# miniufo/xinvert

Measured on AMD Instinct MI355X. Metric: SOR grid-points*iters/sec (fp64) at 3600x1800, masked points counted, higher is better.
Workload: dtype f64

## Files before the change

include/xinv.h:

```cpp
#ifndef XINV_H
#define XINV_H

#include <stdint.h>

#ifdef __cplusplus
extern "C" {
#endif

#define XINV_BC_FIXED    0
#define XINV_BC_EXTEND   1
#define XINV_BC_PERIODIC 2

#define XINV_OK          0
#define XINV_ERR_ARG    -1
#define XINV_ERR_HIP    -2
#define XINV_ERR_NODEV  -3
#define XINV_ERR_NOMEM  -4

#define XINV_PATH_AUTO   0
#define XINV_PATH_COLOUR 1
#define XINV_PATH_FUSED  2
#define XINV_PATH_WAVE1D 4

#define XINV_FLAG_NO_XUNIFORM 1
#define XINV_FLAG_NO_TILE_SKIP 2
#define XINV_FLAG_FORCE_TILE_SKIP 4
#define XINV_FLAG_FMA 32
#define XINV_FLAG_PIN_HOST 8

#define XINV_FLAG_NO_PIPE 16

#define XINV_FLAG_NO_POINT_FACTOR 64

#define XINV_MAX_DEVICES 16

typedef struct xinv_options {
    int32_t device;
    int32_t path;
    int32_t sweeps_per_launch;
    int32_t check_every;
    int32_t rows_per_tile;
    int32_t timing;
    int32_t flags;
    int32_t rowconst_mask;
    int32_t host_chunk;
    int32_t ndev;
    int32_t device_ids[XINV_MAX_DEVICES];
    int32_t prep_flags;
    int32_t f32_mask;
    double  prep_undef;
    double  demask_value;
    const double *prep_rowscale;
    int32_t lanes;
    int32_t norm_lag;
    int32_t pipe_fr;
    int32_t graph;
    int32_t cu_count;
    int32_t host_inflight;
} xinv_options;

#define XINV_PREP_MASK_NAN   1
#define XINV_PREP_MASK_VALUE 2
#define XINV_PREP_ROWSCALE   4
#define XINV_PREP_S_ZERO     8
#define XINV_PREP_DEMASK    16

typedef struct xinv_stats {
    int32_t path;
    int32_t colours;
    int32_t sweeps_per_launch;
    int32_t rows_per_tile;
    int32_t xuniform_mask;
    int32_t masked_tile_pct;
    int64_t sweep_launches;
    int64_t sweeps_max;
    double  sweep_ms;
    double  h2d_ms, d2h_ms;
    double  wall_ms;
    int32_t host_chunks;
    int32_t devices;
    int32_t pipelined;
    int32_t masked_tile_ppm;
    int32_t recovered_members;
    int32_t lanes;
    int32_t planned;
    int32_t point_factor;
    double  plan_ms;
    int32_t k_chunks;
    int32_t cut_tiles;
    int32_t rolling;
    int32_t reserved_;
    double  launch_us_min, launch_us_avg, launch_us_max;
} xinv_stats;

void        xinv_default_options(xinv_options *opt);
int         xinv_last_stats(xinv_stats *out);
const char *xinv_last_error(void);
int         xinv_device_count(void);
int         xinv_version(void);
void        xinv_abi_sizes(int32_t *options_bytes, int32_t *stats_bytes);

int xinv_standard_2d_f64(double *S, const double *A, const double *B, const double *C,
                         const double *F, int64_t yc, int64_t xc, double dely, double delx,
                         int BCy, int BCx, double delxSqr, double ratioQtr, double ratioSqr,
                         double optArg, double undef, double *flags, int64_t mxLoop,
                         double tolerance);

int xinv_general_2d_f64(double *S, const double *A, const double *B, const double *C,
                        const double *D, const double *E, const double *F, const double *G,
                        int64_t yc, int64_t xc, double dely, double delx, int BCy, int BCx,
                        double delxSqr, double ratio, double ratioQtr, double ratioSqr,
                        double optArg, double undef, double *flags, int64_t mxLoop,
                        double tolerance);

int xinv_standard_3d_f64(double *S, const double *A, const double *B, const double *C,
                         const double *F, int64_t zc, int64_t yc, int64_t xc, double delz,
                         double dely, double delx, int BCz, int BCy, int BCx, double delxSqr,
                         double ratio2Sqr, double ratio1Sqr, double optArg, double undef,
                         double *flags, int64_t mxLoop, double tolerance);

int xinv_standard_2d_f64_batched(double *S, const double *A, const double *B, const double *C,
                                 const double *F, int64_t nbatch, const int64_t *strides,
                                 int64_t yc, int64_t xc, double dely, double delx, int BCy,
                                 int BCx, double delxSqr, double ratioQtr, double ratioSqr,
                                 double optArg, double undef, double *flags, int64_t mxLoop,
                                 double tolerance, const xinv_options *opt);

int xinv_general_2d_f64_batched(double *S, const double *A, const double *B, const double *C,
                                const double *D, const double *E, const double *F,
                                const double *G, int64_t nbatch, const int64_t *strides,
                                int64_t yc, int64_t xc, double dely, double delx, int BCy,
                                int BCx, double delxSqr, double ratio, double ratioQtr,
                                double ratioSqr, double optArg, double undef, double *flags,
                                int64_t mxLoop, double tolerance, const xinv_options *opt);

int xinv_standard_3d_f64_batched(double *S, const double *A, const double *B, const double *C,
                                 const double *F, int64_t nbatch, const int64_t *strides,
                                 int64_t zc, int64_t yc, int64_t xc, double delz, double dely,
                                 double delx, int BCz, int BCy, int BCx, double delxSqr,
                                 double ratio2Sqr, double ratio1Sqr, double optArg,
                                 double undef, double *flags, int64_t mxLoop, double tolerance,
                                 const xinv_options *opt);

int xinv_standard_2d_f64_dev(double *S, const double *A, const double *B, const double *C,
                             const double *F, int64_t nbatch, const int64_t *strides,
                             int64_t yc, int64_t xc, double dely, double delx, int BCy,
                             int BCx, double delxSqr, double ratioQtr, double ratioSqr,
                             double optArg, double undef, double *flags, int64_t mxLoop,
                             double tolerance, const xinv_options *opt, void *stream);

int xinv_general_2d_f64_dev(double *S, const double *A, const double *B, const double *C,
                            const double *D, const double *E, const double *F, const double *G,
                            int64_t nbatch, const int64_t *strides, int64_t yc, int64_t xc,
                            double dely, double delx, int BCy, int BCx, double delxSqr,
                            double ratio, double ratioQtr, double ratioSqr, double optArg,
                            double undef, double *flags, int64_t mxLoop, double tolerance,
                            const xinv_options *opt, void *stream);

int xinv_standard_3d_f64_dev(double *S, const double *A, const double *B, const double *C,
                             const double *F, int64_t nbatch, const int64_t *strides,
                             int64_t zc, int64_t yc, int64_t xc, double delz, double dely,
                             double delx, int BCz, int BCy, int BCx, double delxSqr,
                             double ratio2Sqr, double ratio1Sqr, double optArg, double undef,
                             double *flags, int64_t mxLoop, double tolerance,
                             const xinv_options *opt, void *stream);

int xinv_general_3d_f64(double *S, const double *A, const double *B, const double *C,
                        const double *D, const double *E, const double *F, const double *G,
                        const double *H, int64_t zc, int64_t yc, int64_t xc, double delz,
                        double dely, double delx, int BCz, int BCy, int BCx, double delxSqr,
                        double ratio2, double ratio1, double ratio2Sqr, double ratio1Sqr,
                        double optArg, double undef, double *flags, int64_t mxLoop,
                        double tolerance);

int xinv_general_3d_f64_batched(double *S, const double *A, const double *B, const double *C,
                                const double *D, const double *E, const double *F,
                                const double *G, const double *H, int64_t nbatch,
                                const int64_t *strides, int64_t zc, int64_t yc, int64_t xc,
                                double delz, double dely, double delx, int BCz, int BCy, int BCx,
                                double delxSqr, double ratio2, double ratio1, double ratio2Sqr,
                                double ratio1Sqr, double optArg, double undef, double *flags,
                                int64_t mxLoop, double tolerance, const xinv_options *opt);

int xinv_general_3d_f64_dev(double *S, const double *A, const double *B, const double *C,
                            const double *D, const double *E, const double *F, const double *G,
// ... 145 lines not shown
```

xinvert_amd/_lib.py:

```python
import ctypes
import os

import numpy as np

HERE = os.path.dirname(os.path.abspath(__file__))
SO = os.environ.get('XINV_SO') or os.path.join(HERE, 'libxinv_hip.so')

BC_CODES = {'fixed': 0, 'extend': 1, 'periodic': 2}
PATH_AUTO, PATH_COLOUR, PATH_FUSED, PATH_WAVE1D = 0, 1, 2, 4
PREP_MASK_NAN, PREP_MASK_VALUE, PREP_ROWSCALE, PREP_S_ZERO, PREP_DEMASK = 1, 2, 4, 8, 16
MAX_DEVICES = 16

_dp = ctypes.POINTER(ctypes.c_double)
_ip = ctypes.POINTER(ctypes.c_int64)
_i64, _f64, _int, _vp = ctypes.c_int64, ctypes.c_double, ctypes.c_int, ctypes.c_void_p
_pvp = ctypes.POINTER(ctypes.c_void_p)


class XinvOptions(ctypes.Structure):
    _fields_ = [('device', ctypes.c_int32), ('path', ctypes.c_int32),
                ('sweeps_per_launch', ctypes.c_int32), ('check_every', ctypes.c_int32),
                ('rows_per_tile', ctypes.c_int32), ('timing', ctypes.c_int32),
                ('flags', ctypes.c_int32), ('rowconst_mask', ctypes.c_int32),
                ('host_chunk', ctypes.c_int32), ('ndev', ctypes.c_int32),
                ('device_ids', ctypes.c_int32 * MAX_DEVICES),
                ('prep_flags', ctypes.c_int32), ('f32_mask', ctypes.c_int32),
                ('prep_undef', ctypes.c_double), ('demask_value', ctypes.c_double),
                ('prep_rowscale', ctypes.POINTER(ctypes.c_double)),
                ('lanes', ctypes.c_int32), ('norm_lag', ctypes.c_int32),
                ('pipe_fr', ctypes.c_int32), ('graph', ctypes.c_int32),
                ('cu_count', ctypes.c_int32), ('host_inflight', ctypes.c_int32)]


class XinvStats(ctypes.Structure):
    _fields_ = [('path', ctypes.c_int32), ('colours', ctypes.c_int32),
                ('sweeps_per_launch', ctypes.c_int32), ('rows_per_tile', ctypes.c_int32),
                ('xuniform_mask', ctypes.c_int32), ('masked_tile_pct', ctypes.c_int32),
                ('sweep_launches', ctypes.c_int64), ('sweeps_max', ctypes.c_int64),
                ('sweep_ms', ctypes.c_double), ('h2d_ms', ctypes.c_double),
                ('d2h_ms', ctypes.c_double), ('wall_ms', ctypes.c_double),
                ('host_chunks', ctypes.c_int32), ('devices', ctypes.c_int32),
                ('pipelined', ctypes.c_int32), ('masked_tile_ppm', ctypes.c_int32),
                ('recovered_members', ctypes.c_int32), ('lanes', ctypes.c_int32),
                ('planned', ctypes.c_int32), ('point_factor', ctypes.c_int32), ('plan_ms', ctypes.c_double),
                ('k_chunks', ctypes.c_int32), ('cut_tiles', ctypes.c_int32),
                ('rolling', ctypes.c_int32), ('reserved_', ctypes.c_int32),
                ('launch_us_min', ctypes.c_double), ('launch_us_avg', ctypes.c_double),
                ('launch_us_max', ctypes.c_double)]


class XinvError(RuntimeError):
    pass


EXPORTS = [
    'xinv_default_options', 'xinv_last_stats', 'xinv_last_error', 'xinv_device_count',
    'xinv_version', 'xinv_abi_sizes',
    'xinv_standard_2d_f64', 'xinv_general_2d_f64', 'xinv_standard_3d_f64',
    'xinv_standard_2d_f64_batched', 'xinv_general_2d_f64_batched',
    'xinv_standard_3d_f64_batched',
    'xinv_standard_2d_f64_dev', 'xinv_general_2d_f64_dev', 'xinv_standard_3d_f64_dev',
    'xinv_general_bih_2d_f64', 'xinv_general_bih_2d_f64_batched', 'xinv_general_bih_2d_f64_dev',
    'xinv_standard_2d_test_f64', 'xinv_standard_2d_test_f64_batched', 'xinv_standard_2d_test_f64_dev',
    'xinv_general_3d_f64', 'xinv_general_3d_f64_batched', 'xinv_general_3d_f64_dev',
    'xinv_standard_1d_f64', 'xinv_standard_1d_f64_batched', 'xinv_standard_1d_f64_dev',
    'xinv_gm_flow_f64_dev',
    'xinv_abs_norm_f64_dev',
    'xinv_fd_f64', 'xinv_fd_f64_dev',
    'xinv_mg_restrict_f64_dev', 'xinv_mg_prolong_f64_dev',
    'xinv_plan_create_standard_2d_f64_dev', 'xinv_plan_create_general_2d_f64_dev',
    'xinv_plan_create_standard_3d_f64_dev', 'xinv_plan_create_general_3d_f64_dev',
    'xinv_plan_create_general_bih_2d_f64_dev', 'xinv_plan_create_standard_2d_test_f64_dev',
    'xinv_plan_solve_f64_dev', 'xinv_plan_solve_frames_f64_dev', 'xinv_plan_refresh', 'xinv_plan_destroy',
]

_lib = None


def load():
    global _lib
    if _lib is not None:
        return _lib
    if not os.path.exists(SO):
        raise XinvError('HIP extension %s is missing: run `python -m xinvert_amd.build` '
                        '(there is no CPU fallback)' % SO)
    try:
        import torch
    except ImportError:
        pass
    try:
        L = ctypes.CDLL(SO)
    except OSError as e:
        raise XinvError('cannot load %s: %s' % (SO, e))
    _opt = ctypes.POINTER(XinvOptions)
    from . import forms
    for kind, f in forms.FORMS.items():
        for entry in ('single', 'batched', 'dev') + (('plan',) if f.resident else ()):
            getattr(L, forms.symbol(kind, entry)).argtypes = forms.argtypes(kind, entry)
    L.xinv_gm_flow_f64_dev.argtypes = [_vp, _vp, _vp, _i64, _i64, _i64, _vp, _vp, _int, _int, _vp, _f64, _int, _vp]
    L.xinv_abs_norm_f64_dev.argtypes = [_vp, _i64, _f64, _dp, _vp]
    fd_args = [_pvp, _int, _pvp, _int, _int, _ip, _int, _int, _ip, _dp, _vp, _i64, _int, _i64]
    L.xinv_fd_f64.argtypes = fd_args
    L.xinv_fd_f64_dev.argtypes = fd_args + [_vp]
    L.xinv_mg_restrict_f64_dev.argtypes = [_vp, _vp, _i64, _int, _ip, _ip, _f64, _vp]
    L.xinv_mg_prolong_f64_dev.argtypes = [_vp, _vp, _vp, _i64, _int, _ip, _ip, _vp, _vp, _int, _f64, _vp]
    L.xinv_plan_solve_f64_dev.argtypes = [_vp, _vp, _dp, _i64, _f64, _vp]
    L.xinv_plan_solve_frames_f64_dev.argtypes = [_vp, _vp, _vp, _i64, _i64, _dp, _i64, _f64, _vp]
    L.xinv_plan_refresh.argtypes = [_vp, _vp]
    L.xinv_plan_destroy.argtypes = [_vp]
    for name in EXPORTS:
        getattr(L, name).restype = _int
    L.xinv_last_error.restype = ctypes.c_char_p
    L.xinv_default_options.restype = None
    L.xinv_default_options.argtypes = [_opt]
    L.xinv_last_stats.argtypes = [ctypes.POINTER(XinvStats)]
    so, ss = ctypes.c_int32(0), ctypes.c_int32(0)
    try:
        abi_sizes = L.xinv_abi_sizes
    except AttributeError:
        raise XinvError('%s predates xinv_abi_sizes (a stale prebuilt library): rebuild it with '
                        '`python -m xinvert_amd.build --force`' % SO) from None
    abi_sizes.restype = None
    abi_sizes(ctypes.byref(so), ctypes.byref(ss))
    if (so.value, ss.value) != (ctypes.sizeof(XinvOptions), ctypes.sizeof(XinvStats)):
        raise XinvError('%s was built from another include/xinv.h: xinv_options %d / xinv_stats %d bytes there, %d / %d '
                        'in xinvert_amd/_lib.py' % (SO, so.value, ss.value, ctypes.sizeof(XinvOptions),
                                                    ctypes.sizeof(XinvStats)))
    _lib = L
    return L


def require_gpu():
    L = load()
    if L.xinv_device_count() < 1:
        raise XinvError('libxinv_hip.so loaded but no MI355X/HIP device is visible '
                        '(there is no CPU fallback)')
    return L


def check(rc):
    if rc != 0:
        raise XinvError('xinv call failed (rc=%d): %s' % (rc, load().xinv_last_error().decode()))


def options(device=-1, path=PATH_AUTO, sweeps_per_launch=0, check_every=0, rows_per_tile=0,
            timing=0, no_xuniform=0, no_tile_skip=0, force_tile_skip=0, rowconst_mask=0,
            host_chunk=0, devices=None, prep=None, pin_host=0, no_pipe=0, fma=0, f32_mask=0,
            lanes=0, norm_lag=0, pipe_fr=0, graph=0, no_point_factor=0, cu_count=0, host_inflight=0):
    o = XinvOptions()
    load().xinv_default_options(ctypes.byref(o))
    o.device, o.path, o.sweeps_per_launch = device, path, sweeps_per_launch
    o.check_every, o.rows_per_tile, o.timing = check_every, rows_per_tile, timing
    o.flags = (1 if no_xuniform else 0) | (2 if no_tile_skip else 0) | (4 if force_tile_skip else 0) | \
              (8 if pin_host else 0) | (16 if no_pipe else 0) | (32 if fma else 0) | \
              (64 if no_point_factor else 0)
    o.rowconst_mask = int(rowconst_mask)
    o.host_chunk = int(host_chunk)
    o.f32_mask = int(f32_mask)
    o.lanes, o.norm_lag, o.pipe_fr, o.graph = int(lanes), int(norm_lag), int(pipe_fr), int(graph)
    o.cu_count = int(cu_count)
    o.host_inflight = int(host_inflight)
    if prep:
        fl = 0
        if isinstance(prep.get('mask'), str):
            fl |= PREP_MASK_NAN
        elif prep.get('mask') is not None:
            fl |= PREP_MASK_VALUE
            o.prep_undef = float(prep['mask'])
        if prep.get('rowscale') is not None:
            rs = np.ascontiguousarray(prep['rowscale'], dtype=np.float64)
            o._rowscale_keepalive = rs
            o.prep_rowscale = rs.ctypes.data_as(ctypes.POINTER(ctypes.c_double))
            fl |= PREP_ROWSCALE
        if prep.get('s_zero'):
            fl |= PREP_S_ZERO
        if 'demask' in prep and prep['demask'] is not None:
            fl |= PREP_DEMASK
            o.demask_value = float(prep['demask'])
        o.prep_flags = fl
    if devices is None:
        o.ndev = 0
    elif isinstance(devices, str):
        if devices != 'all':
            raise XinvError("devices must be None, 'all' or a list of device ordinals")
        o.ndev = -1
    else:
        devices = [int(d) for d in devices]
        if len(devices) > MAX_DEVICES:
            raise XinvError('at most %d devices' % MAX_DEVICES)
        o.ndev = len(devices)
        for i, d in enumerate(devices):
            o.device_ids[i] = d
    return o


def last_stats():
    s = XinvStats()
    load().xinv_last_stats(ctypes.byref(s))
    return {f: getattr(s, f) for f, _ in XinvStats._fields_}


def bc(b):
    if isinstance(b, str):
        if b not in BC_CODES:
            raise XinvError('unknown boundary condition %r' % (b,))
        return BC_CODES[b]
    return int(b)


def hptr(a, f32=False):
    if a is None:
        return None
    want = np.float32 if f32 else np.float64
    if a.dtype != want or not a.flags.c_contiguous:
        raise XinvError('need a C-contiguous %s array at the C-ABI here, got %s%s'
                        % (np.dtype(want).name, a.dtype.name, '' if a.flags.c_contiguous else ' (not contiguous)'))
    return ctypes.cast(a.ctypes.data, _dp)


def strides_arg(vals):
    return (ctypes.c_int64 * len(vals))(*[int(v) for v in vals])
```

xinvert_amd/csrc/xinv_device.h:

```cpp
#pragma once
#include <hip/hip_runtime.h>
#include <stdint.h>
#include <float.h>
#include <math.h>

#define XINV_WAVE 64

__device__ __forceinline__ void xinv_fresh_scalar_cache()
{
    asm volatile("s_dcache_inv\n\ts_waitcnt lgkmcnt(0)" ::: "memory");
}

struct XinvCtl {
    double normPrev;
    double flag1;
    double flag2;
    long long loop;
    long long sweeps;
    int done;
    int overflow;
    int wrote;
    unsigned ticket;
    unsigned seq;
    unsigned pad_;
};

struct XinvStop {
    long long mxLoop;
    double tolerance;
    int stop_on_zero_norm;
};

__device__ __forceinline__ int xinv_ctl_done(const XinvCtl *c)
{
    return __hip_atomic_load(&c->done, __ATOMIC_RELAXED, __HIP_MEMORY_SCOPE_AGENT);
}
__device__ __forceinline__ unsigned xinv_ctl_seq(const XinvCtl *c)
{
    return __hip_atomic_load(&c->seq, __ATOMIC_RELAXED, __HIP_MEMORY_SCOPE_AGENT);
}

__device__ __forceinline__ void xinv_ctl_update(XinvCtl *c, double sum, long long count,
                                                const XinvStop &st)
{
    if (c->done) return;
    double norm = (count != 0) ? sum / (double)count : NAN;
    if (isnan(norm) || norm > 1e100) {
        c->overflow = 1;
        c->done = 1;
        c->sweeps = c->loop + 1;
        return;
    }
    c->flag1 = fabs(norm - c->normPrev) / c->normPrev;
    c->flag2 = (double)c->loop;
    c->wrote = 1;
    if (c->flag1 < st.tolerance || c->loop >= st.mxLoop ||
        (st.stop_on_zero_norm && norm == 0.0)) {
        c->done = 1;
        c->sweeps = c->loop + 1;
        return;
    }
    c->normPrev = norm;
    c->loop += 1;
}

template <int CTRL, int ROW_MASK>
__device__ __forceinline__ double xinv_dpp_add(double v)
{
    int lo = __builtin_amdgcn_update_dpp(0, __double2loint(v), CTRL, ROW_MASK, 0xf, true);
    int hi = __builtin_amdgcn_update_dpp(0, __double2hiint(v), CTRL, ROW_MASK, 0xf, true);
    return v + __hiloint2double(hi, lo);
}

__device__ __forceinline__ double xinv_wave_sum(double v)
{
    v = xinv_dpp_add<0x111, 0xf>(v);
    v = xinv_dpp_add<0x112, 0xf>(v);
    v = xinv_dpp_add<0x114, 0xf>(v);
    v = xinv_dpp_add<0x118, 0xf>(v);
    v = xinv_dpp_add<0x142, 0xa>(v);
    v = xinv_dpp_add<0x143, 0xc>(v);
    const int lo = __builtin_amdgcn_readlane(__double2loint(v), 63);
    const int hi = __builtin_amdgcn_readlane(__double2hiint(v), 63);
    return __hiloint2double(hi, lo);
}

template <int CTRL, int ROW_MASK>
__device__ __forceinline__ long long xinv_dpp_add_ll(long long v)
{
    const int lo = __builtin_amdgcn_update_dpp(0, (int)(unsigned long long)v, CTRL, ROW_MASK, 0xf, true);
    const int hi = __builtin_amdgcn_update_dpp(0, (int)((unsigned long long)v >> 32), CTRL, ROW_MASK, 0xf, true);
    return v + (long long)(((unsigned long long)(unsigned)hi << 32) | (unsigned)lo);
}

__device__ __forceinline__ long long xinv_wave_sum_ll(long long v)
{
    v = xinv_dpp_add_ll<0x111, 0xf>(v);
    v = xinv_dpp_add_ll<0x112, 0xf>(v);
    v = xinv_dpp_add_ll<0x114, 0xf>(v);
    v = xinv_dpp_add_ll<0x118, 0xf>(v);
    v = xinv_dpp_add_ll<0x142, 0xa>(v);
    v = xinv_dpp_add_ll<0x143, 0xc>(v);
    const unsigned lo = (unsigned)__builtin_amdgcn_readlane((int)(unsigned long long)v, 63);
    const unsigned hi = (unsigned)__builtin_amdgcn_readlane((int)((unsigned long long)v >> 32), 63);
    return (long long)(((unsigned long long)hi << 32) | lo);
}

__device__ __forceinline__ double xinv_lane_up(double v)
{
    int lo = __double2loint(v), hi = __double2hiint(v);
    lo = __builtin_amdgcn_update_dpp(0, lo, 0x138, 0xf, 0xf, true);
    hi = __builtin_amdgcn_update_dpp(0, hi, 0x138, 0xf, 0xf, true);
    return __hiloint2double(hi, lo);
}

__device__ __forceinline__ double xinv_lane_down(double v)
{
    int lo = __double2loint(v), hi = __double2hiint(v);
    lo = __builtin_amdgcn_update_dpp(0, lo, 0x130, 0xf, 0xf, true);
    hi = __builtin_amdgcn_update_dpp(0, hi, 0x130, 0xf, 0xf, true);
    return __hiloint2double(hi, lo);
}

__device__ __forceinline__ double xinv_add_where(double a, double b, unsigned long long mask)
{
    unsigned long long sv;
    asm("s_and_saveexec_b64 %1, %3\n\tv_add_f64 %0, %0, %2\n\ts_mov_b64 exec, %1"
        : "+v"(a), "=&s"(sv) : "v"(b), "s"(mask) : "scc");
    return a;
}
__device__ __forceinline__ double xinv_add_abs_where(double a, double b, unsigned long long mask)
{
    unsigned long long sv;
    asm("s_and_saveexec_b64 %1, %3\n\tv_add_f64 %0, %0, |%2|\n\ts_mov_b64 exec, %1"
        : "+v"(a), "=&s"(sv) : "v"(b), "s"(mask) : "scc");
    return a;
}

__device__ __forceinline__ double xinv_add_where_ne(double a, double b, double f, double u, unsigned long long rowmask)
{
    unsigned long long sv;
    asm("s_and_saveexec_b64 %1, %5\n\tv_cmpx_neq_f64_e32 vcc, %4, %3\n\tv_add_f64 %0, %0, %2\n\ts_mov_b64 exec, %1"
        : "+v"(a), "=&s"(sv) : "v"(b), "v"(f), "s"(u), "s"(rowmask) : "scc", "vcc");
    return a;
}
__device__ __forceinline__ double xinv_fma_where_ne(double a, double t, double rq, double f, double u, unsigned long long rowmask)
{
    unsigned long long sv;
    asm("s_and_saveexec_b64 %1, %6\n\tv_cmpx_neq_f64_e32 vcc, %5, %4\n\tv_fma_f64 %0, %2, %3, %0\n\ts_mov_b64 exec, %1"
        : "+v"(a), "=&s"(sv) : "v"(t), "s"(rq), "v"(f), "s"(u), "s"(rowmask) : "scc", "vcc");
    return a;
}
__device__ __forceinline__ void xinv_norm_row(double &sx, double &sy, int &nx, int &ny, double x, double y, double u)
{
    unsigned long long sv;
    asm("s_mov_b64 %4, exec\n\t"
        "v_cmpx_neq_f64_e32 vcc, %7, %5\n\tv_add_f64 %0, %0, |%5|\n\tv_add_u32 %2, %2, 1\n\ts_mov_b64 exec, %4\n\t"
        "v_cmpx_neq_f64_e32 vcc, %7, %6\n\tv_add_f64 %1, %1, |%6|\n\tv_add_u32 %3, %3, 1\n\ts_mov_b64 exec, %4"
        : "+v"(sx), "+v"(sy), "+v"(nx), "+v"(ny), "=&s"(sv) : "v"(x), "v"(y), "s"(u) : "vcc");
}

struct XinvScal {
    double delx, delxSqr, ratio, ratioQtr, ratioSqr;
    double ratio2Sqr, ratio1Sqr;
    double ratio2, ratio1;
    double delxSSr, delxTr, ratioSSr;
    double optArg, undef;
};


__device__ __forceinline__ double xinv_upd_std2d_9(
    double sC, double sP, double sM, double sW, double sE,
    double sPE, double sPW, double sME, double sMW, double sM_q,
    double aP, double a0, double bE, double bW, double bP_chk, double bP_use, double bM,
    double cE, double c0, double f, const XinvScal &sc)
{
    const double u = sc.undef;
    bool cond = (f != u) && (aP != u) && (a0 != u) && (bE != u) && (bW != u) &&
                (bP_chk != u) && (bM != u) && (cE != u) && (c0 != u);
    if (!cond) return sC;
    double temp = (
        (
            aP * (sP - sC) -
            a0 * (sC - sM)
        ) * sc.ratioSqr + (
            bP_use * (sPE - sPW) -
            bM * (sM_q - sMW)
        ) * sc.ratioQtr + (
            bE * (sPE - sME) -
            bW * (sPW - sMW)
        ) * sc.ratioQtr + (
            cE * (sE - sC) -
            c0 * (sC - sW)
        )
    ) - f * sc.delxSqr;
    temp *= sc.optArg / ((aP + a0) * sc.ratioSqr + (cE + c0));
    return sC + temp;
}

__device__ __forceinline__ double xinv_upd_std2d_5(
    double sC, double sP, double sM, double sW, double sE,
    double aP, double a0, double cE, double c0, double f, bool inrange, const XinvScal &sc)
{
    const double u = sc.undef;
    bool cond = inrange && (f != u) && (aP != u) && (a0 != u) && (cE != u) && (c0 != u);
    double temp = (
        (
            aP * (sP - sC) -
            a0 * (sC - sM)
        ) * sc.ratioSqr + (
            cE * (sE - sC) -
            c0 * (sC - sW)
        )
    ) - f * sc.delxSqr;
    temp *= sc.optArg / ((aP + a0) * sc.ratioSqr + (cE + c0));
    return cond ? sC + temp : sC;
}

__device__ __forceinline__ double xinv_upd_gen2d_9(
    double sC, double sP, double sM, double sW, double sE,
    double sPE, double sPW, double sME, double sMW,
    double A, double B, double C, double D, double E, double F, double G, const XinvScal &sc)
{
    const double u = sc.undef;
    bool cond = (G != u) && (A != u) && (B != u) && (C != u) && (D != u) && (E != u) && (F != u);
    if (!cond) return sC;
    double temp = (
        A * (
            (sP - sC) - (sC - sM)
        ) * sc.ratioSqr +
        B * (
            (sPE - sME) - (sPW - sMW)
        ) * sc.ratioQtr +
        C * (
            (sE - sC) - (sC - sW)
        ) + (
        D * (
            (sP - sM)
        ) * sc.ratio +
        E * (
            (sE - sW)
        )) * sc.delx / 2.0 + (
        F * sC - G) * sc.delxSqr
    );
    temp *= sc.optArg / ((A * sc.ratioSqr + C) * 2.0
                         - F * sc.delxSqr);
    return sC + temp;
}

__device__ __forceinline__ double xinv_upd_gen2d_5(
    double sC, double sP, double sM, double sW, double sE,
    double A, double C, double D, double E, double F, double G, bool inrange,
    const XinvScal &sc)
{
    const double u = sc.undef;
    bool cond = inrange && (G != u) && (A != u) && (C != u) && (D != u) && (E != u) && (F != u);
    double temp = (
        A * (
            (sP - sC) - (sC - sM)
        ) * sc.ratioSqr +
        C * (
            (sE - sC) - (sC - sW)
        ) + (
        D * (
            (sP - sM)
        ) * sc.ratio +
        E * (
            (sE - sW)
        )) * sc.delx / 2.0 + (
        F * sC - G) * sc.delxSqr
    );
    temp *= sc.optArg / ((A * sc.ratioSqr + C) * 2.0
                         - F * sc.delxSqr);
    return cond ? sC + temp : sC;
}

__device__ __forceinline__ double xinv_upd_std3d(
    double sC, double sKP, double sKM, double sJP, double sJM, double sE, double sW,
    double aP, double a0, double bP, double b0, double cE, double c0, double f,
    const XinvScal &sc)
{
    const double u = sc.undef;
    bool cond = (f != u) && (aP != u) && (a0 != u) && (bP != u) && (b0 != u) &&
                (cE != u) && (c0 != u);
    if (!cond) return sC;
    double temp = (
        (
            aP * (sKP - sC) -
            a0 * (sC - sKM)
        ) * sc.ratio2Sqr + (
            bP * (sJP - sC) -
            b0 * (sC - sJM)
        ) * sc.ratio1Sqr + (
            cE * (sE - sC) -
            c0 * (sC - sW)
        )
    ) - f * sc.delxSqr;
    temp *= sc.optArg / ((aP + a0) * sc.ratio2Sqr +
                         (bP + b0) * sc.ratio1Sqr +
                         (cE + c0));
    return sC + temp;
}

__device__ __forceinline__ double xinv_upd_gen3d(
    double sC, double sKP, double sKM, double sJP, double sJM, double sE, double sW,
    double A, double B, double C, double D, double E, double F, double G, double H, bool testH,
    const XinvScal &sc)
{
    const double u = sc.undef;
    bool cond = (!testH || H != u) && (G != u) && (A != u) && (B != u) && (C != u) && (D != u) &&
                (E != u) && (F != u);
    if (!cond) return sC;
// ... 191 lines not shown
```

xinvert_amd/csrc/xinv_dispatch.h:

```cpp
#pragma once
#include <hip/hip_runtime.h>
#include "xinv_fused.h"
#include "xinv_pipe2d.h"
#include "xinv_fused3d.h"
#include "xinv_fused3dg.h"
#include "xinv_pipe3d.h"
#include "xinv_fusedbih.h"

#define XINV_HIDDEN __attribute__((visibility("hidden")))

XINV_HIDDEN int xinv_launch_fused2d_std(bool al, bool ext, unsigned um, int K, dim3 grid, dim3 block,
                                        hipStream_t st, const FusedArgs &a, int *occ);
XINV_HIDDEN int xinv_launch_fused2d_gen(bool al, bool ext, unsigned um, int K, dim3 grid, dim3 block,
                                        hipStream_t st, const FusedArgs &a, int *occ);
XINV_HIDDEN int xinv_launch_fused2d_std2dt(bool al, bool ext, unsigned um, int K, dim3 grid, dim3 block,
                                           hipStream_t st, const FusedArgs &a, int *occ);
XINV_HIDDEN int xinv_launch_fused2d_std_seam(bool al, bool ext, unsigned um, int K, dim3 grid, dim3 block,
                                             hipStream_t st, const FusedArgs &a, int *occ);
XINV_HIDDEN int xinv_launch_fused2d_gen_seam(bool al, bool ext, unsigned um, int K, dim3 grid, dim3 block,
                                             hipStream_t st, const FusedArgs &a, int *occ);
XINV_HIDDEN int xinv_launch_fused2d_std2dt_seam(bool al, bool ext, unsigned um, int K, dim3 grid, dim3 block,
                                                hipStream_t st, const FusedArgs &a, int *occ);
XINV_HIDDEN int xinv_launch_fused2d_stdf(bool al, bool ext, unsigned um, int K, dim3 grid, dim3 block,
                                         hipStream_t st, const FusedArgs &a, int *occ);
XINV_HIDDEN int xinv_launch_fused2d_genf(bool al, bool ext, unsigned um, int K, dim3 grid, dim3 block,
                                         hipStream_t st, const FusedArgs &a, int *occ);
XINV_HIDDEN int xinv_launch_fused2d_genq(bool al, bool ext, unsigned um, int K, dim3 grid, dim3 block,
                                         hipStream_t st, const FusedArgs &a, int *occ);
XINV_HIDDEN int xinv_launch_pipe2d_fma(bool gen, unsigned um, bool fr, bool al, bool ext, dim3 grid, hipStream_t st,
                                       const FusedArgs &a, int *occ, int lds_pad);
XINV_HIDDEN int xinv_launch_pipe2d_std(unsigned um, int np, bool fr, bool al, bool ext, dim3 grid, hipStream_t st,
                                       const FusedArgs &a, int *occ, int lds_pad);
XINV_HIDDEN int xinv_launch_pipe2d_gen(unsigned um, int np, bool fr, bool al, bool ext, dim3 grid, hipStream_t st,
                                       const FusedArgs &a, int *occ, int lds_pad);
XINV_HIDDEN int xinv_launch_pipe2d_std_seam(unsigned um, int np, bool fr, bool al, bool ext, dim3 grid, hipStream_t st,
                                            const FusedArgs &a, int *occ, int lds_pad);
XINV_HIDDEN int xinv_launch_pipe2d_gen_seam(unsigned um, int np, bool fr, bool al, bool ext, dim3 grid, hipStream_t st,
                                            const FusedArgs &a, int *occ, int lds_pad);
static inline int xinv_launch_pipe2d(bool gen, unsigned um, int np, bool fr, bool al, bool ext, dim3 grid, hipStream_t st,
                                     const FusedArgs &a, int *occ, int lds_pad = 0, bool seam = false, bool fma = false)
{
    if (fma) return (seam || np != 1) ? 1 : xinv_launch_pipe2d_fma(gen, um, fr, al, ext, grid, st, a, occ, lds_pad);
    if (seam) return gen ? xinv_launch_pipe2d_gen_seam(um, np, fr, al, ext, grid, st, a, occ, lds_pad)
                         : xinv_launch_pipe2d_std_seam(um, np, fr, al, ext, grid, st, a, occ, lds_pad);
    return gen ? xinv_launch_pipe2d_gen(um, np, fr, al, ext, grid, st, a, occ, lds_pad)
               : xinv_launch_pipe2d_std(um, np, fr, al, ext, grid, st, a, occ, lds_pad);
}
XINV_HIDDEN int xinv_launch_fused9(bool gen, int K, bool al, bool ext, dim3 grid, hipStream_t st,
                                   const FusedArgs &a, int *occ, bool seam = false);
XINV_HIDDEN int xinv_launch_fused3d(int NW, bool al, bool uni, bool ext, dim3 grid, hipStream_t st,
                                    const Fused3Args &a);
XINV_HIDDEN int xinv_launch_pipe3d(bool al, dim3 grid, hipStream_t st, const Fused3Args &a, bool seam = false, bool ext = false);
XINV_HIDDEN int xinv_launch_fused3d_seam(int NW, bool uni, bool ext, dim3 grid, hipStream_t st, const Fused3Args &a);
XINV_HIDDEN int xinv_launch_fused3dg_seam(int NW, bool ext, dim3 grid, hipStream_t st, const Fused3GArgs &a);
XINV_HIDDEN int xinv_launch_fused3d_fma(int NW, bool al, bool ext, dim3 grid, hipStream_t st, const Fused3Args &a);
XINV_HIDDEN int xinv_launch_pipe3d_fma(bool al, dim3 grid, hipStream_t st, const Fused3Args &a);
XINV_HIDDEN int xinv_launch_fused3dg(int NW, bool al, bool ext, dim3 grid, hipStream_t st,
                                     const Fused3GArgs &a);
XINV_HIDDEN int xinv_launch_fusedbih(bool per, bool zbe, int vm, dim3 grid, hipStream_t st,
                                     const FusedBihArgs &a, int *occ);
```

xinvert_amd/csrc/xinv_fused.h:

```cpp
#pragma once
#include "xinv_device.h"
#include <type_traits>
#include <utility>

#define XINV_KMAX 4
#ifndef XINV_TEST_HOOKS
#define XINV_TEST_HOOKS 0
#endif
#if XINV_TEST_HOOKS
#define XINV_WATCHDOG_TICKS 3000000ull
#else
#define XINV_WATCHDOG_TICKS 200000000ull
#endif
__device__ __forceinline__ bool xinv_hook_withhold(const void *hook, int T, unsigned tag, int64_t m)
{
#if XINV_TEST_HOOKS
    const int *h = reinterpret_cast<const int *>(hook);
    return h && __hip_atomic_load(h + 0, __ATOMIC_RELAXED, __HIP_MEMORY_SCOPE_AGENT) == T &&
           (unsigned)__hip_atomic_load(h + 1, __ATOMIC_RELAXED, __HIP_MEMORY_SCOPE_AGENT) == tag &&
           (int64_t)__hip_atomic_load(h + 2, __ATOMIC_RELAXED, __HIP_MEMORY_SCOPE_AGENT) == m;
#else
    (void)hook; (void)T; (void)tag; (void)m;
    return false;
#endif
}
typedef int64_t row_t;

struct FusedArgs {
    const double *src;
    double *dst;
    const double *c[7];
    int64_t sS, sc[7];
    int64_t yc, xc;
    int per, ext, tall;
    int nstrip, nrb, RY;
    int nwg;
    int force, no_ctl;
    int lag;
    unsigned tag;
    unsigned long long *lagp_psum;
    const double *lagp_xsum;
    const long long *lagp_xcnt;
    int lagp_NB, lagp_K;
    unsigned lagp_tag;
    int64_t member0;
    XinvScal sc_;
    XinvCtl *ctl;
    XinvStop stop;
    unsigned long long *psum;
    const int *tile_list;
    int ntl;
    const double *xsum;
    const long long *xcnt;
    const void *rowf;
    double *dbg;
};

#include "xinv_tiles.h"

template <class F, int... U>
__device__ __forceinline__ void xinv_unroll_steps(F &&f, std::integer_sequence<int, U...>)
{
    (f(std::integral_constant<int, U>{}), ...);
}

template <int X> __device__ __forceinline__ double comp(const double2 &v) { return X ? v.y : v.x; }
template <int X> __device__ __forceinline__ void setc(double2 &v, double t) { if (X) v.y = t; else v.x = t; }

template <int X> __device__ __forceinline__ void row_neighbours(const double2 &row, double &w, double &e)
{
    if (X == 0) { w = xinv_lane_up(row.y); e = row.y; }
    else        { w = row.x; e = xinv_lane_down(row.x); }
}

template <int NC, int D> struct CoefWin {
    double2 v[NC][D];
    double s[NC][D];
    double rq[D];
    double2 rqv[D];
    unsigned mx[D], my[D];
};

__device__ __forceinline__ unsigned xinv_lane_word(bool b)
{
    unsigned m = b ? ~0u : 0u;
    return m;
}

__device__ __forceinline__ double xinv_bitsel(unsigned m, double a, double b)
{
    const unsigned long long ua = (unsigned long long)__double_as_longlong(a);
    const unsigned long long ub = (unsigned long long)__double_as_longlong(b);
    const unsigned lo = ((unsigned)ua & m) | ((unsigned)ub & ~m);
    const unsigned hi = ((unsigned)(ua >> 32) & m) | ((unsigned)(ub >> 32) & ~m);
    return __longlong_as_double((long long)(((unsigned long long)hi << 32) | lo));
}

__device__ __forceinline__ double xinv_bitsel64(unsigned long long m, double a, double b)
{
    unsigned lo, hi;
    asm("v_cndmask_b32_e64 %0, %2, %3, %6\n\tv_cndmask_b32_e64 %1, %4, %5, %6"
        : "=&v"(lo), "=&v"(hi)
        : "v"((unsigned)__double2loint(b)), "v"((unsigned)__double2loint(a)),
          "v"((unsigned)__double2hiint(b)), "v"((unsigned)__double2hiint(a)), "s"(m));
    return __hiloint2double((int)hi, (int)lo);
}

template <int X, unsigned UM, int Q, int NC, int D>
__device__ __forceinline__ double cget(const CoefWin<NC, D> &w, int slot)
{
    if ((UM >> Q) & 1u) return w.s[Q][slot];
    return comp<X>(w.v[Q][slot]);
}

struct FusedStd2D {
    static constexpr int NC = 3;
    template <unsigned UM> static constexpr bool hoist() { return (UM & 3u) == 3u; }
    static constexpr int PIPE_PFR = 2;

    template <unsigned UM, int D, bool PRE = true>
    static __device__ __forceinline__ void derive(CoefWin<NC, D> &w, int sr, int s1, bool okx, bool oky,
                                                  const XinvScal &sc)
    {
        const double u = sc.undef;
        const double fx = cget<0, UM, 2>(w, s1), fy = cget<1, UM, 2>(w, s1);
        bool bx = okx && (fx != u), by = oky && (fy != u);
        if (hoist<UM>()) {
            const double aP = w.s[0][sr], a0 = w.s[0][s1], c = w.s[1][s1];
            w.rq[s1] = sc.optArg / ((aP + a0) * sc.ratioSqr + (c + c));
            const bool rok = (aP != u) && (a0 != u) && (c != u);
            bx = bx && rok; by = by && rok;
        } else {
            const double aPx = cget<0, UM, 0>(w, sr), aPy = cget<1, UM, 0>(w, sr);
            const double a0x = cget<0, UM, 0>(w, s1), a0y = cget<1, UM, 0>(w, s1);
            const double c0x = cget<0, UM, 1>(w, s1), c0y = cget<1, UM, 1>(w, s1);
            const double cEy = ((UM >> 1) & 1u) ? w.s[1][s1] : xinv_lane_down(w.v[1][s1].x);
            bx = bx && (aPx != u) && (a0x != u) && (c0y != u) && (c0x != u);
            by = by && (aPy != u) && (a0y != u) && (cEy != u) && (c0y != u);
        }
        w.mx[s1] = xinv_lane_word(bx);
        w.my[s1] = xinv_lane_word(by);
        if (PRE) {
            if (!((UM >> 2) & 1u)) { w.v[2][s1].x = fx * sc.delxSqr; w.v[2][s1].y = fy * sc.delxSqr; }
            else                   w.s[2][s1] = fx * sc.delxSqr;
        }
    }

    template <int X, unsigned UM, int D, bool PRE = true>
    static __device__ __forceinline__ double inc(const CoefWin<NC, D> &w, int sj, int sjp, double sC,
                                                 double sP, double sM, double sW, double sE,
                                                 const XinvScal &sc)
    {
        const double aP = cget<X, UM, 0>(w, sjp);
        const double a0 = cget<X, UM, 0>(w, sj);
        const double c0 = cget<X, UM, 1>(w, sj);
        double cE;
        if ((UM >> 1) & 1u) cE = w.s[1][sj];
        else if (X == 0)    cE = w.v[1][sj].y;
        else                cE = xinv_lane_down(w.v[1][sj].x);
        const double fd = PRE ? cget<X, UM, 2>(w, sj)
                              : cget<X, UM, 2>(w, sj) * sc.delxSqr;
        double temp = (
            (
                aP * (sP - sC) -
                a0 * (sC - sM)
            ) * sc.ratioSqr + (
                cE * (sE - sC) -
                c0 * (sC - sW)
            )
        ) - fd;
        if (hoist<UM>()) temp *= w.rq[sj];
        else             temp *= sc.optArg / ((aP + a0) * sc.ratioSqr + (cE + c0));
        return temp;
    }
    template <int X, unsigned UM, int D, bool PRE = true>
    static __device__ __forceinline__ double upd(const CoefWin<NC, D> &w, int sj, int sjp, double sC,
                                                 double sP, double sM, double sW, double sE,
                                                 const XinvScal &sc)
    {
        const double temp = inc<X, UM, D, PRE>(w, sj, sjp, sC, sP, sM, sW, sE, sc);
        return xinv_bitsel(X ? w.my[sj] : w.mx[sj], sC + temp, sC);
    }
};

struct FusedStd2DT {
    static constexpr int NC = 4;
    template <unsigned UM> static constexpr bool hoist() { return (UM & 7u) == 7u; }

    template <unsigned UM, int D>
    static __device__ __forceinline__ void derive(CoefWin<NC, D> &w, int sr, int s1, bool okx, bool oky,
                                                  const XinvScal &sc)
    {
        const double u = sc.undef;
        bool bx = okx && (cget<0, UM, 3>(w, s1) != u), by = oky && (cget<1, UM, 3>(w, s1) != u);
        if (hoist<UM>()) {
            const double aP = w.s[0][sr], a0 = w.s[0][s1], d = w.s[1][s1], e = w.s[2][s1];
            w.rq[s1] = sc.optArg / ((aP + a0) * sc.ratioSqr +
                                    (d + d) - e * sc.delxSqr);
            const bool rok = (aP != u) && (a0 != u) && (d != u) && (e != u);
            bx = bx && rok; by = by && rok;
        } else {
            const double d0x = cget<0, UM, 1>(w, s1), d0y = cget<1, UM, 1>(w, s1);
            const double dEy = ((UM >> 1) & 1u) ? w.s[1][s1] : xinv_lane_down(w.v[1][s1].x);
            bx = bx && (cget<0, UM, 0>(w, sr) != u) && (cget<0, UM, 0>(w, s1) != u) && (d0y != u) &&
                 (d0x != u) && (cget<0, UM, 2>(w, s1) != u);
            by = by && (cget<1, UM, 0>(w, sr) != u) && (cget<1, UM, 0>(w, s1) != u) && (dEy != u) &&
                 (d0y != u) && (cget<1, UM, 2>(w, s1) != u);
// ... 68 lines not shown
    template <int X, unsigned UM, int D, bool PRE = true>
    static __device__ __forceinline__ double inc(const CoefWin<NC, D> &w, int sj, int, double sC,
                                                 double sP, double sM, double sW, double sE,
                                                 const XinvScal &sc)
    {
        const double A = cget<X, UM, 0>(w, sj), C = cget<X, UM, 1>(w, sj);
        const double Dd = cget<X, UM, 2>(w, sj), E = cget<X, UM, 3>(w, sj);
        const double F = cget<X, UM, 4>(w, sj), G = cget<X, UM, 5>(w, sj);
        double temp = (
            A * (
                (sP - sC) - (sC - sM)
            ) * sc.ratioSqr +
            C * (
                (sE - sC) - (sC - sW)
            ) + (
            Dd * (
                (sP - sM)
            ) * sc.ratio +
            E * (
                (sE - sW)
            )) * sc.delx / 2.0 + (
            F * sC - G) * sc.delxSqr
        );
        if (hoist<UM>()) temp *= w.rq[sj];
        else if (PRE)    temp *= comp<X>(w.rqv[sj]);
        else             temp *= sc.optArg / ((A * sc.ratioSqr + C) * 2.0
                                              - F * sc.delxSqr);
        return temp;
    }
    template <int X, unsigned UM, int D, bool PRE = true>
    static __device__ __forceinline__ double upd(const CoefWin<NC, D> &w, int sj, int sjp, double sC,
                                                 double sP, double sM, double sW, double sE,
                                                 const XinvScal &sc)
    {
        const double temp = inc<X, UM, D, PRE>(w, sj, sjp, sC, sP, sM, sW, sE, sc);
        return xinv_bitsel(X ? w.my[sj] : w.mx[sj], sC + temp, sC);
    }
};

struct FusedStd2DF : FusedStd2D {
    static constexpr bool FMA = true;
    template <unsigned UM, int D, bool PRE = true>
    static __device__ __forceinline__ void derive(CoefWin<NC, D> &w, int sr, int s1, bool okx, bool oky,
                                                  const XinvScal &sc)
    { FusedStd2D::derive<UM, D, false>(w, sr, s1, okx, oky, sc); }
    template <int X, unsigned UM, int D, bool PRE = true>
    static __device__ __forceinline__ double inc(const CoefWin<NC, D> &w, int sj, int sjp, double sC,
                                                 double sP, double sM, double sW, double sE,
                                                 const XinvScal &sc)
    {
        static_assert(hoist<UM>(), "contracted arithmetic: per-row A and C only");
        const double aP = w.s[0][sjp], a0 = w.s[0][sj], c = w.s[1][sj];
        const double y = __builtin_fma(aP, sP - sC, -(a0 * (sC - sM)));
        const double x = __builtin_fma(c, sE - sC, -(c * (sC - sW)));
        double t = __builtin_fma(y, sc.ratioSqr, x);
        t = __builtin_fma(-cget<X, UM, 2>(w, sj), sc.delxSqr, t);
        return t;
    }
    template <int X, unsigned UM, int D, bool PRE = true>
    static __device__ __forceinline__ double upd(const CoefWin<NC, D> &w, int sj, int sjp, double sC,
                                                 double sP, double sM, double sW, double sE,
                                                 const XinvScal &sc)
    {
        const double t = inc<X, UM, D, PRE>(w, sj, sjp, sC, sP, sM, sW, sE, sc);
        return xinv_bitsel(X ? w.my[sj] : w.mx[sj], __builtin_fma(t, w.rq[sj], sC), sC);
    }
};

struct FusedGen2DF : FusedGen2D {
    static constexpr bool FMA = true;
    template <int X, unsigned UM, int D, bool PRE = true>
    static __device__ __forceinline__ double inc(const CoefWin<NC, D> &w, int sj, int, double sC,
                                                 double sP, double sM, double sW, double sE,
                                                 const XinvScal &sc)
    {
        static_assert((UM & 0x1fu) == 0x1fu, "contracted arithmetic: per-row A, C, D, E, F only");
        const double A = w.s[0][sj], C = w.s[1][sj], Dd = w.s[2][sj], E = w.s[3][sj], F = w.s[4][sj];
        const double G = cget<X, UM, 5>(w, sj);
        double t = (A * ((sP - sC) - (sC - sM))) * sc.ratioSqr;
        t = __builtin_fma(C, (sE - sC) - (sC - sW), t);
        double v = (Dd * (sP - sM)) * sc.ratio;
        v = __builtin_fma(E, sE - sW, v);
        t = __builtin_fma(v * sc.delx, 0.5, t);
        t = __builtin_fma(__builtin_fma(F, sC, -G), sc.delxSqr, t);
        return t;
    }
    template <int X, unsigned UM, int D, bool PRE = true>
    static __device__ __forceinline__ double upd(const CoefWin<NC, D> &w, int sj, int sjp, double sC,
                                                 double sP, double sM, double sW, double sE,
                                                 const XinvScal &sc)
    {
        const double t = inc<X, UM, D, PRE>(w, sj, sjp, sC, sP, sM, sW, sE, sc);
        return xinv_bitsel(X ? w.my[sj] : w.mx[sj], __builtin_fma(t, w.rq[sj], sC), sC);
    }
};

template <bool AC> struct FusedGen2DQ_ {
    static constexpr int NC = 7;
    static constexpr bool PQ = true;
    static constexpr int QI = 5;
    template <unsigned UM> static constexpr bool hoist() { return false; }
    static constexpr int PIPE_PFR = 1;
    template <unsigned UM, int D, bool PRE = true>
    static __device__ __forceinline__ void derive(CoefWin<NC, D> &w, int, int s1, bool okx, bool oky, const XinvScal &)
    {
        w.mx[s1] = xinv_lane_word(okx && (w.v[QI][s1].x != 0.0));
        w.my[s1] = xinv_lane_word(oky && (w.v[QI][s1].y != 0.0));
    }
    template <int X, unsigned UM, int D, bool PRE = true>
    static __device__ __forceinline__ double upd(const CoefWin<NC, D> &w, int sj, int sjp, double sC,
                                                 double sP, double sM, double sW, double sE,
                                                 const XinvScal &sc)
    {
        const double temp = inc<X, UM, D, PRE>(w, sj, sjp, sC, sP, sM, sW, sE, sc);
        return xinv_bitsel(X ? w.my[sj] : w.mx[sj], sC + temp, sC);
    }
    template <int X, unsigned UM, int D, bool PRE = true>
    static __device__ __forceinline__ double inc(const CoefWin<NC, D> &w, int sj, int, double sC,
                                                 double sP, double sM, double sW, double sE,
                                                 const XinvScal &sc)
    {
        const double A = cget<X, UM, 0>(w, sj), C = AC ? A : cget<X, UM, 1>(w, sj);
        const double Dd = cget<X, UM, 2>(w, sj), E = cget<X, UM, 3>(w, sj);
        const double F = cget<X, UM, 4>(w, sj), G = cget<X, UM, 6>(w, sj);
        double temp = (
            A * (
                (sP - sC) - (sC - sM)
            ) * sc.ratioSqr +
            C * (
                (sE - sC) - (sC - sW)
            ) + (
            Dd * (
                (sP - sM)
            ) * sc.ratio +
            E * (
                (sE - sW)
            )) * sc.delx / 2.0 + (
            F * sC - G) * sc.delxSqr
        );
        temp *= cget<X, UM, QI>(w, sj);
        return temp;
    }
};
using FusedGen2DQ = FusedGen2DQ_<false>;
using FusedGen2DQA = FusedGen2DQ_<true>;
template <class M, class = void> struct ModelPQ { static constexpr bool value = false; };
template <class M> struct ModelPQ<M, std::void_t<decltype(M::PQ)>> { static constexpr bool value = M::PQ; };

template <class M, class = void> struct ModelFma { static constexpr bool value = false; };
template <class M> struct ModelFma<M, std::void_t<decltype(M::FMA)>> { static constexpr bool value = M::FMA; };

template <int NC> struct RowPack { double2 s; double2 c[NC]; double cs[NC]; };

struct LaneCols {
    int64_t l0, l1;
    bool ok_x, ok_y;
    bool use_x, use_y;
    int cls_x, cls_y;
};

template <bool AL>
__device__ __forceinline__ double2 ld2(const double *p, int64_t row_off, const LaneCols &lc)
{
    if (AL) return *reinterpret_cast<const double2 *>(p + row_off + lc.l0);
    double2 v; v.x = p[row_off + lc.l0]; v.y = p[row_off + lc.l1]; return v;
}

template <bool AL>
__device__ __forceinline__ LaneCols make_lanecols(int64_t xu0, int H, int UW, int lane, int64_t xc,
                                                  bool per, int np = 1, int q = 0)
{
    LaneCols lc;
    const int64_t c0 = xu0 - H + 2 * np * lane + 2 * q, c1 = c0 + 1;
    if (per) {
        int64_t w0 = c0 % xc; if (w0 < 0) w0 += xc;
        int64_t w1 = c1 % xc; if (w1 < 0) w1 += xc;
        lc.l0 = w0; lc.l1 = w1;
        lc.ok_x = lc.ok_y = true;
        lc.cls_x = lc.cls_y = 1;
    } else {
        if (AL) {
            int64_t p = c0 < 0 ? 0 : (c0 > xc - 2 ? xc - 2 : c0);
            lc.l0 = p; lc.l1 = p + 1;
        } else {
            lc.l0 = c0 < 0 ? 0 : (c0 > xc - 1 ? xc - 1 : c0);
            lc.l1 = c1 < 0 ? 0 : (c1 > xc - 1 ? xc - 1 : c1);
        }
        lc.ok_x = (c0 >= 1 && c0 <= xc - 2);
        lc.ok_y = (c1 >= 1 && c1 <= xc - 2);
        lc.cls_x = lc.ok_x ? 1 : (c0 == 0 ? 2 : (c0 == xc - 1 ? 3 : 0));
        lc.cls_y = lc.ok_y ? 1 : (c1 == xc - 1 ? 3 : 0);
    }
    lc.use_x = (c0 >= xu0 && c0 < xu0 + UW && c0 < xc);
    lc.use_y = (c1 >= xu0 && c1 < xu0 + UW && c1 < xc);
    return lc;
}

struct RingSeam { unsigned long long lanes; bool any; };
__device__ __forceinline__ LaneCols make_lanecols_ring(int64_t xu0, int HW, int UW, int lane, int64_t xc, RingSeam &rs)
{
    LaneCols lc;
    const int64_t c0 = xu0 - HW + 2 * lane, c1 = c0 + 1, xv = xc + 1;
    int64_t w0 = c0 % xv; if (w0 < 0) w0 += xv;
    int64_t w1 = c1 % xv; if (w1 < 0) w1 += xv;
    lc.l0 = w0; lc.l1 = (w1 == xc) ? xc - 1 : w1;
    lc.ok_x = true; lc.ok_y = (w1 != xc);
    lc.cls_x = lc.cls_y = 1;
    lc.use_x = (c0 >= xu0 && c0 < xu0 + UW && c0 < xc);
    lc.use_y = (c1 >= xu0 && c1 < xu0 + UW && c1 < xc);
    rs.lanes = __builtin_amdgcn_ballot_w64(w0 == xc - 1);
    rs.any = rs.lanes != 0ull;
    return lc;
}

__device__ __forceinline__ void fused_extend_fix(double2 &edge, const double2 &inner,
                                                 const LaneCols &lc, bool tall, double u)
{
    const double inner_w = xinv_lane_up(inner.y);
    if (lc.cls_x == 1) { if (inner.x != u) edge.x = inner.x; }
    else if (lc.cls_x == 2) { if (inner.y != u) edge.x = inner.y; }
    else if (lc.cls_x == 3) {
        if (tall && inner.x != u) edge.x = inner.x;
        if (inner_w != u) edge.x = inner_w;
    }
    if (lc.cls_y == 1) { if (inner.y != u) edge.y = inner.y; }
    else if (lc.cls_y == 3) {
        if (tall && inner.y != u) edge.y = inner.y;
        if (inner.x != u) edge.y = inner.x;
    }
}

#define XINV_PW 3
template <int K, int NWV, bool EXTS = false>
__device__ __forceinline__ void xinv_norm_publish(const double (&acc)[K], const int (&cnt)[K],
                                                  int wave, int lane, int NB, int T, unsigned tag,
                                                  unsigned long long *pw, char *scr = nullptr, bool withhold = false)
{
    double (*ls)[K]; long long (*lcn)[K];
    if constexpr (EXTS) {
        ls = reinterpret_cast<double (*)[K]>(scr);
        lcn = reinterpret_cast<long long (*)[K]>(scr + sizeof(double) * NWV * K);
    } else {
        __shared__ double ls_[NWV][K];
        __shared__ long long lcn_[NWV][K];
        ls = ls_; lcn = lcn_;
    }
#pragma unroll
    for (int s = 0; s < K; s++) {
        double ws = xinv_wave_sum(acc[s]);
        long long wc = xinv_wave_sum_ll((long long)cnt[s]);
        if (lane == 0) { ls[wave][s] = ws; lcn[wave][s] = wc; }
    }
    __syncthreads();
    const unsigned long long hi = (unsigned long long)tag << 32;
    if (threadIdx.x < K && !withhold) {
        const int s = threadIdx.x;
        double ts = 0.0; long long tc = 0;
        for (int q = 0; q < NWV; q++) { ts += ls[q][s]; tc += lcn[q][s]; }
        const unsigned long long bits = (unsigned long long)__double_as_longlong(ts);
        unsigned long long *q = pw + ((size_t)s * NB + T) * XINV_PW;
        __hip_atomic_store(q + 0, hi | (bits & 0xffffffffull), __ATOMIC_RELAXED, __HIP_MEMORY_SCOPE_AGENT);
        __hip_atomic_store(q + 1, hi | (bits >> 32), __ATOMIC_RELAXED, __HIP_MEMORY_SCOPE_AGENT);
        __hip_atomic_store(q + 2, hi | (unsigned long long)(unsigned)tc, __ATOMIC_RELAXED,
                           __HIP_MEMORY_SCOPE_AGENT);
    }
}

template <int K, int NWV, bool EXTS = false>
__device__ __forceinline__ void xinv_norm_reduce(int wave, int lane, int NB, unsigned tag,
                                                 unsigned long long *pw, XinvCtl *ctl, const XinvStop &stop,
                                                 double xsum, long long xcnt, char *scr = nullptr)
{
    double (*ls)[K]; long long (*lcn)[K]; unsigned *s_timeout_p;
    if constexpr (EXTS) {
        ls = reinterpret_cast<double (*)[K]>(scr);
        lcn = reinterpret_cast<long long (*)[K]>(scr + sizeof(double) * NWV * K);
        s_timeout_p = reinterpret_cast<unsigned *>(scr + 2 * sizeof(double) * NWV * K);
    } else {
        __shared__ double ls_[NWV][K];
        __shared__ long long lcn_[NWV][K];
        __shared__ unsigned s_timeout_;
        ls = ls_; lcn = lcn_; s_timeout_p = &s_timeout_;
    }
#define s_timeout (*s_timeout_p)
    if (threadIdx.x == 0) s_timeout = 0u;
    const unsigned long long hi = (unsigned long long)tag << 32;
    constexpr int NT = NWV * XINV_WAVE, C = 4;
    const int tid = threadIdx.x, nitem = K * NB;
    double ps[K]; long long pc[K];
#pragma unroll
    for (int s = 0; s < K; s++) { ps[s] = 0.0; pc[s] = 0; }
    unsigned long long t0 = 0;
    bool timed_out = false;
    for (int base = 0; base < nitem && !timed_out; base += NT * C) {
        unsigned long long w[C][XINV_PW];
        bool ready;
        do {
            ready = true;
#pragma unroll
            for (int c = 0; c < C; c++) {
                const int i = base + c * NT + tid;
                if (i < nitem) {
#pragma unroll
                    for (int k = 0; k < XINV_PW; k++)
                        w[c][k] = __hip_atomic_load(pw + (size_t)i * XINV_PW + k, __ATOMIC_RELAXED,
                                                    __HIP_MEMORY_SCOPE_AGENT);
                } else {
#pragma unroll
                    for (int k = 0; k < XINV_PW; k++) w[c][k] = hi;
                }
            }
#pragma unroll
            for (int c = 0; c < C; c++)
#pragma unroll
                for (int k = 0; k < XINV_PW; k++) ready = ready && ((unsigned)(w[c][k] >> 32) == tag);
            if (!ready) {
                const unsigned long long now = __builtin_amdgcn_s_memrealtime();
                if (t0 == 0) t0 = now;
                else if (now - t0 > XINV_WATCHDOG_TICKS) { timed_out = true; s_timeout = 1u; }
            }
        } while (!ready && !timed_out);
#pragma unroll
        for (int c = 0; c < C; c++) {
            const int i = base + c * NT + tid;
            const double v = __longlong_as_double((long long)((w[c][1] << 32) | (w[c][0] & 0xffffffffull)));
            const long long n = (long long)(unsigned)w[c][2];
#pragma unroll
            for (int s = 0; s < K; s++) {
                const bool mine = (i < nitem) && (i >= s * NB) && (i < (s + 1) * NB);
                ps[s] += mine ? v : 0.0;
                pc[s] += mine ? n : 0;
            }
        }
    }
    __syncthreads();
    if (s_timeout) {
        if (tid == 0) {
            ctl->overflow = 2; ctl->done = 1; ctl->sweeps = ctl->loop + 1;
            ctl->seq = tag + 1u;
        }
        return;
    }
#pragma unroll
    for (int s = 0; s < K; s++) {
        double ws = xinv_wave_sum(ps[s]);
        long long wc = xinv_wave_sum_ll(pc[s]);
        if (lane == 0) { ls[wave][s] = ws; lcn[wave][s] = wc; }
    }
    __syncthreads();
    if (tid == 0) {
#pragma unroll
        for (int s = 0; s < K; s++) {
            double ts = 0.0; long long tc = 0;
            for (int q = 0; q < NWV; q++) { ts += ls[q][s]; tc += lcn[q][s]; }
            xinv_ctl_update(ctl, ts + xsum, tc + xcnt, stop);
        }
        ctl->seq = tag + 1u;
    }
#undef s_timeout
}

template <int K, int NWV, bool EXTS = false>
__device__ __forceinline__ void xinv_norm_finalize(const double (&acc)[K], const int (&cnt)[K],
// ... 441 lines not shown
```

xinvert_amd/csrc/xinv_launch.h:

```cpp
#pragma once

static inline unsigned cdiv(int64_t a, int64_t b) { return (unsigned)((a + b - 1) / b); }

#if XINV_TEST_HOOKS
static thread_local int *t_hook_record = nullptr;
#endif

struct Plan {
    int path, base, seam, ncol;
    int K, RY, nsg, nrb;
    int nkc, KC;
    bool K2;
    int nsg2, nrb2, nkc2, KC2;
    int joff2;
    int cus;
    int64_t srowf2;
    bool bih_zbe;
    int bih_vm;
    bool aligned;
    unsigned umask;
    unsigned um;
    bool even_split;
    bool nine;
    bool skip;
    SkipNormArgs skipna;
    int ntl, nskip;
    int skip_pct;
    int skip_ppm;
    double lone = 1.6;
    bool pipe;
    int tpw;
    int npair;
    bool pipe_fr;
    int64_t xc;
    bool fma;
    bool alias_ac;
    bool pq;
};

static unsigned pick_um(int kind, unsigned umask)
{
    if (kind == KIND_STD2D) return ((umask & 3u) == 3u) ? 3u : 0u;
    if (kind == KIND_STD2DT) return ((umask & 7u) == 7u) ? 7u : 0u;
    if ((umask & 0x1fu) == 0x1fu) return 0x1fu;
    if ((umask & 0x1cu) == 0x1cu) return 0x1cu;
    return 0u;
}

struct StreamMap {
    int n, c[6];
    int forcing;
    int nuni;
};
static const StreamMap &stream_map(int kind)
{
    static const StreamMap std2d = {3, {0, 2, 3}, 2, 2}, std2dt = {4, {0, 3, 4, 5}, 3, 3}, gen2d = {6, {0, 2, 3, 4, 5, 6}, 5, 5};
    return kind == KIND_STD2D ? std2d : (kind == KIND_STD2DT ? std2dt : gen2d);
}

static inline int strip_uw(const Plan &pl, int K, bool pipe)
{
    if (pl.seam) return xinv_ring_uw(pl.xc, pipe ? 2 * XINV_PIPE_P : 2 * K);
    return pipe ? XINV_PIPE_UW(pl.npair) : 128 - 4 * K;
}

static int p3_extend_joff(int64_t yc)
{
    static_assert(XINV_P3_RR == 3 && XINV_P3_G * XINV_P3_RR - 8 > 0, "k_pipe3d: three rows per wavefront");
    return xinv_p3_extend_joff(yc, XINV_P3_G * XINV_P3_RR - 8, 4, XINV_P3_RR);
}

static int fused_dispatch(int kind, bool al, bool ext, unsigned um, int K, dim3 grid, dim3 block,
                          hipStream_t st, const FusedArgs &a, int *occ, bool seam = false, bool fma = false, bool pq = false)
{
    if (pq) return (kind != KIND_GEN2D || seam || fma) ? 1 : xinv_launch_fused2d_genq(al, ext, um, K, grid, block, st, a, occ);
    if (fma) {
        if (seam || kind == KIND_STD2DT) return 1;
        return kind == KIND_GEN2D ? xinv_launch_fused2d_genf(al, ext, um, K, grid, block, st, a, occ)
                                  : xinv_launch_fused2d_stdf(al, ext, um, K, grid, block, st, a, occ);
    }
    if (seam) {
        if (kind == KIND_GEN2D) return xinv_launch_fused2d_gen_seam(al, ext, um, K, grid, block, st, a, occ);
        if (kind == KIND_STD2DT) return xinv_launch_fused2d_std2dt_seam(al, ext, um, K, grid, block, st, a, occ);
        return xinv_launch_fused2d_std_seam(al, ext, um, K, grid, block, st, a, occ);
    }
    if (kind == KIND_GEN2D) return xinv_launch_fused2d_gen(al, ext, um, K, grid, block, st, a, occ);
    if (kind == KIND_STD2DT) return xinv_launch_fused2d_std2dt(al, ext, um, K, grid, block, st, a, occ);
    return xinv_launch_fused2d_std(al, ext, um, K, grid, block, st, a, occ);
}

static bool ptr_al16(const void *p) { return (((uintptr_t)p) & 15u) == 0; }
static bool vec_aligned(const double *a, int64_t stride) { return ptr_al16(a) && !(stride & 1); }

template <class F>
static int for_member_chunks(int64_t member0, int64_t nmem, F launch, int64_t chunk = XINV_MEMBER_CHUNK)
{
    for (int64_t m0 = 0; m0 < nmem; m0 += chunk) {
        const int rc = launch(member0 + m0, std::min<int64_t>(chunk, nmem - m0));
        if (rc) return rc;
    }
    return XINV_OK;
}

static void launch_extend(const Problem &p, const Workspace *ws, hipStream_t st, double *S, int force, int64_t member0, int64_t nm)
{
    ExtendArgs e;
    e.S = S; e.sS = p.sS; e.yc = p.yc; e.xc = p.xc;
    e.kfirst = is3d(p.kind) ? 1 : 0;
    e.nk = is3d(p.kind) ? p.zc - 2 : 1;
    e.per = (p.BCx == XINV_BC_PERIODIC); e.tall = (p.kind != KIND_STD3D) && (p.yc > p.xc); e.force = force;
    e.undef = p.sc_.undef; e.ctl = ws->ctl; e.member0 = member0;
    dim3 g(cdiv(p.xc, 256), (unsigned)e.nk, (unsigned)nm), b(256, 1, 1);
    if (p.kind == KIND_BIH2D) hipLaunchKernelGGL(k_extend_bih, g, b, 0, st, e);
    else                      hipLaunchKernelGGL(k_extend, g, b, 0, st, e);
}

struct TsumPtrs { double *tsum; long long *tcnt; double *xsum; long long *xcnt; unsigned *ticket; size_t bytes; };
static TsumPtrs tsum_layout(void *buf, int64_t nbatch, int nskip)
{
    const size_t nb = (size_t)nbatch, nt = nb * (size_t)nskip, pair = sizeof(double) + sizeof(long long);
    const uintptr_t base = (uintptr_t)buf;
    TsumPtrs t;
    t.tsum = (double *)base;
    t.tcnt = (long long *)(base + nt * sizeof(double));
    t.xsum = (double *)(base + nt * pair);
    t.xcnt = (long long *)(base + nt * pair + nb * sizeof(double));
    t.ticket = (unsigned *)(base + (nt + nb) * pair);
    t.bytes = (nt + nb) * pair + nb * sizeof(unsigned);
    return t;
}

template <class A>
static void set_skip(A &a, const Workspace *ws, const Problem &p, const Plan &pl, int tpw)
{
    a.tile_list = ws->d_list;
    a.ntl = pl.ntl;
    a.nwg = pl.ntl / tpw;
    const TsumPtrs t = tsum_layout(ws->d_tsum, p.nbatch, pl.nskip);
    a.xsum = t.xsum; a.xcnt = t.xcnt;
}

template <class A>
static void set_lag(A &a, const Workspace *ws, const Problem &p, int K, unsigned lag_tag, NormLagArgs *lag_out,
                    const NormLagArgs *lag_prev)
{
    if (lag_tag) {
        a.lag = 1; a.tag = lag_tag;
        a.psum = (unsigned long long *)((char *)ws->partials + (size_t)((lag_tag - 1u) & 1u) * ws->partials_half);
        if (lag_prev && lag_prev->tag) {
            a.lagp_psum = lag_prev->psum; a.lagp_xsum = lag_prev->xsum; a.lagp_xcnt = lag_prev->xcnt;
            a.lagp_NB = lag_prev->NB; a.lagp_K = lag_prev->K; a.lagp_tag = lag_prev->tag;
        }
    }
    if (lag_out) {
        memset(lag_out, 0, sizeof *lag_out);
        lag_out->psum = a.psum; lag_out->ctl = ws->ctl; lag_out->stop = p.stop;
        lag_out->xsum = a.xsum; lag_out->xcnt = a.xcnt; lag_out->NB = a.nwg; lag_out->K = K; lag_out->tag = lag_tag;
    }
}

static void fused_args(FusedArgs &a, const Problem &p, const Plan &pl, const Workspace *ws, const double *src, double *dst,
                       int UW, int force, int no_ctl)
{
    memset(&a, 0, sizeof a);
    a.src = src; a.dst = dst; a.sS = p.sS;
    a.yc = p.yc; a.xc = p.xc;
    a.per = (p.BCx == XINV_BC_PERIODIC);
    a.ext = (p.BCy == XINV_BC_EXTEND);
    a.tall = (p.yc > p.xc);
    a.RY = pl.even_split ? 0 : pl.RY;
    a.nstrip = (int)cdiv(p.xc, UW);
    a.nrb = pl.even_split ? pl.nrb : (int)cdiv(p.yc, pl.RY);
    a.nwg = (int)cdiv((int64_t)a.nstrip * a.nrb, 4);
    a.force = force; a.no_ctl = no_ctl;
    a.sc_ = p.sc_; a.ctl = ws->ctl; a.stop = p.stop;
    a.psum = (unsigned long long *)ws->partials;
}

static int launch_fused(const Problem &p, const Plan &pl, int K, const double *src, double *dst,
                        Workspace *ws, hipStream_t st, int64_t member0, int64_t nmem, int force,
                        int no_ctl, unsigned lag_tag = 0, NormLagArgs *lag_out = nullptr,
                        const NormLagArgs *lag_prev = nullptr)
{
    FusedArgs a;
    const bool pipe = pl.pipe && K == pl.K;
    fused_args(a, p, pl, ws, src, dst, strip_uw(pl, K, pipe), force, no_ctl);
    const StreamMap &sm = stream_map(p.kind);
    for (int q = 0; q < sm.n; q++) { a.c[q] = p.c[sm.c[q]]; a.sc[q] = p.sc[sm.c[q]]; }
    if (pl.pq) {
        a.c[sm.forcing + 1] = a.c[sm.forcing]; a.sc[sm.forcing + 1] = a.sc[sm.forcing];
        a.c[sm.forcing] = (const double *)ws->d_pfac; a.sc[sm.forcing] = p.yc * p.xc;
    }
    if (pipe) { a.nwg = a.nstrip * a.nrb; a.rowf = ws->d_rowf; }
#if XINV_TEST_HOOKS
    a.dbg = (double *)t_hook_record;
#endif
    if (pl.skip && K == pl.K) set_skip(a, ws, p, pl, pl.tpw);
    set_lag(a, ws, p, K, lag_tag, lag_out, lag_prev);
    const int rc = for_member_chunks(member0, nmem, [&](int64_t m, int64_t nm) {
        a.member0 = m;
        dim3 grid((unsigned)a.nwg + (lag_tag ? 1u : 0u), (unsigned)nm, 1), block(256, 1, 1);
        if (pipe) {
            const int pad = std::max(0, XINV_ENV_INT("XINV_PIPE_LDSPAD", 0));
            xinv_launch_pipe2d(p.kind == KIND_GEN2D, pl.um, pl.npair, pl.pipe_fr, pl.aligned, a.ext != 0, grid, st, a, nullptr, pad, pl.seam != 0, pl.fma);
            return XINV_OK;
        }
        if (fused_dispatch(p.kind, pl.aligned, a.ext != 0, pl.um | (pl.alias_ac ? 2u : 0u), K, grid, block, st, a, nullptr, pl.seam != 0, pl.fma, pl.pq))
            return fail_arg("unsupported sweeps_per_launch for this kernel variant");
        return XINV_OK;
    });
    if (rc) return rc;
    HIPCHK(hipGetLastError());
    return XINV_OK;
}

static inline int strip9_uw(const Plan &pl, int K) { return pl.seam ? xinv_ring_uw(pl.xc, 4 * K) : 128 - 8 * K; }

static int launch_fused9(const Problem &p, const Plan &pl, int K, const double *src, double *dst,
                         Workspace *ws, hipStream_t st, int64_t member0, int64_t nmem, int force,
                         int no_ctl, unsigned lag_tag = 0, NormLagArgs *lag_out = nullptr,
                         const NormLagArgs *lag_prev = nullptr)
{
    FusedArgs a;
    fused_args(a, p, pl, ws, src, dst, strip9_uw(pl, K), force, no_ctl);
    const int nc = (p.kind == KIND_GEN2D) ? 7 : 4;
    for (int q = 0; q < nc; q++) { a.c[q] = p.c[q]; a.sc[q] = p.sc[q]; }
    if (pl.skip && K == pl.K) set_skip(a, ws, p, pl, 4);
    set_lag(a, ws, p, K, lag_tag, lag_out, lag_prev);
    const int rc = for_member_chunks(member0, nmem, [&](int64_t m, int64_t nm) {
        a.member0 = m;
        dim3 grid((unsigned)a.nwg + (lag_tag ? 1u : 0u), (unsigned)nm, 1);
        if (xinv_launch_fused9(p.kind == KIND_GEN2D, K, pl.aligned, a.ext != 0, grid, st, a, nullptr, pl.seam != 0))
            return fail_arg("unsupported sweeps_per_launch for the 9-point kernel");
        return XINV_OK;
    });
    if (rc) return rc;
    HIPCHK(hipGetLastError());
    return XINV_OK;
}

static int launch_fused3d(const Problem &p, const Plan &pl, int K, const double *src, double *dst,
                          Workspace *ws, hipStream_t st, int64_t member0, int64_t nmem, int force,
                          int no_ctl)
{
    Fused3Args a;
    memset(&a, 0, sizeof a);
    a.src = src; a.dst = dst; a.sS = p.sS;
    for (int q = 0; q < 4; q++) { a.c[q] = p.c[q]; a.sc[q] = p.sc[q]; }
    a.zc = p.zc; a.yc = p.yc; a.xc = p.xc;
    a.per = (p.BCx == XINV_BC_PERIODIC);
    a.force = force; a.no_ctl = no_ctl;
    a.sc_ = p.sc_; a.ctl = ws->ctl; a.stop = p.stop;
    a.psum = (unsigned long long *)ws->partials;
    int rc;
    if (K == 2) {
        if (!pl.K2) return fail_arg("internal: two-sweep 3-D pass without its plan");
        a.nstrip = pl.nsg2; a.njb = pl.nrb2; a.joff = pl.joff2;
        a.nkc = std::max(1, pl.nkc2); a.KC = pl.KC2;
        a.rowf = (const double *)ws->d_rowf; a.srowf = pl.srowf2;
        const int64_t NT2 = (int64_t)a.nstrip * a.njb;
        const int64_t mstep = std::max<int64_t>(1, std::min<int64_t>(XINV_MEMBER_CHUNK, ((int64_t)1 << 30) / (NT2 * a.nkc)));
        const bool ext2 = (p.BCy == XINV_BC_EXTEND);
        rc = for_member_chunks(member0, nmem, [&](int64_t m, int64_t nm) {
            a.member0 = m;
            if (ext2)
                for_member_chunks(m, nm, [&](int64_t q, int64_t nq) { launch_extend(p, ws, st, const_cast<double *>(src), force, q, nq); return XINV_OK; });
            a.nfull = xinv_p3_whole_tiles(NT2 * nm, a.nkc, a.KC, p.zc, pl.cus);
            const int64_t nwg = a.nfull + (NT2 * nm - a.nfull) * a.nkc;
            if (pl.fma) xinv_launch_pipe3d_fma(pl.aligned, dim3((unsigned)nwg, 1, 1), st, a);
            else        xinv_launch_pipe3d(pl.aligned, dim3((unsigned)nwg, 1, 1), st, a, pl.seam != 0, ext2);
            return XINV_OK;
        }, mstep);
    } else {
        a.nstrip = pl.nsg; a.njb = pl.nrb;
        a.nkc = std::max(1, pl.nkc); a.KC = pl.KC;
        const size_t NB = (size_t)pl.nsg * pl.nrb * a.nkc;
        const bool ext = (p.BCy == XINV_BC_EXTEND), uni = (pl.um == 7u);
        rc = for_member_chunks(member0, nmem, [&](int64_t m, int64_t nm) {
            a.member0 = m;
            dim3 grid((unsigned)NB, (unsigned)nm, 1);
            if (pl.seam ? xinv_launch_fused3d_seam(pl.RY, uni, ext, grid, st, a)
                : pl.fma ? xinv_launch_fused3d_fma(pl.RY, pl.aligned, ext, grid, st, a)
                         : xinv_launch_fused3d(pl.RY, pl.aligned, uni, ext, grid, st, a))
                return fail_arg("internal: no 3-D kernel variant for this cross-section");
            return XINV_OK;
        });
    }
    if (rc) return rc;
    HIPCHK(hipGetLastError());
    return XINV_OK;
}

static int launch_fusedbih(const Problem &p, const Plan &pl, const double *src, double *dst,
                           Workspace *ws, hipStream_t st, int64_t member0, int64_t nmem, int force,
                           int no_ctl, unsigned lag_tag = 0, NormLagArgs *lag_out = nullptr,
                           const NormLagArgs *lag_prev = nullptr, bool prepass = true)
{
    const bool per = (p.BCx == XINV_BC_PERIODIC);
    if (p.BCy == XINV_BC_EXTEND && prepass)
        for_member_chunks(member0, nmem, [&](int64_t m, int64_t nm) { launch_extend(p, ws, st, const_cast<double *>(src), force, m, nm); return XINV_OK; });
    FusedBihArgs a;
    memset(&a, 0, sizeof a);
    a.src = src; a.dst = dst; a.sS = p.sS;
    for (int q = 0; q < 10; q++) { a.c[q] = p.c[q]; a.sc[q] = p.sc[q]; }
    a.yc = p.yc; a.xc = p.xc; a.per = per;
    a.nstrip = (int)cdiv(p.xc, XINV_BIH_OWN(per)); a.nrb = pl.nrb; a.RB = pl.RY;
    a.nwg = (int)cdiv((int64_t)a.nstrip * a.nrb, 4);
    a.force = force; a.no_ctl = no_ctl;
    a.sc_ = p.sc_; a.ctl = ws->ctl; a.stop = p.stop;
    a.rowf = (const double *)ws->d_rowf;
    a.q = pl.bih_vm ? (const double *)ws->d_pfac : nullptr;
    a.psum = (unsigned long long *)ws->partials;
    if (pl.skip) set_skip(a, ws, p, pl, 4);
    set_lag(a, ws, p, 1, lag_tag, lag_out, lag_prev);
    for_member_chunks(member0, nmem, [&](int64_t m, int64_t nm) {
        a.member0 = m;
        dim3 grid((unsigned)a.nwg + (lag_tag ? 1u : 0u), (unsigned)nm, 1);
        xinv_launch_fusedbih(per, pl.bih_zbe, pl.bih_vm, grid, st, a, nullptr);
        return XINV_OK;
    });
    HIPCHK(hipGetLastError());
    return XINV_OK;
}

static int launch_fused3dg(const Problem &p, const Plan &pl, const double *src, double *dst,
                           Workspace *ws, hipStream_t st, int64_t member0, int64_t nmem, int force,
                           int no_ctl)
{
    Fused3GArgs a;
    memset(&a, 0, sizeof a);
    a.src = src; a.dst = dst; a.sS = p.sS;
    for (int q = 0; q < 8; q++) { a.c[q] = p.c[q]; a.sc[q] = p.sc[q]; }
    a.zc = p.zc; a.yc = p.yc; a.xc = p.xc;
    a.per = (p.BCx == XINV_BC_PERIODIC);
    a.nstrip = pl.nsg; a.njb = pl.nrb;
    a.nkc = std::max(1, pl.nkc); a.KC = pl.KC;
    a.force = force; a.no_ctl = no_ctl;
    a.sc_ = p.sc_; a.ctl = ws->ctl; a.stop = p.stop;
    const size_t NB = (size_t)pl.nsg * pl.nrb * a.nkc;
    a.psum = (unsigned long long *)ws->partials;
    const bool ext = (p.BCy == XINV_BC_EXTEND);
    const int rc = for_member_chunks(member0, nmem, [&](int64_t m, int64_t nm) {
        a.member0 = m;
        dim3 grid((unsigned)NB, (unsigned)nm, 1);
        if (pl.seam ? xinv_launch_fused3dg_seam(pl.RY, ext, grid, st, a) : xinv_launch_fused3dg(pl.RY, pl.aligned, ext, grid, st, a))
            return fail_arg("internal: no general 3-D kernel variant for this cross-section");
        return XINV_OK;
    });
    if (rc) return rc;
    HIPCHK(hipGetLastError());
    return XINV_OK;
}

static inline int seam_sequence(int pos, int base, int seam)
{
    static const int s2[4] = {0, 2, 1, 3}, s4[6] = {0, 4, 1, 2, 5, 3};
    if (!seam) return pos;
    return base == 2 ? s2[pos] : s4[pos];
}

static int launch_colour_chunk(const Problem &p, const Plan &pl, Workspace *ws, hipStream_t st,
                               int64_t m0, int64_t nm)
{
    const int per = (p.BCx == XINV_BC_PERIODIC);
    if (p.BCy == XINV_BC_EXTEND) launch_extend(p, ws, st, p.S, 0, m0, nm);
    if (p.kind == KIND_BIH2D) {
        ColourArgsBih a;
        memset(&a, 0, sizeof a);
        a.S = p.S; a.sS = p.sS;
        for (int q = 0; q < 10; q++) { a.c[q] = p.c[q]; a.sc[q] = p.sc[q]; }
        a.yc = p.yc; a.xc = p.xc; a.per = per; a.trail = pl.seam; a.force = 0; a.member0 = m0;
        a.sc_ = p.sc_; a.ctl = ws->ctl; a.umask = pl.umask;
        dim3 b(64, 4, 1);
        dim3 g(cdiv(cdiv(p.xc, 3) + 1, 64), cdiv(cdiv(p.yc, 3) + 1, 4), (unsigned)nm);
        if (!per || p.xc % 3 == 0) {
            dim3 gb(cdiv(cdiv(p.xc, 180), 4), cdiv(p.yc, 3) + 1, (unsigned)nm), bb(256, 1, 1);
            a.Y = ws->S2; a.sY = p.sS;
            for (int cj = 0; cj < 3; cj++) {
                a.colour = cj;
                if (per) {
                    if (pl.umask) hipLaunchKernelGGL((k_bih_rowclass<true, true>), gb, bb, 0, st, a);
                    else          hipLaunchKernelGGL((k_bih_rowclass<false, true>), gb, bb, 0, st, a);
                } else {
                    if (pl.umask) hipLaunchKernelGGL((k_bih_rowclass<true, false>), gb, bb, 0, st, a);
                    else          hipLaunchKernelGGL((k_bih_rowclass<false, false>), gb, bb, 0, st, a);
                }
            }
            hipLaunchKernelGGL(k_rows_copy_back, dim3(256, (unsigned)nm, 1), dim3(256), 0, st,
                               (const double *)ws->S2, p.sS, p.S, p.sS, p.yc, p.xc,
                               (const XinvCtl *)ws->ctl, m0, 0);
        } else
        for (int cc = 0; cc < pl.ncol; cc++) {
            a.colour = cc;
            if (pl.umask) hipLaunchKernelGGL(k_colour_bih2d<true>, g, b, 0, st, a);
            else          hipLaunchKernelGGL(k_colour_bih2d<false>, g, b, 0, st, a);
        }
    } else if (is3d(p.kind)) {
        ColourArgs3D a;
        memset(&a, 0, sizeof a);
        a.S = p.S; a.sS = p.sS;
        for (int q = 0; q < p.ncoef; q++) { a.c[q] = p.c[q]; a.sc[q] = p.sc[q]; }
        a.zc = p.zc; a.yc = p.yc; a.xc = p.xc;
        a.per = per; a.seam = pl.seam; a.force = 0; a.sc_ = p.sc_; a.ctl = ws->ctl;
        a.nbatch = p.nbatch; a.member0 = m0;
        dim3 b(64, 4, 1);
        dim3 g(cdiv(cdiv(p.xc, 2) + 1, 64), cdiv(p.yc - 2, 4), (unsigned)(nm * (p.zc - 2)));
        for (int pos = 0; pos < pl.ncol; pos++) {
            a.colour = seam_sequence(pos, 2, pl.seam);
            if (p.kind == KIND_GEN3D) hipLaunchKernelGGL(k_colour_gen3d, g, b, 0, st, a);
            else                      hipLaunchKernelGGL(k_colour_std3d, g, b, 0, st, a);
        }
    } else {
        ColourArgs2D a;
        memset(&a, 0, sizeof a);
        a.S = p.S; a.sS = p.sS;
        for (int q = 0; q < p.ncoef; q++) { a.c[q] = p.c[q]; a.sc[q] = p.sc[q]; }
        a.yc = p.yc; a.xc = p.xc;
        a.per = per; a.base = pl.base; a.seam = pl.seam; a.force = 0;
        a.sc_ = p.sc_; a.ctl = ws->ctl; a.member0 = m0;
        dim3 b(64, 4, 1);
        dim3 g(cdiv(cdiv(p.xc, 2) + 1, 64), cdiv(p.yc - 2, 4), (unsigned)nm);
        const bool nine = (pl.base == 4);
        for (int pos = 0; pos < pl.ncol; pos++) {
            a.colour = seam_sequence(pos, pl.base, pl.seam);
            if (p.kind == KIND_STD2D) {
                if (nine) hipLaunchKernelGGL(k_colour_std2d<true>, g, b, 0, st, a);
                else      hipLaunchKernelGGL(k_colour_std2d<false>, g, b, 0, st, a);
            } else if (p.kind == KIND_STD2DT) {
                if (nine) hipLaunchKernelGGL(k_colour_std2dt<true>, g, b, 0, st, a);
                else      hipLaunchKernelGGL(k_colour_std2dt<false>, g, b, 0, st, a);
            } else {
                if (nine) hipLaunchKernelGGL(k_colour_gen2d<true>, g, b, 0, st, a);
                else      hipLaunchKernelGGL(k_colour_gen2d<false>, g, b, 0, st, a);
            }
        }
    }
    NormArgs n;
    n.S = p.S; n.sS = p.sS; n.n = p.zc * p.yc * p.xc; n.undef = p.sc_.undef;
    n.psum = (double *)ws->partials;
    n.pcnt = (long long *)((char *)ws->partials + p.nbatch * XINV_NORM_BLOCKS * sizeof(double));
    n.ctl = ws->ctl; n.stop = p.stop; n.force = 0; n.member0 = m0;
    int nblk = (int)std::min<int64_t>(XINV_NORM_BLOCKS, std::max<int64_t>(1, n.n / 2048));
    hipLaunchKernelGGL(k_norm_partial, dim3(nblk, (unsigned)nm, 1), dim3(256, 1, 1), 0, st, n);
    hipLaunchKernelGGL(k_norm_final, dim3((unsigned)nm, 1, 1), dim3(64, 1, 1), 0, st, n, nblk);
    HIPCHK(hipGetLastError());
    return XINV_OK;
}

static int launch_colour_sweep(const Problem &p, const Plan &pl, Workspace *ws, hipStream_t st)
{
    int64_t chunk = XINV_MEMBER_CHUNK;
    if (is3d(p.kind)) chunk = std::max<int64_t>(1, 65535 / std::max<int64_t>(1, p.zc - 2));
    return for_member_chunks(0, p.nbatch, [&](int64_t m0, int64_t nm) { return launch_colour_chunk(p, pl, ws, st, m0, nm); }, chunk);
}

static int pipe_occ_cap()
{
    return std::max(1, XINV_ENV_INT("XINV_PIPE_OCC", 5));
}

static double tile_cost(int64_t wgs, int64_t rows, int K, int occ, double lone, bool pipe)
{
    return xinv_tile_cost(wgs, rows, K, occ, pipe ? pipe_occ_cap() : 3, lone, pipe ? XINV_PIPE_LAG : 0);
}

static int64_t choose_row_blocks(int64_t yc, int64_t nstrip, int64_t nbatch, int K, int occ, double lone, bool pipe)
{
    return xinv_choose_row_blocks(yc, nstrip, nbatch, K, occ, pipe ? pipe_occ_cap() : 3, lone, pipe ? XINV_PIPE_LAG : 0);
}

static int plan_occ(const Problem &p, const Plan &pl, hipStream_t st, int K, bool *have = nullptr)
{
    const bool ext = (p.BCy == XINV_BC_EXTEND);
    int occ, missing;
    if (p.kind == KIND_BIH2D) {
        FusedBihArgs dummy; memset(&dummy, 0, sizeof dummy);
        occ = 1;
        missing = xinv_launch_fusedbih(false, pl.bih_zbe, pl.bih_vm, dim3(1), st, dummy, &occ);
    } else {
        FusedArgs dummy; memset(&dummy, 0, sizeof dummy);
        occ = pl.nine ? 1 : 2;
        if (pl.nine) missing = xinv_launch_fused9(p.kind == KIND_GEN2D, K, pl.aligned, ext, dim3(1), st, dummy, &occ, pl.seam != 0);
        else if (pl.pipe) missing = xinv_launch_pipe2d(p.kind == KIND_GEN2D, pl.um, pl.npair, pl.pipe_fr, pl.aligned, ext, dim3(1), st, dummy, &occ, 0, pl.seam != 0, pl.fma);
        else missing = fused_dispatch(p.kind, pl.aligned, ext, pl.um | (pl.alias_ac ? 2u : 0u), K, dim3(1), dim3(256), st, dummy, &occ, pl.seam != 0, pl.fma, pl.pq);
    }
    if (have) *have = !missing;
    return occ;
}

static void split_rows_evenly(const Problem &p, Plan &pl, int64_t nrb)
{
    pl.nrb = (int)nrb;
    pl.even_split = true;
    pl.RY = (int)cdiv(p.yc, pl.nrb);
}
static bool rows_per_tile_given(const Problem &p, const xinv_options &opt, Plan &pl)
{
    pl.even_split = false;
    if (opt.rows_per_tile > 0) {
        pl.RY = (opt.rows_per_tile + 1) & ~1;
        pl.nrb = (int)cdiv(p.yc, pl.RY);
    } else if (opt.rows_per_tile < 0)
        split_rows_evenly(p, pl, std::max<int64_t>(1, std::min<int64_t>(-opt.rows_per_tile, p.yc / 2)));
    return opt.rows_per_tile != 0;
}

static int issue_strip_active(const Problem &p, Workspace *ws, hipStream_t st, int UW, int fi)
{
    const int64_t yc = p.yc, nb = p.nbatch;
    const int nstrip = (int)cdiv(p.xc, UW);
    const int64_t cells = yc * nstrip;
    int rc = ensure_dev(&ws->d_act, &ws->d_act_cap, (size_t)(nb * cells));
    if (rc) return rc;
    if (ws->h_act_cap < (size_t)(nb * cells)) {
        if (ws->h_act) HIPCHK(hipHostFree(ws->h_act));
        HIPCHK(hipHostMalloc((void **)&ws->h_act, (size_t)(nb * cells), hipHostMallocDefault));
        ws->h_act_cap = (size_t)(nb * cells);
    }
    StripActArgs sa;
    sa.f = p.c[fi]; sa.sf = p.sc[fi]; sa.yc = yc; sa.xc = p.xc; sa.nstrip = nstrip; sa.UW = UW;
    sa.undef = p.sc_.undef; sa.act = ws->d_act;
    hipLaunchKernelGGL(k_strip_active, dim3(cdiv(cells, 4), (unsigned)nb, 1), dim3(256), 0, st, sa);
    HIPCHK(hipMemcpyAsync(ws->h_act, ws->d_act, (size_t)(nb * cells), hipMemcpyDeviceToHost, st));
    ws->act_ready = true; ws->act_uw = UW; ws->act_f = p.c[fi]; ws->act_synced = false;
    return XINV_OK;
}

static int plan_tile_skip(const Problem &p, Plan &pl, Workspace *ws, hipStream_t st,
                          const xinv_options &opt, int fixedRB = 0, int UW_ = 0)
{
    pl.skip = false; pl.ntl = pl.nskip = 0; pl.skip_pct = 0; pl.skip_ppm = 0;
    const bool forced = (opt.flags & XINV_FLAG_FORCE_TILE_SKIP) != 0;
    const int tpw = pl.pipe ? 1 : 4;
    const int K = pl.K, UW = UW_ ? UW_ : strip_uw(pl, K, pl.pipe);
    const int nstrip = (int)cdiv(p.xc, UW);
    const int64_t wscale = 4 / tpw;
    if (!forced && ((int64_t)nstrip * pl.nrb * p.nbatch * wscale < 1024 || (int64_t)nstrip * pl.nrb * wscale < 64 ||
                    p.nbatch > 64))
        return XINV_OK;
    const int64_t yc = p.yc, nb = p.nbatch;
    const int64_t cells = yc * nstrip;
    if (nb * nstrip * (yc + 1) > (int64_t)50000000) return XINV_OK;
    const StreamMap &sm = stream_map(p.kind);
    const int fi = (p.kind == KIND_BIH2D) ? 9 : sm.c[sm.forcing];

    int rc = XINV_OK;
    if (!(ws->act_ready && ws->act_uw == UW && ws->act_f == p.c[fi])) {
        rc = issue_strip_active(p, ws, st, UW, fi);
        if (rc) return rc;
        HIPCHK(hipStreamSynchronize(st));
    } else if (!ws->act_synced)
        HIPCHK(hipStreamSynchronize(st));
    ws->act_ready = false;

    std::vector<int> &pre = ws->h_pre;
    pre.resize((size_t)(nb * nstrip * (yc + 1)));
    int64_t nact = 0;
    for (int64_t m = 0; m < nb; m++) {
        int *q = &pre[(size_t)(m * (yc + 1) * nstrip)];
        for (int s = 0; s < nstrip; s++) q[s] = 0;
        const unsigned char *ha = ws->h_act + m * yc * nstrip;
        for (int64_t r = 0; r < yc; r++, q += nstrip, ha += nstrip)
            for (int s = 0; s < nstrip; s++) q[nstrip + s] = q[s] + ha[s];
        for (int s = 0; s < nstrip; s++) nact += q[s];
    }
    if (!forced && (double)nact > 0.92 * (double)(nb * cells)) return XINV_OK;
    auto rows_active = [&](int64_t m, int strip, int64_t y0, int64_t y1) {
        const int *q = &pre[(size_t)(m * (yc + 1) * nstrip)];
        return q[y1 * nstrip + strip] - q[y0 * nstrip + strip] > 0;
    };

    const bool ext = (p.BCy == XINV_BC_EXTEND);
    auto ntile_ids = [&](int nrb) { return nstrip * nrb; };
    auto id_rb = [&](int, int id) { return id / nstrip; };
    auto tile_active = [&](int64_t m, int nrb, int id) {
        const int rb = id_rb(nrb, id);
        const TileRows t = xinv_tile_rows(id, nstrip, nrb, yc, fixedRB);
        if (t.y0 >= t.y1) return false;
        if (ext && (rb == 0 || rb >= nrb - (fixedRB ? 2 : 1))) return true;
        return rows_active(m, t.strip, t.y0, t.y1);
    };
    auto active_wgs = [&](int nrb, int64_t *maxact) {
        int64_t wgs = 0, mx = 0;
        for (int64_t m = 0; m < nb; m++) {
            int64_t c = 0;
            const int *q = &pre[(size_t)(m * (yc + 1) * nstrip)];
            for (int rb = 0; rb < nrb; rb++) {
                const TileRows t = xinv_tile_rows(rb * nstrip, nstrip, nrb, yc, fixedRB);
                if (t.y0 >= t.y1) continue;
                if (ext && (rb == 0 || rb >= nrb - (fixedRB ? 2 : 1))) { c += nstrip; continue; }
                const int *q0 = q + t.y0 * nstrip, *q1 = q + t.y1 * nstrip;
                for (int st_ = 0; st_ < nstrip; st_++) c += (q1[st_] - q0[st_]) > 0;
            }
            wgs += cdiv(c, tpw); mx = std::max(mx, c);
        }
        if (maxact) *maxact = mx;
        return wgs;
    };
    const int occ = fixedRB ? 2 : plan_occ(p, pl, st, K);
    const bool pp = pl.pipe;
    const double cost0 = tile_cost((int64_t)cdiv((int64_t)nstrip * pl.nrb, tpw) * nb, cdiv(yc, pl.nrb), K, occ, pl.lone, pp);
    int best = pl.nrb; double best_cost = 1e300;
    int lo = pl.nrb, hi = pl.nrb;
    if (!forced && opt.rows_per_tile == 0 && !fixedRB) {
        const int64_t w0 = active_wgs(pl.nrb, nullptr);
        const double share = std::max(0.05, (double)w0 / (double)((int64_t)cdiv((int64_t)nstrip * pl.nrb, tpw) * nb));
        const double centre = (double)pl.nrb / share;
        const int64_t cap_rows = std::max<int64_t>(pl.nrb, yc / 4);
        lo = (int)std::min<int64_t>(cap_rows, std::max<int64_t>(pl.nrb, (int64_t)(centre * 0.85)));
        hi = (int)std::min<int64_t>(cap_rows, std::max<int64_t>(lo, (int64_t)(centre * 1.10) + 1));
    }
    best_cost = tile_cost(active_wgs(pl.nrb, nullptr), cdiv(yc, pl.nrb), K, occ, pl.lone, pp);
    for (int nrb = lo; nrb <= hi; nrb++) {
        const double c = tile_cost(active_wgs(nrb, nullptr), cdiv(yc, nrb), K, occ, pl.lone, pp);
        if (c < best_cost) { best_cost = c; best = nrb; }
    }
    if (!forced && best_cost > 0.95 * cost0) return XINV_OK;

    int64_t maxact = 0;
    active_wgs(best, &maxact);
    const int64_t ntiles = (int64_t)ntile_ids(best);
    const int ntl = (int)(tpw * std::max<int64_t>(1, cdiv(maxact, tpw)));
    int64_t maxskip = 0, nskipped = 0;
    std::vector<std::vector<int>> act((size_t)nb), skp((size_t)nb);
    for (int64_t m = 0; m < nb; m++) {
        for (int id = 0; id < (int)ntiles; id++) {
            const TileRows t = xinv_tile_rows(id, nstrip, best, yc, fixedRB);
            if (t.y0 >= t.y1) continue;
            (tile_active(m, best, id) ? act[(size_t)m] : skp[(size_t)m]).push_back(id);
        }
        maxskip = std::max<int64_t>(maxskip, (int64_t)skp[(size_t)m].size());
        nskipped += (int64_t)skp[(size_t)m].size();
    }
    if (nskipped == 0) return XINV_OK;
    const int nskip = (int)maxskip;
    const size_t nints = (size_t)nb * ((size_t)ntl + nskip);
// ... 92 lines not shown
```

xinvert_amd/csrc/xinv_pipe2d.h:

```cpp
#pragma once
#include "xinv_fused.h"

#define XINV_PIPE_P 4
#ifndef XINV_PIPE_B
#define XINV_PIPE_B 2
#endif
#define XINV_PIPE_LAG (XINV_PIPE_B + 5)
#define XINV_PIPE_NS 4
#define XINV_PIPE_UW(np) (128 * (np) - 4 * XINV_PIPE_P)
#ifndef XINV_PIPE_PF0
#define XINV_PIPE_PF0 4
#endif
#ifndef XINV_PIPE_PF
#define XINV_PIPE_PF 4
#endif

template <class M, unsigned UM> struct PipeRec {
    static constexpr int NCO = M::NC - 1;
    static constexpr int NUNI = __builtin_popcount(UM & ((1u << NCO) - 1u));
    static constexpr bool HOIST = M::template hoist<UM>();
    static constexpr int NW = NUNI + (HOIST ? 2 : 0);
    static constexpr int RW = NW == 0 ? 0 : (NW <= 4 ? 4 : 8);
};

struct RowFactorArgs {
    const double *c[5];
    int64_t sc[5];
    int64_t yc, xc;
    int gen;
    unsigned um;
    int hoist, rw;
    XinvScal sc_;
    double *rowf;
};

#ifdef XINV_AUX_KERNELS
__global__ __launch_bounds__(256) void k_row_factor(RowFactorArgs a)
{
    const int64_t j = (int64_t)blockIdx.x * 256 + threadIdx.x, m = blockIdx.y;
    if (j >= a.yc) return;
    const double u = a.sc_.undef;
    const bool inner = (j >= 1 && j <= a.yc - 2);
    const int nco = a.gen ? 5 : 2;
    const double ones = __longlong_as_double(-1LL);
    double *f = a.rowf + (m * a.yc + j) * a.rw;
    double v[5];
    int k = 0;
    bool def = true;
    for (int q = 0; q < nco; q++) {
        v[q] = 0.0;
        if ((a.um >> q) & 1u) { v[q] = a.c[q][m * a.sc[q] + j * a.xc]; f[k++] = v[q]; def = def && (v[q] != u); }
    }
    if (a.hoist) {
        double rq = 0.0, rok = 0.0;
        if (inner) {
            if (!a.gen) {
                const double aP = a.c[0][m * a.sc[0] + (j + 1) * a.xc], a0 = v[0], c = v[1];
                rq = a.sc_.optArg / ((aP + a0) * a.sc_.ratioSqr + (c + c));
                rok = (def && (aP != u)) ? ones : 0.0;
            } else {
                const double A = v[0], C = v[1], F = v[4];
                rq = a.sc_.optArg / ((A * a.sc_.ratioSqr + C) * 2.0
                                     - F * a.sc_.delxSqr);
                rok = def ? ones : 0.0;
            }
        }
        f[k++] = rq; f[k++] = rok;
    }
    for (; k < a.rw; k++) f[k] = 0.0;
}
#endif

struct PointFactorArgs {
    const double *c[6];
    int64_t sc[6];
    int64_t yc, xc, n;
    XinvScal sc_;
    double *q;
    int *flag;
};
#ifdef XINV_AUX_KERNELS
__global__ __launch_bounds__(256) void k_point_factor(PointFactorArgs a)
{
    const int64_t m = blockIdx.y;
    const double u = a.sc_.undef;
    bool zero = false, differ = false;
    for (int64_t t = (int64_t)blockIdx.x * 256 + threadIdx.x; t < a.n; t += (int64_t)gridDim.x * 256) {
        const int64_t j = t / a.xc;
        const double A = a.c[0][m * a.sc[0] + t], C = a.c[1][m * a.sc[1] + t], Dd = a.c[2][m * a.sc[2] + t];
        const double E = a.c[3][m * a.sc[3] + t], F = a.c[4][m * a.sc[4] + t], G = a.c[5][m * a.sc[5] + t];
        differ = differ || (__double_as_longlong(A) != __double_as_longlong(C));
        const bool ok = (j >= 1) && (j <= a.yc - 2) && (G != u) && (A != u) && (C != u) && (Dd != u) && (E != u) && (F != u);
        double q = 0.0;
        if (ok) {
            q = a.sc_.optArg / ((A * a.sc_.ratioSqr + C) * 2.0
                                - F * a.sc_.delxSqr);
            zero = zero || (q == 0.0);
        }
        a.q[m * a.n + t] = q;
    }
    if (__any(zero) && (threadIdx.x & 63) == 0) atomicOr(a.flag, 1);
    if (__any(differ) && (threadIdx.x & 63) == 0) atomicOr(a.flag, 2);
}
#endif

__device__ __forceinline__ void xinv_pipe_barrier()
{
    asm volatile("s_waitcnt lgkmcnt(0)\n\ts_barrier" ::: "memory");
}

typedef const double __attribute__((address_space(4))) *xinv_cdouble_ptr;
typedef const char __attribute__((address_space(1))) *xinv_gcptr;
typedef char __attribute__((address_space(1))) *xinv_gptr;
typedef double xinv_v2d __attribute__((ext_vector_type(2)));
typedef const xinv_v2d __attribute__((address_space(1))) *xinv_gcd2ptr;
typedef const double __attribute__((address_space(1))) *xinv_gcdptr;
typedef xinv_v2d __attribute__((address_space(1))) *xinv_gd2ptr;
typedef double __attribute__((address_space(1))) *xinv_gdptr;

__device__ __forceinline__ void pipe_extend_fix(double2 &edge, const double2 &inner, double inner_w,
                                                const LaneCols &lc, bool tall, double u)
{
    if (lc.cls_x == 1) { if (inner.x != u) edge.x = inner.x; }
    else if (lc.cls_x == 2) { if (inner.y != u) edge.x = inner.y; }
    else if (lc.cls_x == 3) {
        if (tall && inner.x != u) edge.x = inner.x;
        if (inner_w != u) edge.x = inner_w;
    }
    if (lc.cls_y == 1) { if (inner.y != u) edge.y = inner.y; }
    else if (lc.cls_y == 3) {
        if (tall && inner.y != u) edge.y = inner.y;
        if (inner.x != u) edge.y = inner.x;
    }
}

template <class M, unsigned UM, bool FR, int NP, bool AL, bool EXT, int PW, int PF, bool SEAM = false>
__device__ __forceinline__ void xinv_pipe_wave(const FusedArgs &a, int64_t m, int yu0, int yu1,
                                               const LaneCols (&lc)[NP], const int64_t (&st0)[NP], int lane,
                                               double2 (*ring)[XINV_PIPE_NS][NP * (FR ? 2 : 1)][XINV_WAVE], int gtot,
                                               double &acc, int &cnt,
                                               unsigned long long seam_lanes = 0ull)
{
    constexpr int P = XINV_PIPE_P, H = 2 * P, D = 4, LAG = XINV_PIPE_LAG, B = XINV_PIPE_B;
    constexpr int R = PF + D;
    constexpr int PFR = M::PIPE_PFR;
    using REC = PipeRec<M, UM>;
    constexpr int NC = M::NC, FQ = M::NC - 1, RW = REC::RW;
    constexpr bool HOIST = REC::HOIST;
    constexpr int RS = FR ? 2 : 1;
    static_assert(R % D == 0 && R % B == 0 && R % XINV_PIPE_NS == 0,
                  "the unroll period must keep row parity, ring slots and barriers compile-time");
    const int ycr = (int)a.yc;
    const unsigned rowbytes = (unsigned)a.xc * 8u;
    const double u = a.sc_.undef;
    const int slice_bytes = (int)(rowbytes * (unsigned)ycr);
    const __amdgpu_buffer_rsrc_t rsS = __builtin_amdgcn_make_buffer_rsrc((void *)(a.src + m * a.sS), 0, slice_bytes, 0x00020000);
    const __amdgpu_buffer_rsrc_t rsD = __builtin_amdgcn_make_buffer_rsrc((void *)(a.dst + m * a.sS), 0, slice_bytes, 0x00020000);
    __amdgpu_buffer_rsrc_t rsC[NC];
#pragma unroll
    for (int q = 0; q < NC; q++)
        rsC[q] = __builtin_amdgcn_make_buffer_rsrc((void *)(a.c[q] + m * a.sc[q]), 0, slice_bytes, 0x00020000);
    const xinv_cdouble_ptr rowf = (xinv_cdouble_ptr)(uintptr_t)(reinterpret_cast<const double *>(a.rowf) + m * a.yc * RW);
    unsigned lo0[NP], lo1[NP], so0[NP], so1[NP];
#pragma unroll
    for (int q = 0; q < NP; q++) {
        lo0[q] = (unsigned)lc[q].l0 * 8u; lo1[q] = (unsigned)lc[q].l1 * 8u;
        so0[q] = lc[q].use_x ? (unsigned)st0[q] * 8u : 0xffffffffu;
        so1[q] = lc[q].use_y ? (unsigned)(st0[q] + 1) * 8u : 0xffffffffu;
    }

    unsigned long long okx64[NP], oky64[NP];
    double nsx[NP], nsy[NP];
    int nnx[NP], nny[NP];
#pragma unroll
    for (int q = 0; q < NP; q++) {
        okx64[q] = __builtin_amdgcn_ballot_w64(lc[q].ok_x) & ~seam_lanes; oky64[q] = __builtin_amdgcn_ballot_w64(lc[q].ok_y);
        nsx[q] = nsy[q] = 0.0; nnx[q] = nny[q] = 0;
    }
    static_assert(!SEAM || (NP == 1 && !AL && PipeRec<M, UM>::HOIST),
                  "seam variants: one column pair per lane, per-row records, updates under EXEC masks");

    const int in_lo = yu0 - H + 2 * PW;
    const int in_hi = yu1 - 1 + H - 2 * PW;

    double2 sw[NP][R];
    CoefWin<NC, R> cw[NP];
    double rokw[R];
#pragma unroll
    for (int t = 0; t < R; t++) {
        rokw[t] = 0.0;
#pragma unroll
        for (int q = 0; q < NP; q++) {
            sw[q][t] = make_double2(0.0, 0.0);
            cw[q].rq[t] = 0.0; cw[q].mx[t] = 0u; cw[q].my[t] = 0u;
#pragma unroll
            for (int c = 0; c < NC; c++) { cw[q].v[c][t] = make_double2(0.0, 0.0); cw[q].s[c][t] = 0.0; }
        }
    }

    const int maxo = (int)(rowbytes * (unsigned)(ycr - 1));
    int nxo = (yu0 - H + 2 * PW) * (int)rowbytes;
    int nxr = (yu0 - H + 2 * PW) * (RW * 8);
    auto ldrow = [&](__amdgpu_buffer_rsrc_t rs, int soff, auto qtag) {
        constexpr int q = decltype(qtag)::value;
        double2 v;
        if (AL) {
            const auto t = __builtin_amdgcn_raw_buffer_load_b128(rs, (int)lo0[q], soff, 0);
            v.x = __hiloint2double((int)t[1], (int)t[0]); v.y = __hiloint2double((int)t[3], (int)t[2]);
        } else {
            const auto t0 = __builtin_amdgcn_raw_buffer_load_b64(rs, (int)lo0[q], soff, 0);
            const auto t1 = __builtin_amdgcn_raw_buffer_load_b64(rs, (int)lo1[q], soff, 0);
            v.x = __hiloint2double((int)t0[1], (int)t0[0]); v.y = __hiloint2double((int)t1[1], (int)t1[0]);
        }
        return v;
    };
    auto request = [&](int, auto stag) {
        constexpr int slot = decltype(stag)::value;
        const int soff = min(max(nxo, 0), maxo);
        nxo += (int)rowbytes;
        asm("" : "+s"(nxo));
        xinv_unroll_steps([&](auto qtag) {
            constexpr int q = decltype(qtag)::value;
            if (PW == 0) sw[q][slot] = ldrow(rsS, soff, qtag);
            xinv_unroll_steps([&](auto ctag) {
                constexpr int c = decltype(ctag)::value;
                if (!((UM >> c) & 1u) && !(FR && c == FQ && PW > 0)) cw[q].v[c][slot] = ldrow(rsC[c], soff, qtag);
            }, std::make_integer_sequence<int, NC>{});
        }, std::make_integer_sequence<int, NP>{});
    };
    auto request_rf = [&](int, auto stag) {
        constexpr int slot = decltype(stag)::value;
        if constexpr (RW > 0) {
            const unsigned roff = (unsigned)min(max(nxr, 0), (ycr - 1) * (RW * 8));
            nxr += RW * 8;
            const xinv_cdouble_ptr pr = (xinv_cdouble_ptr)((const char __attribute__((address_space(4))) *)rowf + roff);
            double rec[RW];
#pragma unroll
            for (int k = 0; k < RW; k++) rec[k] = pr[k];
#pragma unroll
            for (int q = 0; q < NP; q++) {
                int k = 0;
#pragma unroll
                for (int c = 0; c < NC - 1; c++)
                    if ((UM >> c) & 1u) cw[q].s[c][slot] = rec[k++];
                if (HOIST) { cw[q].rq[slot] = rec[k]; rokw[slot] = rec[k + 1]; }
            }
        }
    };
    xinv_unroll_steps([&](auto ttag) { request(in_lo + decltype(ttag)::value, ttag); asm volatile("" ::: "memory"); },
                      std::make_integer_sequence<int, PF>{});
    xinv_unroll_steps([&](auto ttag) { request_rf(in_lo + decltype(ttag)::value, ttag); },
                      std::make_integer_sequence<int, PFR>{});

    auto half_pass = [&](auto xtag, auto jtag, auto ptag, auto mtag, auto fixt) {
        constexpr int X = decltype(xtag)::value, sj = decltype(jtag)::value, sjp = decltype(ptag)::value,
                      sjm = decltype(mtag)::value;
        constexpr bool FIX = decltype(fixt)::value;
        static_assert(!FIX || (X == 0 && NP == 1), "column xc-1 sits in an .x slot");
        const double edge = (X == 0) ? xinv_lane_up(sw[NP - 1][sj].y) : xinv_lane_down(sw[0][sj].x);
        double nv[NP];
#pragma unroll
        for (int q = 0; q < NP; q++) {
            double w, e;
            if (X == 0) { w = (q == 0) ? edge : sw[q > 0 ? q - 1 : 0][sj].y; e = sw[q][sj].y; }
            else        { w = sw[q][sj].x; e = (q == NP - 1) ? edge : sw[q < NP - 1 ? q + 1 : q][sj].x; }
            if constexpr (FIX) e = xinv_lane_down(sw[q][sj].x);
            const double t = M::template inc<X, UM, R, false>(cw[q], sj, sjp, comp<X>(sw[q][sj]), comp<X>(sw[q][sjp]),
                                              comp<X>(sw[q][sjm]), w, e, a.sc_);
            if constexpr (HOIST) {
                const unsigned long long rm = (FIX ? seam_lanes : (X ? oky64[q] : okx64[q])) &
                                              (unsigned long long)__double_as_longlong(rokw[sj]);
                if constexpr (ModelFma<M>::value)
                    nv[q] = xinv_fma_where_ne(comp<X>(sw[q][sj]), t, cw[q].rq[sj], comp<X>(cw[q].v[FQ][sj]), u, rm);
                else
                    nv[q] = xinv_add_where_ne(comp<X>(sw[q][sj]), t, comp<X>(cw[q].v[FQ][sj]), u, rm);
            } else {
                const unsigned long long pm = __builtin_amdgcn_ballot_w64((X ? cw[q].my[sj] : cw[q].mx[sj]) != 0u);
                nv[q] = xinv_add_where(comp<X>(sw[q][sj]), t, pm);
            }
        }
#pragma unroll
        for (int q = 0; q < NP; q++) setc<X>(sw[q][sj], nv[q]);
    };
    auto half_sweep = [&](auto xtag, auto jtag, auto ptag, auto mtag) {
        constexpr int X = decltype(xtag)::value;
        half_pass(xtag, jtag, ptag, mtag, std::false_type{});
        if constexpr (SEAM && X == 0) {
            constexpr int sj = decltype(jtag)::value;
            half_pass(xtag, jtag, ptag, mtag, std::true_type{});
            sw[0][sj].y = xinv_bitsel64(seam_lanes, sw[0][sj].x, sw[0][sj].y);
        }
    };

    int g = 0;
#pragma unroll
    for (; g < LAG * PW; g++) {
        if (PW > 0 && g == LAG * PW - 1) {
#pragma unroll
            for (int q = 0; q < NP; q++) {
                sw[q][0] = ring[PW - 1][(2 * PW) % XINV_PIPE_NS][q * RS][lane];
                if (FR) cw[q].v[FQ][0] = ring[PW - 1][(2 * PW) % XINV_PIPE_NS][q * RS + 1][lane];
            }
        }
        if ((g + 1) % B == 0) xinv_pipe_barrier();
    }

    for (int rb_ = in_lo; rb_ <= in_hi; rb_ += R) {
        xinv_unroll_steps([&](auto utag) {
            constexpr int U = decltype(utag)::value;
            constexpr int X = (U & 1) ? 0 : 1;
#define SLOT(w) ((U - (w) + 4 * R) % R)
#define RSLOT(w) ((2 * PW + U - (w) + 64 * XINV_PIPE_NS) % XINV_PIPE_NS)
#define ITAG(v) std::integral_constant<int, (v)>{}
            const int r = rb_ + U;
            request(r + PF, ITAG((U + PF) % R));
            request_rf(r + PFR, ITAG((U + PFR) % R));
            if (PW > 0) {
#pragma unroll
                for (int q = 0; q < NP; q++) {
                    sw[q][(U + 1) % R] = ring[PW - 1][RSLOT(-1)][q * RS][lane];
                    if (FR) cw[q].v[FQ][(U + 1) % R] = ring[PW - 1][RSLOT(-1)][q * RS + 1][lane];
                }
            }
            if constexpr (!HOIST) {
                const bool rv = (r - 1 >= 1) && (r - 1 <= ycr - 2);
#pragma unroll
                for (int q = 0; q < NP; q++)
                    M::template derive<UM, R, false>(cw[q], SLOT(0), SLOT(1), rv && lc[q].ok_x, rv && lc[q].ok_y, a.sc_);
            }
            {
                const int ja = r - 1;
                constexpr int sj = SLOT(1), sjp = SLOT(0), sjm = SLOT(2);
                if (EXT) {
                    if (ja == 1 || ja == ycr - 2) {
                        const double wl = xinv_lane_up(sw[NP - 1][sj].y);
#pragma unroll
                        for (int q = 0; q < NP; q++) {
                            const double iw = (q == 0) ? wl : sw[q > 0 ? q - 1 : 0][sj].y;
                            if (ja == 1) pipe_extend_fix(sw[q][sjm], sw[q][sj], iw, lc[q], a.tall, u);
                            if (ja == ycr - 2) pipe_extend_fix(sw[q][sjp], sw[q][sj], iw, lc[q], a.tall, u);
                        }
                    }
                }
                half_sweep(ITAG(X), ITAG(sj), ITAG(sjp), ITAG(sjm));
            }
            {
                const int jb = r - 2;
                constexpr int sj = SLOT(2), sjp = SLOT(1), sjm = SLOT(3);
                half_sweep(ITAG(X), ITAG(sj), ITAG(sjp), ITAG(sjm));
                if ((unsigned)(jb - yu0) < (unsigned)(yu1 - yu0)) {
#pragma unroll
                    for (int q = 0; q < NP; q++) {
                        const double2 t = sw[q][sj];
                        xinv_norm_row(nsx[q], nsy[q], nnx[q], nny[q], t.x, t.y, u);
                    }
                }
                if (PW < P - 1) {
#pragma unroll
                    for (int q = 0; q < NP; q++) {
                        ring[PW][RSLOT(2)][q * RS][lane] = sw[q][sj];
                        if (FR) ring[PW][RSLOT(2)][q * RS + 1][lane] = cw[q].v[FQ][sj];
                    }
                } else if ((unsigned)(jb - yu0) < (unsigned)(yu1 - yu0)) {
                    const int doff = jb * (int)rowbytes;
                    xinv_unroll_steps([&](auto qtag) {
                        constexpr int q = decltype(qtag)::value;
                        const double2 t = sw[q][sj];
                        typedef unsigned xinv_v4u __attribute__((__vector_size__(16)));
                        typedef unsigned xinv_v2u __attribute__((__vector_size__(8)));
                        if (AL) {
                            const xinv_v4u tv = {(unsigned)__double2loint(t.x), (unsigned)__double2hiint(t.x),
                                                 (unsigned)__double2loint(t.y), (unsigned)__double2hiint(t.y)};
                            __builtin_amdgcn_raw_buffer_store_b128(tv, rsD, (int)so0[q], doff, 0);
                        } else {
                            const xinv_v2u tx = {(unsigned)__double2loint(t.x), (unsigned)__double2hiint(t.x)};
                            const xinv_v2u ty = {(unsigned)__double2loint(t.y), (unsigned)__double2hiint(t.y)};
                            __builtin_amdgcn_raw_buffer_store_b64(tx, rsD, (int)so0[q], doff, 0);
                            __builtin_amdgcn_raw_buffer_store_b64(ty, rsD, (int)so1[q], doff, 0);
                        }
                    }, std::make_integer_sequence<int, NP>{});
                }
            }
            if ((LAG * PW + U + 1) % B == 0) xinv_pipe_barrier();
#undef SLOT
#undef RSLOT
#undef ITAG
        }, std::make_integer_sequence<int, R>{});
        g += R;
    }
    for (; g < gtot; g++) if ((g + 1) % B == 0) xinv_pipe_barrier();
#pragma unroll
    for (int q = 0; q < NP; q++) {
        acc += (lc[q].use_x ? nsx[q] : 0.0);
        acc += (lc[q].use_y ? nsy[q] : 0.0);
        cnt += (lc[q].use_x ? nnx[q] : 0) + (lc[q].use_y ? nny[q] : 0);
    }
}

template <class M, unsigned UM, bool FR, int NP, bool AL, bool EXT, bool SEAM = false>
__global__ __launch_bounds__(64 * XINV_PIPE_P) void k_pipe2d(FusedArgs a_)
{
    xinv_fresh_scalar_cache();
    constexpr int P = XINV_PIPE_P, K = P, H = 2 * K, LAG = XINV_PIPE_LAG, B = XINV_PIPE_B;
    __shared__ double2 ring[P - 1][XINV_PIPE_NS][NP * (FR ? 2 : 1)][XINV_WAVE];

    unsigned tag;
    int T;
    double acc = 0.0;
    int cnt = 0;
    const int wave = threadIdx.x >> 6, lane = threadIdx.x & 63;
    int pwi;
    {
    const FusedArgs &a = a_;
    const int64_t m = a.member0 + blockIdx.y;
    XinvCtl *ctl = a.ctl + m;
    if (!a.force && xinv_ctl_done(ctl)) return;
    if (a.lag && (int)blockIdx.x == a.nwg) { xinv_lag_reduce_prev(a, ctl, m); return; }
    tag = a.lag ? a.tag : xinv_ctl_seq(ctl);

    const int NB = a.nwg;
    {
        const int L = blockIdx.x, q = NB >> 3, rem = NB & 7, xcd = L & 7, idx = L >> 3;
        T = xcd * q + (xcd < rem ? xcd : rem) + idx;
    }
    pwi = (wave + (int)(blockIdx.x >> 8)) & (P - 1);
    int wt = T;
    bool active = wt < a.nstrip * a.nrb;
    if constexpr (SEAM) {
        if (!a.tile_list && NB == a.nstrip * a.nrb)
            wt = xinv_seam_tile(xinv_heavy_first((int)blockIdx.x, NB, (a.nstrip == 1 ? 1 : 2) * a.nrb), a.nstrip, a.nrb);
    }
    if (a.tile_list) {
        wt = a.tile_list[m * a.ntl + T];
        active = wt >= 0;
        wt = active ? wt : 0;
    }
    int rb = wt / a.nstrip, strip = wt - rb * a.nstrip;
    const int64_t xc = a.xc, yc = a.yc;
    int yu0, yu1;
    if (a.RY > 0) {
        yu0 = rb * a.RY;
        yu1 = (yu0 + a.RY < (int)yc) ? yu0 + a.RY : (int)yc;
    } else {
        yu0 = (int)((((int64_t)rb * yc) / a.nrb) & ~(int64_t)1);
        yu1 = (rb + 1 == a.nrb) ? (int)yc : (int)((((int64_t)(rb + 1) * yc) / a.nrb) & ~(int64_t)1);
    }
    const int UW = SEAM ? xinv_ring_uw(xc, H) : XINV_PIPE_UW(NP), HW = SEAM ? xinv_ring_hw(xc, H, strip) : H;
    const int64_t xu0 = (int64_t)strip * UW;
    LaneCols lc[NP];
    int64_t st0[NP];
    RingSeam rs = {0ull, false};
#pragma unroll
    for (int q = 0; q < NP; q++) {
        if constexpr (SEAM) lc[q] = make_lanecols_ring(xu0, HW, UW, lane, xc, rs);
        else lc[q] = make_lanecols<AL>(xu0, H, UW, lane, xc, a.per != 0, NP, q);
        st0[q] = xu0 - HW + 2 * NP * lane + 2 * q;
    }

    if (active) {
        const int ry = yu1 - yu0;
        int gtot = 0;
#pragma unroll
        for (int pw = 0; pw < P; pw++) {
            const int per = (pw == 0 ? XINV_PIPE_PF0 : XINV_PIPE_PF) + 4;
            const int n = ry + 2 * H - 4 * pw;
            const int g = LAG * pw + ((n + per - 1) / per) * per;
            gtot = g > gtot ? g : gtot;
        }
        gtot = ((gtot + B - 1) / B) * B;
        const bool wraps = rs.any;
#define XINV_PIPE_MARCH(SM) \
        switch (pwi) { \
        case 0: xinv_pipe_wave<M, UM, FR, NP, AL, EXT, 0, XINV_PIPE_PF0, SM>(a, m, yu0, yu1, lc, st0, lane, ring, gtot, acc, cnt, rs.lanes); break; \
        case 1: xinv_pipe_wave<M, UM, FR, NP, AL, EXT, 1, XINV_PIPE_PF, SM>(a, m, yu0, yu1, lc, st0, lane, ring, gtot, acc, cnt, rs.lanes); break; \
        case 2: xinv_pipe_wave<M, UM, FR, NP, AL, EXT, 2, XINV_PIPE_PF, SM>(a, m, yu0, yu1, lc, st0, lane, ring, gtot, acc, cnt, rs.lanes); break; \
        default: xinv_pipe_wave<M, UM, FR, NP, AL, EXT, 3, XINV_PIPE_PF, SM>(a, m, yu0, yu1, lc, st0, lane, ring, gtot, acc, cnt, rs.lanes); break; \
        }
        if (wraps) { XINV_PIPE_MARCH(SEAM) } else { XINV_PIPE_MARCH(false) }
#undef XINV_PIPE_MARCH
    }
    }
    const FusedArgs __attribute__((address_space(4))) *kp =
        (const FusedArgs __attribute__((address_space(4))) *)__builtin_amdgcn_kernarg_segment_ptr();
    asm volatile("" : "+s"(kp) :: "memory");
    if (kp->no_ctl) return;
    const int64_t m = kp->member0 + blockIdx.y;
    XinvCtl *ctl = kp->ctl + m;
    const int NB = kp->nwg;
    struct { unsigned long long *psum; const double *xsum; const long long *xcnt; int lag; XinvStop stop; const void *hook; } a;
    a.psum = kp->psum; a.xsum = kp->xsum; a.xcnt = kp->xcnt; a.lag = kp->lag;
    a.hook = XINV_TEST_HOOKS ? (const void *)kp->dbg : nullptr;
    a.stop.mxLoop = kp->stop.mxLoop; a.stop.tolerance = kp->stop.tolerance;
    a.stop.stop_on_zero_norm = kp->stop.stop_on_zero_norm;

    {
        unsigned long long *pw = a.psum + (size_t)m * XINV_KMAX * NB * XINV_PW;
        const double ws = xinv_wave_sum(acc);
        const long long wc = xinv_wave_sum_ll((long long)cnt);
        if (lane == 0 && !xinv_hook_withhold(a.hook, T, tag, m)) {
            const unsigned long long hi = (unsigned long long)tag << 32;
            const unsigned long long bits = (unsigned long long)__double_as_longlong(ws);
            unsigned long long *q = pw + ((size_t)pwi * NB + T) * XINV_PW;
            __hip_atomic_store(q + 0, hi | (bits & 0xffffffffull), __ATOMIC_RELAXED, __HIP_MEMORY_SCOPE_AGENT);
            __hip_atomic_store(q + 1, hi | (bits >> 32), __ATOMIC_RELAXED, __HIP_MEMORY_SCOPE_AGENT);
            __hip_atomic_store(q + 2, hi | (unsigned long long)(unsigned)wc, __ATOMIC_RELAXED,
                               __HIP_MEMORY_SCOPE_AGENT);
        }
        if (a.lag || blockIdx.x != gridDim.x - 1) return;
        __syncthreads();
        xinv_norm_reduce<K, P>(wave, lane, NB, tag, pw, ctl, a.stop, a.xsum ? a.xsum[m] : 0.0,
                               a.xcnt ? a.xcnt[m] : 0);
    }
}
```

xinvert_amd/csrc/xinv_plan.h:

```cpp
#pragma once


template <class F>
static int flag_pass(Workspace *ws, hipStream_t st, int *flag, F issue)
{
    HIPCHK(hipMemsetAsync(ws->dflag, 0, sizeof(int), st));
    issue();
    HIPCHK(hipMemcpyAsync(ws->hflag, ws->dflag, sizeof(int), hipMemcpyDeviceToHost, st));
    HIPCHK(hipStreamSynchronize(st));
    *flag = *ws->hflag;
    return XINV_OK;
}

static int any_nonzero(const Problem &p, Workspace *ws, hipStream_t st, std::initializer_list<int> arrays, int *nonzero)
{
    const int64_t n = p.zc * p.yc * p.xc;
    return flag_pass(ws, st, nonzero, [&] {
        for (int q : arrays) {
            const int64_t nb = (p.sc[q] == 0) ? n : (p.nbatch - 1) * p.sc[q] + n;
            hipLaunchKernelGGL(k_any_nonzero, dim3(1024), dim3(256), 0, st, p.c[q], nb, ws->dflag);
        }
    });
}

// ... 81 lines not shown
        const int n = streams ? 1 : std::min(occ, 3);
        const int64_t cap = 256 * (int64_t)n;
        const int64_t rounds = cdiv(wgs, cap);
        const int64_t w_last = wgs - (rounds - 1) * cap;
        const double cost = ((double)(rounds - 1) * wg_cost((double)n) + wg_cost((double)w_last / 256.0)) * (double)(RB + 11 + 8);
        if (cost < best) { best = cost; bestRB = RB; }
    }
    pl.RY = bestRB;
    pl.nrb = (int)cdiv(p.yc, bestRB);
    pl.nsg = (int)cdiv((int64_t)nstrip * pl.nrb, 4) + 1;
    if (!(opt.flags & XINV_FLAG_NO_TILE_SKIP)) {
        rc = plan_tile_skip(p, pl, ws, st, opt, bestRB, XINV_BIH_OWN(p.BCx == XINV_BC_PERIODIC));
        if (rc) return rc;
    }
    return XINV_OK;
}

static int plan_fused9(const Problem &p, const xinv_options &opt, Workspace *ws, hipStream_t st, Plan &pl)
{
    pl.um = pl.umask = 0;
    const int k9max = (p.kind == KIND_STD2D) ? 3 : 2;
    const int k9def = 2;
    pl.K = opt.sweeps_per_launch > 0 ? std::min(opt.sweeps_per_launch, k9max) : k9def;
    pl.aligned = !(p.xc & 1) && vec_aligned(p.S, p.sS);
    for (int q = 0; q < p.ncoef; q++) pl.aligned = pl.aligned && vec_aligned(p.c[q], p.sc[q]);
    if (!rows_per_tile_given(p, opt, pl)) {
        const int occ = plan_occ(p, pl, st, pl.K);
        pl.lone = 1.0;
        split_rows_evenly(p, pl, choose_row_blocks(p.yc, cdiv(p.xc, strip9_uw(pl, pl.K)), p.nbatch, pl.K, occ, pl.lone, false));
    }
    pl.nsg = (int)cdiv((int64_t)cdiv(p.xc, strip9_uw(pl, XINV_KMAX)) * pl.nrb, 4) + 1;
    if (pl.even_split && !(opt.flags & XINV_FLAG_NO_TILE_SKIP))
        return plan_tile_skip(p, pl, ws, st, opt, 0, strip9_uw(pl, pl.K));
    return XINV_OK;
}

static int plan_fused3d(const Problem &p, const xinv_options &opt, Workspace *ws, hipStream_t st, Plan &pl)
{
    int rc = XINV_OK;
    pl.K = 1;
    pl.RY = (opt.rows_per_tile == 8 || opt.rows_per_tile == 12 || opt.rows_per_tile == 16)
                ? opt.rows_per_tile : 0;
    pl.nsg = (int)cdiv(p.xc, pl.seam ? xinv_ring_uw(p.xc, 2) : 124);
    pl.aligned = !(p.xc & 1) && vec_aligned(p.S, p.sS) && vec_aligned(p.c[p.ncoef - 1], p.sc[p.ncoef - 1]);
    if (p.kind == KIND_STD3D) {
        for (int q = 0; q < 3; q++) pl.aligned = pl.aligned && vec_aligned(p.c[q], p.sc[q]);
        pl.umask = 0;
        if (!(opt.flags & XINV_FLAG_NO_XUNIFORM)) {
            const int idx3[3] = {0, 1, 2};
            rc = detect_xuniform_of(p, ws, st, idx3, 3, p.zc * p.yc, &pl.umask);
            if (rc) return rc;
        }
        pl.um = (pl.umask == 7u) ? 7u : 0u;
        const bool nw16_ok = (pl.um == 7u && p.BCy != XINV_BC_EXTEND);
        const bool nw16 = nw16_ok && !pl.seam;
        if (pl.RY == 0) pl.RY = nw16 ? 16 : 12;
        if (pl.RY == 16 && !nw16) pl.RY = 12;
    } else {
        pl.um = pl.umask;
        if (pl.RY == 0 || pl.RY == 16) pl.RY = 12;
    }
    pl.nrb = (int)cdiv(p.yc, pl.RY - 4);
    pl.nkc = xinv_k_chunks_fused3d(p.zc, (int64_t)pl.nsg * pl.nrb * p.nbatch);
    pl.KC = (int)xinv_k_chunk_planes(p.zc, pl.nkc);
    pl.K2 = false;
    const int k2_auto = XINV_ENV_INT("XINV_3D_K2", 1);
    const bool ext3 = (p.BCy == XINV_BC_EXTEND);
    if (p.kind == KIND_STD3D && pl.um == 7u && !(ext3 && (pl.seam || pl.fma || p3_extend_joff(p.yc) < 0)) && !(pl.seam && (pl.fma || p.xc < 64)) &&
        (opt.sweeps_per_launch == 2 || (opt.sweeps_per_launch == 0 && k2_auto)) &&
        opt.rows_per_tile == 0 && p.stop.mxLoop >= 1 &&
        p.zc * p.yc * 64 < ((int64_t)1 << 31) &&
        p.zc * p.yc * p.xc * 8 < ((int64_t)1 << 31)) {
        pl.K2 = true;
        pl.K = 2;
        pl.nsg2 = (int)cdiv(p.xc, pl.seam ? xinv_ring_uw(p.xc, 4) : 120);
        pl.joff2 = ext3 ? p3_extend_joff(p.yc) : 0;
        pl.nrb2 = (int)cdiv(p.yc + pl.joff2, XINV_P3_G * XINV_P3_RR - 8);
        {
            const bool shared = (p.sc[0] == 0 && p.sc[1] == 0 && p.sc[2] == 0);
            const int64_t tab = p.zc * p.yc * 8;
            rc = ensure_dev(&ws->d_rowf, &ws->d_rowf_cap, (size_t)(shared ? 1 : p.nbatch) * tab * sizeof(double));
            if (rc) return rc;
            RowFactor3Args ra;
            memset(&ra, 0, sizeof ra);
            for (int q = 0; q < 3; q++) { ra.c[q] = p.c[q]; ra.sc[q] = p.sc[q]; }
            ra.zc = p.zc; ra.yc = p.yc; ra.xc = p.xc; ra.sc_ = p.sc_;
            ra.rowf = (double *)ws->d_rowf; ra.srowf = shared ? 0 : tab;
            pl.srowf2 = ra.srowf;
            hipLaunchKernelGGL(k_row_factor3d, dim3((unsigned)cdiv(p.zc * p.yc, 256), (unsigned)(shared ? 1 : p.nbatch), 1),
                               dim3(256), 0, st, ra);
        }
        pl.nkc2 = xinv_k_chunks_pipe3d(p.zc, (int64_t)pl.nsg2 * pl.nrb2 * p.nbatch, pl.cus);
        pl.KC2 = (int)xinv_k_chunk_planes(p.zc, pl.nkc2);
    }
    return XINV_OK;
}

static int plan5_xuniform(const Problem &p, const xinv_options &opt, Workspace *ws, hipStream_t st, Plan &pl)
{
    const StreamMap &sm = stream_map(p.kind);
    pl.umask = 0;
    ws->act_ready = false;
    if (!(opt.flags & XINV_FLAG_NO_XUNIFORM)) {
        if (p.kind != KIND_STD2DT && opt.rows_per_tile == 0 && opt.sweeps_per_launch == 0 &&
            !(opt.flags & (XINV_FLAG_NO_TILE_SKIP | XINV_FLAG_NO_PIPE)) && p.nbatch <= 64 &&
            p.nbatch * p.yc * p.xc >= (int64_t)2000000) {
            const int uw_pipe = pl.seam ? xinv_ring_uw(p.xc, 2 * XINV_PIPE_P) : XINV_PIPE_UW(1);
            if (p.xc >= uw_pipe && p.nbatch * cdiv(p.xc, uw_pipe) * (p.yc + 1) <= (int64_t)50000000) {
                const int rc = issue_strip_active(p, ws, st, uw_pipe, sm.c[sm.forcing]);
                if (rc) return rc;
            }
        }
        const int rc = detect_xuniform_of(p, ws, st, sm.c, sm.nuni, p.yc, &pl.umask);
        if (rc) return rc;
    }
    pl.um = pick_um(p.kind, pl.umask);
    return XINV_OK;
}

static int plan5_sweeps(const Problem &p, const xinv_options &opt, Workspace *, hipStream_t st, Plan &pl)
{
    if (opt.sweeps_per_launch > XINV_KMAX) return fail_arg("sweeps_per_launch must be 1 to 4");
    const StreamMap &sm = stream_map(p.kind);
    pl.aligned = !(p.xc & 1) && vec_aligned(p.S, p.sS);
    for (int q = 0; q < sm.n; q++) pl.aligned = pl.aligned && vec_aligned(p.c[sm.c[q]], p.sc[sm.c[q]]);
    const int nvec = 1 + sm.n - __builtin_popcount(pl.um & ((1u << sm.n) - 1u));
    pl.lone = nvec <= 2 ? 1.6 : (nvec == 3 ? 1.3 : 1.0);
    const int pipe_mode = XINV_ENV_INT("XINV_PIPE", 1);
    const bool pipe_form = (p.kind == KIND_STD2D && pl.um == 3u) || (p.kind == KIND_GEN2D && pl.um == 0x1fu);
    const bool pipe_size_ok = pipe_mode != 3 || p.kind == KIND_GEN2D || p.nbatch * p.yc * p.xc <= (int64_t)10000000;
    const bool pipe_want = pipe_mode != 0 && pipe_form && pipe_size_ok && !(opt.flags & XINV_FLAG_NO_PIPE) &&
                           (opt.sweeps_per_launch == 0 || opt.sweeps_per_launch == XINV_PIPE_P) &&
                           (p.yc + 16) * p.xc * 8 < ((int64_t)1 << 31);
    const bool hoisted_gen = (p.kind == KIND_GEN2D && nvec <= 2);
    const int ksup = (p.kind == KIND_STD2D && nvec <= 2) ? XINV_KMAX : (hoisted_gen ? 2 : 3);
    const int occ_needed = nvec >= 4 ? 1 : 2;
    if (pipe_want)
        pl.K = XINV_PIPE_P;
    else if (opt.sweeps_per_launch > 0)
        pl.K = std::min(opt.sweeps_per_launch, (p.kind == KIND_STD2D) ? XINV_KMAX : 3);
    else {
        pl.K = 2;
        for (int k = ksup; k > 2; k--) {
            bool have = false;
            if (plan_occ(p, pl, st, k, &have) >= occ_needed && have) { pl.K = k; break; }
        }
    }
    pl.pipe = pipe_want && pl.K == XINV_PIPE_P;
    pl.tpw = pl.pipe ? 1 : 4;
    pl.npair = 1;
    const int fr_env = opt.pipe_fr ? (opt.pipe_fr > 0 ? 1 : 0) : XINV_ENV_INT("XINV_PIPE_FR", -1);
    const bool fr_size = (double)p.nbatch * (double)p.yc * (double)p.xc * 24.0 > 2.0e8;
    pl.pipe_fr = pl.pipe && pipe_form && pl.npair == 1 && (fr_env < 0 ? fr_size : fr_env != 0);
    return XINV_OK;
}

static int plan5_point_factor(const Problem &p, const xinv_options &opt, Workspace *ws, hipStream_t st, Plan &pl)
{
    pl.pq = p.kind == KIND_GEN2D && (pl.um == 0x1cu || pl.um == 0u) && !pl.pipe && !pl.seam && !pl.fma &&
            !(opt.flags & XINV_FLAG_NO_POINT_FACTOR) && p.sc_.optArg != 0.0;
    if (!pl.pq) return XINV_OK;
    int rc = ensure_dev(&ws->d_pfac, &ws->d_pfac_cap, (size_t)p.nbatch * p.yc * p.xc * sizeof(double));
    if (rc) return rc;
    const StreamMap &sm = stream_map(p.kind);
    PointFactorArgs fa;
    memset(&fa, 0, sizeof fa);
    for (int q = 0; q < sm.n; q++) { fa.c[q] = p.c[sm.c[q]]; fa.sc[q] = p.sc[sm.c[q]]; }
    fa.yc = p.yc; fa.xc = p.xc; fa.n = p.yc * p.xc; fa.sc_ = p.sc_; fa.q = ws->d_pfac; fa.flag = ws->dflag;
    int flag = 0;
    rc = flag_pass(ws, st, &flag, [&] {
        hipLaunchKernelGGL(k_point_factor, dim3((unsigned)std::min<int64_t>(2048, cdiv(fa.n, 256)), (unsigned)p.nbatch, 1),
                           dim3(256), 0, st, fa);
    });
    if (rc) return rc;
    if (flag & 1) pl.pq = false;
    pl.alias_ac = pl.pq && !(flag & 2);
    return XINV_OK;
}

static int plan5_row_records(const Problem &p, const xinv_options &, Workspace *ws, hipStream_t st, Plan &pl)
{
    if (!pl.pipe) return XINV_OK;
    const StreamMap &sm = stream_map(p.kind);
    const bool gen = (p.kind == KIND_GEN2D);
    const bool hoist = gen ? ((pl.um & 0x13u) == 0x13u) : ((pl.um & 3u) == 3u);
    const int nw = __builtin_popcount(pl.um & ((1u << sm.nuni) - 1u)) + (hoist ? 2 : 0);
    const int rw = nw == 0 ? 0 : (nw <= 4 ? 4 : 8);
    if (!rw) return XINV_OK;
    const int rc = ensure_dev(&ws->d_rowf, &ws->d_rowf_cap, (size_t)p.nbatch * p.yc * rw * sizeof(double));
    if (rc) return rc;
    RowFactorArgs ra;
    memset(&ra, 0, sizeof ra);
    for (int q = 0; q < sm.nuni; q++) { ra.c[q] = p.c[sm.c[q]]; ra.sc[q] = p.sc[sm.c[q]]; }
    ra.gen = gen ? 1 : 0; ra.um = pl.um; ra.hoist = hoist ? 1 : 0; ra.rw = rw;
    ra.yc = p.yc; ra.xc = p.xc; ra.sc_ = p.sc_; ra.rowf = (double *)ws->d_rowf;
    hipLaunchKernelGGL(k_row_factor, dim3(cdiv(p.yc, 256), (unsigned)p.nbatch, 1), dim3(256), 0, st, ra);
    return XINV_OK;
}

static int plan5_row_split(const Problem &p, const xinv_options &opt, Workspace *, hipStream_t st, Plan &pl)
{
    if (rows_per_tile_given(p, opt, pl)) return XINV_OK;
    const int occ = plan_occ(p, pl, st, pl.K);
    split_rows_evenly(p, pl, choose_row_blocks(p.yc, cdiv(p.xc, strip_uw(pl, pl.K, pl.pipe)), p.nbatch, pl.K, occ, pl.lone, pl.pipe));
    return XINV_OK;
}

static int plan5_partials(const Problem &p, const xinv_options &, Workspace *, hipStream_t, Plan &pl)
{
    pl.nsg = (int)cdiv((int64_t)cdiv(p.xc, strip_uw(pl, XINV_KMAX, false)) * pl.nrb, 4) + 1;
    if (pl.pipe) pl.nsg = std::max(pl.nsg, (int)cdiv(p.xc, strip_uw(pl, pl.K, true)) * pl.nrb + 1);
    return XINV_OK;
}

static int plan_fused5(const Problem &p, const xinv_options &opt, Workspace *ws, hipStream_t st, Plan &pl)
{
    for (auto step : {plan5_xuniform, plan5_sweeps, plan5_point_factor, plan5_row_records, plan5_row_split, plan5_partials}) {
        const int rc = step(p, opt, ws, st, pl);
        if (rc) return rc;
    }
    if (pl.even_split && !(opt.flags & XINV_FLAG_NO_TILE_SKIP)) return plan_tile_skip(p, pl, ws, st, opt);
    return XINV_OK;
}

static int plan_path(const Problem &p, const xinv_options &opt, Workspace *ws, hipStream_t st, Plan &pl)
{
    ws->act_ready = false;
    int rc = XINV_OK;
    const bool seam5_ok = !pl.seam || p.xc >= 64;
    const bool fused5_ok = pl.base == 2 && seam5_ok && p.kind != KIND_BIH2D && p.kind != KIND_GEN3D;
    const bool fused9_ok = pl.base == 4 && seam5_ok && p.c[1] &&
                           (p.kind == KIND_STD2D || p.kind == KIND_GEN2D);
    bool fusedbih_ok = false;
    if (p.kind == KIND_BIH2D) {
        pl.umask = 0;
        if (!(opt.flags & XINV_FLAG_NO_XUNIFORM)) {
            const int idx10[10] = {0, 1, 2, 3, 4, 5, 6, 7, 8, 9};
            rc = detect_xuniform_of(p, ws, st, idx10, 10, p.yc, &pl.umask);
            if (rc) return rc;
        }
        pl.um = pl.umask;
        fusedbih_ok = (p.BCx != XINV_BC_PERIODIC || p.xc % 3 == 0) && !(opt.flags & XINV_FLAG_NO_XUNIFORM) &&
                      p.sc_.optArg != 0.0;
    }
    bool fused3g_ok = false;
    if (p.kind == KIND_GEN3D && seam5_ok && opt.path != XINV_PATH_COLOUR && !(opt.flags & XINV_FLAG_NO_XUNIFORM)) {
        const int idx7[7] = {0, 1, 2, 3, 4, 5, 6};
        rc = detect_xuniform_of(p, ws, st, idx7, 7, p.zc * p.yc, &pl.umask);
        if (rc) return rc;
        fused3g_ok = (pl.umask == 0x7fu);
    }
    const bool fused_ok = fused5_ok || fused9_ok || fused3g_ok || fusedbih_ok;
    pl.path = XINV_PATH_COLOUR;
    pl.nine = false;
    if (fused_ok && opt.path != XINV_PATH_COLOUR) { pl.path = XINV_PATH_FUSED; pl.nine = fused9_ok && !fused5_ok; }
    if (opt.path == XINV_PATH_FUSED && !fused_ok)
        return fail_arg("no fused kernel for this form (odd-xc periodic seam with xc < 64; 9-point test form; biharmonic with periodic x and xc % 3 != 0; general 3-D with coefficients that vary along x)");
    if (pl.path == XINV_PATH_COLOUR && !is3d(p.kind) && !p.c[1] && pl.base == 4)
        return fail_arg("internal: 9-point form without B");

    if (pl.path != XINV_PATH_FUSED) return XINV_OK;
    if (p.kind == KIND_BIH2D) return plan_fusedbih(p, opt, ws, st, pl);
    if (pl.nine) return plan_fused9(p, opt, ws, st, pl);
    if (is3d(p.kind)) return plan_fused3d(p, opt, ws, st, pl);
    return plan_fused5(p, opt, ws, st, pl);
}
```

xinvert_amd/csrc/xinv_tiles.h:

```cpp
#pragma once
#include <cstdint>
#ifndef __HIPCC__
#ifndef __host__
#define __host__
#endif
#ifndef __device__
#define __device__
#endif
#endif

struct TileRows { int strip; int64_t y0, y1; };
__host__ __device__ inline TileRows xinv_tile_rows(int wt, int nstrip, int nrb, int64_t yc, int RY)
{
    TileRows t;
    const int rb = wt / nstrip;
    t.strip = wt - rb * nstrip;
    if (RY > 0) { t.y0 = (int64_t)rb * RY; t.y1 = (t.y0 + RY < yc) ? t.y0 + RY : yc; }
    else {
        t.y0 = (((int64_t)rb * yc) / nrb) & ~(int64_t)1;
        t.y1 = (rb + 1 == nrb) ? yc : ((((int64_t)(rb + 1) * yc) / nrb) & ~(int64_t)1);
    }
    return t;
}

__host__ __device__ inline int xinv_heavy_first(int L, int n, int nh)
{
    const int hq = (nh < n ? nh : n) >> 3, xcd = L & 7, idx = L >> 3;
    if (idx < hq) return idx * 8 + xcd;
    const int nr = n - 8 * hq, q = nr >> 3, rem = nr & 7;
    return 8 * hq + xcd * q + (xcd < rem ? xcd : rem) + (idx - hq);
}
__host__ __device__ inline int xinv_seam_tile(int s, int nstrip, int nrb)
{
    const int edges = nstrip == 1 ? 1 : 2, nh = edges * nrb;
    if (s < nh) {
        const int e = s / nrb, rb = s - e * nrb;
        return rb * nstrip + (e == 0 ? nstrip - 1 : 0);
    }
    const int k = s - nh, nl = nstrip > edges ? nstrip - edges : 1, rb = k / nl;
    return rb * nstrip + (k - rb * nl) + 1;
}

__host__ __device__ inline bool xinv_ring_asym(int64_t xc, int H) { return xc >= (int64_t)(128 - 2 * H - 2) + H; }
__host__ __device__ inline int xinv_ring_uw(int64_t xc, int H) { return 128 - 2 * H - (xinv_ring_asym(xc, H) ? 2 : 4); }
__host__ __device__ inline int xinv_ring_hw(int64_t xc, int H, int strip)
{
    return xinv_ring_asym(xc, H) ? (strip == 0 ? H + 2 : H) : H + 2;
}

__host__ __device__ inline int xinv_p3_slot_tile(int L, int nfull, int nkc, int &kc)
{
    int g;
    kc = 0;
    if (L < nfull) g = L;
    else { const int q = L - nfull; g = nfull + q / nkc; kc = q - (g - nfull) * nkc; }
    return g;
}
__host__ __device__ inline bool xinv_p3_slot_reduces(int L, int nfull, int nkc, int NT, int ml)
{
    const int gl = (ml + 1) * NT - 1;
    return (gl < nfull) ? (L == gl) : (L == nfull + (gl - nfull) * nkc + nkc - 1);
}
__host__ __device__ inline int xinv_p3_slot_member_tile(int L, int nfull, int NT, int ml, int g)
{
    if (L < nfull) {
        const int L0 = ml * NT;
        const int n = (L0 + NT <= nfull) ? NT : (nfull - L0);
        const int xcd = L & 7;
        auto below = [](int e, int x) { return (e >> 3) * x + ((e & 7) < x ? (e & 7) : x); };
        auto same = [](int e, int x) { return e <= x ? 0 : ((e - x + 7) >> 3); };
        return (below(L0 + n, xcd) - below(L0, xcd)) + (same(L, xcd) - same(L0, xcd));
    }
    return g - ml * NT;
}
struct P3Slot { int ml, Tj, kc; bool whole, reducer; };
__host__ __device__ inline P3Slot xinv_p3_slot(int L, int nfull, int nkc, int NT)
{
    P3Slot s;
    s.whole = L < nfull;
    const int g = xinv_p3_slot_tile(L, nfull, nkc, s.kc);
    s.ml = g / NT;
    s.reducer = xinv_p3_slot_reduces(L, nfull, nkc, NT, s.ml);
    s.Tj = xinv_p3_slot_member_tile(L, nfull, NT, s.ml, g);
    return s;
}

__host__ inline int64_t xinv_p3_whole_tiles(int64_t tiles, int nk, int64_t KC, int64_t zc, int cus_, double *cost_out = nullptr)
{
    const bool no_rem = cus_ < 0;
    const int64_t cus = cus_ < 0 ? -cus_ : cus_;
    auto cdiv64 = [](int64_t a, int64_t b) { return (a + b - 1) / b; };
    const double cf = (double)(zc + 4), cs = (double)(KC + 14);
    double best = (double)cdiv64(tiles, cus) * cf;
    int64_t nfull = tiles;
    if (nk > 1) {
        const double call = (double)cdiv64(tiles * nk, cus) * cs;
        if (call < best * 0.97) { best = call; nfull = 0; }
        const int64_t r = tiles % cus, R = tiles / cus;
        if (r && R && !no_rem) {
            const double crem = (double)R * cf + (double)cdiv64(r * nk, cus) * cs;
            if (crem < best * 0.985) { best = crem; nfull = tiles - r; }
        }
    }
    if (cost_out) *cost_out = best;
    return nfull;
}

__host__ __device__ inline bool xinv_p3_extend_ok(int64_t yc, int joff, int RJ, int H, int RR)
{
    if ((H + joff) % RR == RR - 1) return false;
    const int64_t jbo = (yc - 1 + joff) / RJ;
    auto together = [&](int64_t jb) { return ((yc - 2) - (jb * RJ - H - joff)) % RR != RR - 1; };
    if (!together(jbo)) return false;
    if (jbo > 0 && (yc - 1 + joff) - jbo * RJ <= 1 && !together(jbo - 1)) return false;
    return true;
}
__host__ __device__ inline int xinv_p3_extend_joff(int64_t yc, int RJ, int H, int RR)
{
    return xinv_p3_extend_ok(yc, 0, RJ, H, RR) ? 0 : (xinv_p3_extend_ok(yc, 2, RJ, H, RR) ? 2 : -1);
}

__host__ inline int64_t xinv_cdiv(int64_t a, int64_t b) { return (a + b - 1) / b; }

__host__ inline double xinv_tile_cost(int64_t wgs, int64_t rows, int K, int occ, int occ_cap, double lone, int pipe_lag)
{
    const bool pipe = pipe_lag > 0;
    occ = occ < occ_cap ? occ : occ_cap;
    occ = occ > 1 ? occ : 1;
    const int64_t cap = 256 * (int64_t)occ, period = pipe ? 4 : 2 * K + 2;
    const int64_t steps = pipe ? xinv_cdiv(rows + 1 + 4 + 3 * pipe_lag, 8) * 8
                               : xinv_cdiv(rows + 1 + 4 * K, period) * period;
    const int64_t r = xinv_cdiv(wgs, cap), rounds = r > 1 ? r : 1;
    const int64_t w_last = wgs - (rounds - 1) * cap;
    const double full = pipe ? 1.5 + occ : ((occ == 1) ? lone : (double)occ);
    const double last = pipe ? 1.5 + (double)xinv_cdiv(w_last, 256) : ((w_last <= 256) ? lone : (double)xinv_cdiv(w_last, 256));
    return ((double)(rounds - 1) * full + last) * (double)steps;
}

__host__ inline int64_t xinv_choose_row_blocks(int64_t yc, int64_t nstrip, int64_t nbatch, int K, int occ, int occ_cap,
                                               double lone, int pipe_lag)
{
    const bool pipe = pipe_lag > 0;
    int64_t best = 1; double best_cost = 1e300;
    const int64_t n0 = xinv_cdiv(yc, pipe ? 512 : 128), nmin = n0 > 1 ? n0 : 1, nmax = nmin > yc / 4 ? nmin : yc / 4;
    for (int64_t nr = nmin; nr <= nmax; nr++) {
        const int64_t wgs = xinv_cdiv(nstrip * nr, pipe ? 1 : 4) * nbatch;
        const double cost = xinv_tile_cost(wgs, xinv_cdiv(yc, nr), K, occ, occ_cap, lone, pipe_lag);
        if (cost <= best_cost * 1.0001) { best_cost = cost < best_cost ? cost : best_cost; best = nr; }
    }
    return best;
}

__host__ inline int64_t xinv_k_chunk_planes(int64_t zc, int nk) { return xinv_cdiv(xinv_cdiv(zc, nk), 4) * 4; }
template <class Cost>
__host__ inline int xinv_choose_k_chunks(int64_t zc, Cost cost)
{
    int best = 1; double best_cost = 1e300;
    for (int nk = 1; nk <= 16; nk++) {
        const int64_t KC = xinv_k_chunk_planes(zc, nk);
        if (nk > 1 && (KC < 16 || (int64_t)(nk - 1) * KC >= zc)) break;
        const double c = cost(nk, KC);
        if (c < best_cost * 0.97) { best_cost = c; best = nk; }
    }
    return best;
}
__host__ inline int xinv_k_chunks_fused3d(int64_t zc, int64_t wgs)
{
    return xinv_choose_k_chunks(zc, [&](int nk, int64_t KC) { return (double)xinv_cdiv(wgs * nk, 256) * (double)(KC + (nk > 1 ? 10 : 2)); });
}
__host__ inline int xinv_k_chunks_pipe3d(int64_t zc, int64_t tiles, int cus)
{
    return xinv_choose_k_chunks(zc, [&](int nk, int64_t KC) { double c; xinv_p3_whole_tiles(tiles, nk, KC, zc, cus, &c); return c; });
}
```

xinvert_amd/csrc/xinv_tu_pipe2d.hip:

```cpp
#include "xinv_dispatch.h"

#ifndef XINV_TU_SEAM
#define XINV_TU_SEAM 0
#endif
constexpr bool SEAM = XINV_TU_SEAM != 0;

template <class M, unsigned UM, bool FR, int NP, bool AL, bool EXT>
static int pipe_one(dim3 grid, hipStream_t st, const FusedArgs &a, int *occ, int lds_pad)
{
    if (occ) {
        static int cached = 0;
        int n = cached;
        if (!n) {
            if (hipOccupancyMaxActiveBlocksPerMultiprocessor(&n, k_pipe2d<M, UM, FR, NP, AL, EXT, SEAM>, 64 * XINV_PIPE_P, 0) != hipSuccess)
                n = 1;
            cached = n = n < 1 ? 1 : n;
        }
        *occ = n;
        return 0;
    }
    hipLaunchKernelGGL((k_pipe2d<M, UM, FR, NP, AL, EXT, SEAM>), grid, dim3(64 * XINV_PIPE_P, 1, 1), (size_t)lds_pad, st, a);
    return 0;
}

template <class M, unsigned UM, bool FR, int NP>
static int pipe_np(bool al, bool ext, dim3 grid, hipStream_t st, const FusedArgs &a, int *occ, int lds_pad)
{
    if constexpr (!SEAM) {
        if (al) return ext ? pipe_one<M, UM, FR, NP, true, true>(grid, st, a, occ, lds_pad) : pipe_one<M, UM, FR, NP, true, false>(grid, st, a, occ, lds_pad);
    } else if (al) return 1;
    return ext ? pipe_one<M, UM, FR, NP, false, true>(grid, st, a, occ, lds_pad) : pipe_one<M, UM, FR, NP, false, false>(grid, st, a, occ, lds_pad);
}

#if XINV_TU_SEAM
#define xinv_launch_pipe2d_std xinv_launch_pipe2d_std_seam
#define xinv_launch_pipe2d_gen xinv_launch_pipe2d_gen_seam
#endif
#if XINV_TU_MODEL == 2
int xinv_launch_pipe2d_fma(bool gen, unsigned um, bool fr, bool al, bool ext, dim3 grid, hipStream_t st, const FusedArgs &a, int *occ, int lds_pad)
{
    if (!gen && um == 3u) return fr ? pipe_np<FusedStd2DF, 3u, true, 1>(al, ext, grid, st, a, occ, lds_pad)
                                    : pipe_np<FusedStd2DF, 3u, false, 1>(al, ext, grid, st, a, occ, lds_pad);
    if (gen && um == 0x1fu) return fr ? pipe_np<FusedGen2DF, 0x1fu, true, 1>(al, ext, grid, st, a, occ, lds_pad)
                                      : pipe_np<FusedGen2DF, 0x1fu, false, 1>(al, ext, grid, st, a, occ, lds_pad);
    return 1;
}
#elif XINV_TU_MODEL == 0
int xinv_launch_pipe2d_std(unsigned um, int np, bool fr, bool al, bool ext, dim3 grid, hipStream_t st, const FusedArgs &a, int *occ, int lds_pad)
{
    if (um == 3u && np == 1) return fr ? pipe_np<FusedStd2D, 3u, true, 1>(al, ext, grid, st, a, occ, lds_pad)
                                       : pipe_np<FusedStd2D, 3u, false, 1>(al, ext, grid, st, a, occ, lds_pad);
    return 1;
}
#else
int xinv_launch_pipe2d_gen(unsigned um, int np, bool fr, bool al, bool ext, dim3 grid, hipStream_t st, const FusedArgs &a, int *occ, int lds_pad)
{
    (void)np;
    if (um == 0x1fu) return fr ? pipe_np<FusedGen2D, 0x1fu, true, 1>(al, ext, grid, st, a, occ, lds_pad)
                               : pipe_np<FusedGen2D, 0x1fu, false, 1>(al, ext, grid, st, a, occ, lds_pad);
    return 1;
}
#endif
```

Before: 737.2 billion.

## Precompute per-row lane masks for pipelined 2D SOR to replace per-point predicates

Adds a preparation kernel that builds, for each row and strip, 64-bit wave lane masks combining the undefined-value test with the row-valid word. The pipelined 2D kernel gains an LM variant that loads these masks as scalar (constant address space) words and applies updates and norm accumulation under EXEC masks, using s_bcnt for counts. This is meant to remove per-point forcing comparisons and the per-row rok record load from the inner loop. In exchange it adds a padded mask buffer, an extra prep pass and more template instantiations, and a flag is added to disable it.

```diff
diff --git a/include/xinv.h b/include/xinv.h
--- a/include/xinv.h
+++ b/include/xinv.h
@@ -31,6 +31,8 @@
 #define XINV_FLAG_NO_PIPE 16
 
 #define XINV_FLAG_NO_POINT_FACTOR 64
+
+#define XINV_FLAG_NO_LANE_MASKS 128
 
 #define XINV_MAX_DEVICES 16
 
diff --git a/xinvert_amd/_lib.py b/xinvert_amd/_lib.py
--- a/xinvert_amd/_lib.py
+++ b/xinvert_amd/_lib.py
@@ -146,14 +146,15 @@
 def options(device=-1, path=PATH_AUTO, sweeps_per_launch=0, check_every=0, rows_per_tile=0,
             timing=0, no_xuniform=0, no_tile_skip=0, force_tile_skip=0, rowconst_mask=0,
             host_chunk=0, devices=None, prep=None, pin_host=0, no_pipe=0, fma=0, f32_mask=0,
-            lanes=0, norm_lag=0, pipe_fr=0, graph=0, no_point_factor=0, cu_count=0, host_inflight=0):
+            lanes=0, norm_lag=0, pipe_fr=0, graph=0, no_point_factor=0, cu_count=0, host_inflight=0,
+            no_lane_masks=0):
     o = XinvOptions()
     load().xinv_default_options(ctypes.byref(o))
     o.device, o.path, o.sweeps_per_launch = device, path, sweeps_per_launch
     o.check_every, o.rows_per_tile, o.timing = check_every, rows_per_tile, timing
     o.flags = (1 if no_xuniform else 0) | (2 if no_tile_skip else 0) | (4 if force_tile_skip else 0) | \
               (8 if pin_host else 0) | (16 if no_pipe else 0) | (32 if fma else 0) | \
-              (64 if no_point_factor else 0)
+              (64 if no_point_factor else 0) | (128 if no_lane_masks else 0)
     o.rowconst_mask = int(rowconst_mask)
     o.host_chunk = int(host_chunk)
     o.f32_mask = int(f32_mask)
diff --git a/xinvert_amd/csrc/xinv_device.h b/xinvert_amd/csrc/xinv_device.h
--- a/xinvert_amd/csrc/xinv_device.h
+++ b/xinvert_amd/csrc/xinv_device.h
@@ -158,6 +158,26 @@
         "v_cmpx_neq_f64_e32 vcc, %7, %5\n\tv_add_f64 %0, %0, |%5|\n\tv_add_u32 %2, %2, 1\n\ts_mov_b64 exec, %4\n\t"
         "v_cmpx_neq_f64_e32 vcc, %7, %6\n\tv_add_f64 %1, %1, |%6|\n\tv_add_u32 %3, %3, 1\n\ts_mov_b64 exec, %4"
         : "+v"(sx), "+v"(sy), "+v"(nx), "+v"(ny), "=&s"(sv) : "v"(x), "v"(y), "s"(u) : "vcc");
+}
+
+__device__ __forceinline__ double xinv_fma_where(double a, double t, double rq, unsigned long long mask)
+{
+    unsigned long long sv;
+    asm("s_and_saveexec_b64 %1, %4\n\tv_fma_f64 %0, %2, %3, %0\n\ts_mov_b64 exec, %1"
+        : "+v"(a), "=&s"(sv) : "v"(t), "s"(rq), "s"(mask) : "scc");
+    return a;
+}
+__device__ __forceinline__ void xinv_norm_row_owned(double &sx, double &sy, int &n, double x, double y, double u,
+                                                    unsigned long long ownx, unsigned long long owny)
+{
+    unsigned long long sv;
+    int t;
+    asm("s_and_saveexec_b64 %3, %8\n\t"
+        "v_cmpx_neq_f64_e32 vcc, %7, %5\n\tv_add_f64 %0, %0, |%5|\n\ts_bcnt1_i32_b64 %4, exec\n\ts_add_i32 %2, %2, %4\n\t"
+        "s_and_b64 exec, %3, %9\n\t"
+        "v_cmpx_neq_f64_e32 vcc, %7, %6\n\tv_add_f64 %1, %1, |%6|\n\ts_bcnt1_i32_b64 %4, exec\n\ts_add_i32 %2, %2, %4\n\t"
+        "s_mov_b64 exec, %3"
+        : "+v"(sx), "+v"(sy), "+s"(n), "=&s"(sv), "=&s"(t) : "v"(x), "v"(y), "s"(u), "s"(ownx), "s"(owny) : "vcc", "scc");
 }
 
 struct XinvScal {
diff --git a/xinvert_amd/csrc/xinv_dispatch.h b/xinvert_amd/csrc/xinv_dispatch.h
--- a/xinvert_amd/csrc/xinv_dispatch.h
+++ b/xinvert_amd/csrc/xinv_dispatch.h
@@ -28,23 +28,23 @@
 XINV_HIDDEN int xinv_launch_fused2d_genq(bool al, bool ext, unsigned um, int K, dim3 grid, dim3 block,
                                          hipStream_t st, const FusedArgs &a, int *occ);
 XINV_HIDDEN int xinv_launch_pipe2d_fma(bool gen, unsigned um, bool fr, bool al, bool ext, dim3 grid, hipStream_t st,
-                                       const FusedArgs &a, int *occ, int lds_pad);
+                                       const FusedArgs &a, int *occ, int lds_pad, bool lm);
 XINV_HIDDEN int xinv_launch_pipe2d_std(unsigned um, int np, bool fr, bool al, bool ext, dim3 grid, hipStream_t st,
-                                       const FusedArgs &a, int *occ, int lds_pad);
+                                       const FusedArgs &a, int *occ, int lds_pad, bool lm);
 XINV_HIDDEN int xinv_launch_pipe2d_gen(unsigned um, int np, bool fr, bool al, bool ext, dim3 grid, hipStream_t st,
-                                       const FusedArgs &a, int *occ, int lds_pad);
+                                       const FusedArgs &a, int *occ, int lds_pad, bool lm);
 XINV_HIDDEN int xinv_launch_pipe2d_std_seam(unsigned um, int np, bool fr, bool al, bool ext, dim3 grid, hipStream_t st,
-                                            const FusedArgs &a, int *occ, int lds_pad);
+                                            const FusedArgs &a, int *occ, int lds_pad, bool lm);
 XINV_HIDDEN int xinv_launch_pipe2d_gen_seam(unsigned um, int np, bool fr, bool al, bool ext, dim3 grid, hipStream_t st,
-                                            const FusedArgs &a, int *occ, int lds_pad);
+                                            const FusedArgs &a, int *occ, int lds_pad, bool lm);
 static inline int xinv_launch_pipe2d(bool gen, unsigned um, int np, bool fr, bool al, bool ext, dim3 grid, hipStream_t st,
-                                     const FusedArgs &a, int *occ, int lds_pad = 0, bool seam = false, bool fma = false)
+                                     const FusedArgs &a, int *occ, int lds_pad = 0, bool seam = false, bool fma = false, bool lm = false)
 {
-    if (fma) return (seam || np != 1) ? 1 : xinv_launch_pipe2d_fma(gen, um, fr, al, ext, grid, st, a, occ, lds_pad);
-    if (seam) return gen ? xinv_launch_pipe2d_gen_seam(um, np, fr, al, ext, grid, st, a, occ, lds_pad)
-                         : xinv_launch_pipe2d_std_seam(um, np, fr, al, ext, grid, st, a, occ, lds_pad);
-    return gen ? xinv_launch_pipe2d_gen(um, np, fr, al, ext, grid, st, a, occ, lds_pad)
-               : xinv_launch_pipe2d_std(um, np, fr, al, ext, grid, st, a, occ, lds_pad);
+    if (fma) return (seam || np != 1) ? 1 : xinv_launch_pipe2d_fma(gen, um, fr, al, ext, grid, st, a, occ, lds_pad, lm);
+    if (seam) return gen ? xinv_launch_pipe2d_gen_seam(um, np, fr, al, ext, grid, st, a, occ, lds_pad, lm)
+                         : xinv_launch_pipe2d_std_seam(um, np, fr, al, ext, grid, st, a, occ, lds_pad, lm);
+    return gen ? xinv_launch_pipe2d_gen(um, np, fr, al, ext, grid, st, a, occ, lds_pad, lm)
+               : xinv_launch_pipe2d_std(um, np, fr, al, ext, grid, st, a, occ, lds_pad, lm);
 }
 XINV_HIDDEN int xinv_launch_fused9(bool gen, int K, bool al, bool ext, dim3 grid, hipStream_t st,
                                    const FusedArgs &a, int *occ, bool seam = false);
diff --git a/xinvert_amd/csrc/xinv_fused.h b/xinvert_amd/csrc/xinv_fused.h
--- a/xinvert_amd/csrc/xinv_fused.h
+++ b/xinvert_amd/csrc/xinv_fused.h
@@ -53,6 +53,7 @@
     const double *xsum;
     const long long *xcnt;
     const void *rowf;
+    const void *lmask;
     double *dbg;
 };
 
@@ -427,13 +428,6 @@
 
 template <int NC> struct RowPack { double2 s; double2 c[NC]; double cs[NC]; };
 
-struct LaneCols {
-    int64_t l0, l1;
-    bool ok_x, ok_y;
-    bool use_x, use_y;
-    int cls_x, cls_y;
-};
-
 template <bool AL>
 __device__ __forceinline__ double2 ld2(const double *p, int64_t row_off, const LaneCols &lc)
 {
@@ -441,49 +435,12 @@
     double2 v; v.x = p[row_off + lc.l0]; v.y = p[row_off + lc.l1]; return v;
 }
 
-template <bool AL>
-__device__ __forceinline__ LaneCols make_lanecols(int64_t xu0, int H, int UW, int lane, int64_t xc,
-                                                  bool per, int np = 1, int q = 0)
-{
-    LaneCols lc;
-    const int64_t c0 = xu0 - H + 2 * np * lane + 2 * q, c1 = c0 + 1;
-    if (per) {
-        int64_t w0 = c0 % xc; if (w0 < 0) w0 += xc;
-        int64_t w1 = c1 % xc; if (w1 < 0) w1 += xc;
-        lc.l0 = w0; lc.l1 = w1;
-        lc.ok_x = lc.ok_y = true;
-        lc.cls_x = lc.cls_y = 1;
-    } else {
-        if (AL) {
-            int64_t p = c0 < 0 ? 0 : (c0 > xc - 2 ? xc - 2 : c0);
-            lc.l0 = p; lc.l1 = p + 1;
-        } else {
-            lc.l0 = c0 < 0 ? 0 : (c0 > xc - 1 ? xc - 1 : c0);
-            lc.l1 = c1 < 0 ? 0 : (c1 > xc - 1 ? xc - 1 : c1);
-        }
-        lc.ok_x = (c0 >= 1 && c0 <= xc - 2);
-        lc.ok_y = (c1 >= 1 && c1 <= xc - 2);
-        lc.cls_x = lc.ok_x ? 1 : (c0 == 0 ? 2 : (c0 == xc - 1 ? 3 : 0));
-        lc.cls_y = lc.ok_y ? 1 : (c1 == xc - 1 ? 3 : 0);
-    }
-    lc.use_x = (c0 >= xu0 && c0 < xu0 + UW && c0 < xc);
-    lc.use_y = (c1 >= xu0 && c1 < xu0 + UW && c1 < xc);
-    return lc;
-}
-
 struct RingSeam { unsigned long long lanes; bool any; };
 __device__ __forceinline__ LaneCols make_lanecols_ring(int64_t xu0, int HW, int UW, int lane, int64_t xc, RingSeam &rs)
 {
-    LaneCols lc;
-    const int64_t c0 = xu0 - HW + 2 * lane, c1 = c0 + 1, xv = xc + 1;
-    int64_t w0 = c0 % xv; if (w0 < 0) w0 += xv;
-    int64_t w1 = c1 % xv; if (w1 < 0) w1 += xv;
-    lc.l0 = w0; lc.l1 = (w1 == xc) ? xc - 1 : w1;
-    lc.ok_x = true; lc.ok_y = (w1 != xc);
-    lc.cls_x = lc.cls_y = 1;
-    lc.use_x = (c0 >= xu0 && c0 < xu0 + UW && c0 < xc);
-    lc.use_y = (c1 >= xu0 && c1 < xu0 + UW && c1 < xc);
-    rs.lanes = __builtin_amdgcn_ballot_w64(w0 == xc - 1);
+    bool seam_lane;
+    const LaneCols lc = make_lanecols_ring_lane(xu0, HW, UW, lane, xc, seam_lane);
+    rs.lanes = __builtin_amdgcn_ballot_w64(seam_lane);
     rs.any = rs.lanes != 0ull;
     return lc;
 }
diff --git a/xinvert_amd/csrc/xinv_launch.h b/xinvert_amd/csrc/xinv_launch.h
--- a/xinvert_amd/csrc/xinv_launch.h
+++ b/xinvert_amd/csrc/xinv_launch.h
@@ -32,6 +32,8 @@
     int tpw;
     int npair;
     bool pipe_fr;
+    bool lmask;
+    size_t lm_off;
     int64_t xc;
     bool fma;
     bool alias_ac;
@@ -191,7 +193,7 @@
         a.c[sm.forcing + 1] = a.c[sm.forcing]; a.sc[sm.forcing + 1] = a.sc[sm.forcing];
         a.c[sm.forcing] = (const double *)ws->d_pfac; a.sc[sm.forcing] = p.yc * p.xc;
     }
-    if (pipe) { a.nwg = a.nstrip * a.nrb; a.rowf = ws->d_rowf; }
+    if (pipe) { a.nwg = a.nstrip * a.nrb; a.rowf = ws->d_rowf; a.lmask = pl.lmask ? (const char *)ws->d_rowf + pl.lm_off : nullptr; }
 #if XINV_TEST_HOOKS
     a.dbg = (double *)t_hook_record;
 #endif
@@ -202,7 +204,7 @@
         dim3 grid((unsigned)a.nwg + (lag_tag ? 1u : 0u), (unsigned)nm, 1), block(256, 1, 1);
         if (pipe) {
             const int pad = std::max(0, XINV_ENV_INT("XINV_PIPE_LDSPAD", 0));
-            xinv_launch_pipe2d(p.kind == KIND_GEN2D, pl.um, pl.npair, pl.pipe_fr, pl.aligned, a.ext != 0, grid, st, a, nullptr, pad, pl.seam != 0, pl.fma);
+            xinv_launch_pipe2d(p.kind == KIND_GEN2D, pl.um, pl.npair, pl.pipe_fr, pl.aligned, a.ext != 0, grid, st, a, nullptr, pad, pl.seam != 0, pl.fma, pl.lmask);
             return XINV_OK;
         }
         if (fused_dispatch(p.kind, pl.aligned, a.ext != 0, pl.um | (pl.alias_ac ? 2u : 0u), K, grid, block, st, a, nullptr, pl.seam != 0, pl.fma, pl.pq))
@@ -481,7 +483,7 @@
         FusedArgs dummy; memset(&dummy, 0, sizeof dummy);
         occ = pl.nine ? 1 : 2;
         if (pl.nine) missing = xinv_launch_fused9(p.kind == KIND_GEN2D, K, pl.aligned, ext, dim3(1), st, dummy, &occ, pl.seam != 0);
-        else if (pl.pipe) missing = xinv_launch_pipe2d(p.kind == KIND_GEN2D, pl.um, pl.npair, pl.pipe_fr, pl.aligned, ext, dim3(1), st, dummy, &occ, 0, pl.seam != 0, pl.fma);
+        else if (pl.pipe) missing = xinv_launch_pipe2d(p.kind == KIND_GEN2D, pl.um, pl.npair, pl.pipe_fr, pl.aligned, ext, dim3(1), st, dummy, &occ, 0, pl.seam != 0, pl.fma, pl.lmask);
         else missing = fused_dispatch(p.kind, pl.aligned, ext, pl.um | (pl.alias_ac ? 2u : 0u), K, dim3(1), dim3(256), st, dummy, &occ, pl.seam != 0, pl.fma, pl.pq);
     }
     if (have) *have = !missing;
diff --git a/xinvert_amd/csrc/xinv_pipe2d.h b/xinvert_amd/csrc/xinv_pipe2d.h
--- a/xinvert_amd/csrc/xinv_pipe2d.h
+++ b/xinvert_amd/csrc/xinv_pipe2d.h
@@ -68,6 +68,47 @@
         f[k++] = rq; f[k++] = rok;
     }
     for (; k < a.rw; k++) f[k] = 0.0;
+}
+#endif
+
+#define XINV_LM_PAD 24
+struct LaneMaskArgs {
+    const double *f;
+    int64_t sf;
+    const double *rowf;
+    int rw, irok;
+    int64_t yc, xc;
+    int nstrip, UW, H;
+    int per, seam, al, np;
+    double undef;
+    unsigned long long *lm;
+};
+
+#ifdef XINV_AUX_KERNELS
+__global__ __launch_bounds__(256) void k_lane_masks(LaneMaskArgs a)
+{
+    const int wave = threadIdx.x >> 6, lane = threadIdx.x & 63;
+    const int64_t cell = (int64_t)blockIdx.x * 4 + wave, m = blockIdx.y;
+    if (cell >= a.yc * a.nstrip) return;
+    const int64_t row = cell / a.nstrip;
+    const int strip = (int)(cell - row * a.nstrip);
+    const double *frow = a.f + m * a.sf + row * a.xc;
+    const unsigned long long rok =
+        (unsigned long long)__double_as_longlong(a.rowf[(m * a.yc + row) * a.rw + a.irok]);
+    const int64_t xu0 = (int64_t)strip * a.UW;
+    {
+        const int q = 0;
+        LaneCols lc;
+        if (a.seam) { bool sl; lc = make_lanecols_ring_lane(xu0, xinv_ring_hw(a.xc, a.H, strip), a.UW, lane, a.xc, sl); }
+        else if (a.al) lc = make_lanecols<true>(xu0, a.H, a.UW, lane, a.xc, a.per != 0, a.np, q);
+        else lc = make_lanecols<false>(xu0, a.H, a.UW, lane, a.xc, a.per != 0, a.np, q);
+        const unsigned long long mx = __builtin_amdgcn_ballot_w64(xinv_lane_pred(lc, 0, frow, a.undef)) & rok;
+        const unsigned long long my = __builtin_amdgcn_ballot_w64(xinv_lane_pred(lc, 1, frow, a.undef)) & rok;
+        if (lane == 0) {
+            unsigned long long *o = a.lm + (((m * a.nstrip + strip) * (a.yc + 2 * XINV_LM_PAD) + XINV_LM_PAD + row) << 1);
+            o[0] = (row & 1) ? my : mx; o[1] = (row & 1) ? mx : my;
+        }
+    }
 }
 #endif
 
@@ -134,12 +175,12 @@
     }
 }
 
-template <class M, unsigned UM, bool FR, int NP, bool AL, bool EXT, int PW, int PF, bool SEAM = false>
+template <class M, unsigned UM, bool FR, int NP, bool AL, bool EXT, int PW, int PF, bool SEAM = false, bool LM = false>
 __device__ __forceinline__ void xinv_pipe_wave(const FusedArgs &a, int64_t m, int yu0, int yu1,
                                                const LaneCols (&lc)[NP], const int64_t (&st0)[NP], int lane,
                                                double2 (*ring)[XINV_PIPE_NS][NP * (FR ? 2 : 1)][XINV_WAVE], int gtot,
                                                double &acc, int &cnt,
-                                               unsigned long long seam_lanes = 0ull)
+                                               unsigned long long seam_lanes = 0ull, const void *lmrow = nullptr)
 {
     constexpr int P = XINV_PIPE_P, H = 2 * P, D = 4, LAG = XINV_PIPE_LAG, B = XINV_PIPE_B;
     constexpr int R = PF + D;
@@ -179,6 +220,21 @@
     }
     static_assert(!SEAM || (NP == 1 && !AL && PipeRec<M, UM>::HOIST),
                   "seam variants: one column pair per lane, per-row records, updates under EXEC masks");
+    static_assert(!LM || PipeRec<M, UM>::HOIST, "lane-mask records: the variants whose row predicate is a record word");
+    typedef const unsigned long long __attribute__((address_space(4))) *xinv_cull_ptr;
+    const xinv_cull_ptr lmp = (xinv_cull_ptr)(uintptr_t)lmrow;
+    static_assert(!LM || NP == 1, "lane-mask records: one column pair per lane");
+    static_assert(XINV_LM_PAD >= 2 * XINV_PIPE_P + PF + 4 + 2, "the zero rows cover every row a tile marches outside the slice");
+    unsigned long long ownx64[NP], owny64[NP];
+    unsigned long long mblk[PF + 4], mred[PF + 4];
+    int scnt = 0;
+#pragma unroll
+    for (int q = 0; q < NP; q++) {
+        ownx64[q] = __builtin_amdgcn_ballot_w64(lc[q].use_x);
+        owny64[q] = AL ? ownx64[q] : __builtin_amdgcn_ballot_w64(lc[q].use_y);
+    }
+#pragma unroll
+    for (int t = 0; t < PF + 4; t++) mblk[t] = mred[t] = 0ull;
 
     const int in_lo = yu0 - H + 2 * PW;
     const int in_hi = yu1 - 1 + H - 2 * PW;
@@ -243,16 +299,27 @@
 #pragma unroll
                 for (int c = 0; c < NC - 1; c++)
                     if ((UM >> c) & 1u) cw[q].s[c][slot] = rec[k++];
-                if (HOIST) { cw[q].rq[slot] = rec[k]; rokw[slot] = rec[k + 1]; }
-            }
+                if (HOIST) { cw[q].rq[slot] = rec[k]; if (!LM) rokw[slot] = rec[k + 1]; }
+            }
+        }
+    };
+    int nxm = ((yu0 - H + 2 * PW + XINV_LM_PAD) * 2 - 3) * 8;
+    auto request_lm = [&](auto stag) {
+        constexpr int slot = decltype(stag)::value;
+        if constexpr (LM) {
+            const xinv_cull_ptr pm = (xinv_cull_ptr)((const char __attribute__((address_space(4))) *)lmp + nxm);
+            nxm += 16;
+            asm("" : "+s"(nxm));
+            mblk[slot] = pm[0]; mred[slot] = pm[1];
         }
     };
     xinv_unroll_steps([&](auto ttag) { request(in_lo + decltype(ttag)::value, ttag); asm volatile("" ::: "memory"); },
                       std::make_integer_sequence<int, PF>{});
     xinv_unroll_steps([&](auto ttag) { request_rf(in_lo + decltype(ttag)::value, ttag); },
                       std::make_integer_sequence<int, PFR>{});
-
-    auto half_pass = [&](auto xtag, auto jtag, auto ptag, auto mtag, auto fixt) {
+    request_lm(std::integral_constant<int, 0>{});
+
+    auto half_pass = [&](auto xtag, auto jtag, auto ptag, auto mtag, auto fixt, unsigned long long lm) {
         constexpr int X = decltype(xtag)::value, sj = decltype(jtag)::value, sjp = decltype(ptag)::value,
                       sjm = decltype(mtag)::value;
         constexpr bool FIX = decltype(fixt)::value;
@@ -267,7 +334,14 @@
             if constexpr (FIX) e = xinv_lane_down(sw[q][sj].x);
             const double t = M::template inc<X, UM, R, false>(cw[q], sj, sjp, comp<X>(sw[q][sj]), comp<X>(sw[q][sjp]),
                                               comp<X>(sw[q][sjm]), w, e, a.sc_);
-            if constexpr (HOIST) {
+            if constexpr (LM) {
+                unsigned long long rm = lm;
+                if constexpr (SEAM) { if (X == 0) rm &= FIX ? seam_lanes : ~seam_lanes; }
+                if constexpr (ModelFma<M>::value)
+                    nv[q] = xinv_fma_where(comp<X>(sw[q][sj]), t, cw[q].rq[sj], rm);
+                else
+                    nv[q] = xinv_add_where(comp<X>(sw[q][sj]), t, rm);
+            } else if constexpr (HOIST) {
                 const unsigned long long rm = (FIX ? seam_lanes : (X ? oky64[q] : okx64[q])) &
                                               (unsigned long long)__double_as_longlong(rokw[sj]);
                 if constexpr (ModelFma<M>::value)
@@ -282,12 +356,12 @@
 #pragma unroll
         for (int q = 0; q < NP; q++) setc<X>(sw[q][sj], nv[q]);
     };
-    auto half_sweep = [&](auto xtag, auto jtag, auto ptag, auto mtag) {
+    auto half_sweep = [&](auto xtag, auto jtag, auto ptag, auto mtag, unsigned long long lm) {
         constexpr int X = decltype(xtag)::value;
-        half_pass(xtag, jtag, ptag, mtag, std::false_type{});
+        half_pass(xtag, jtag, ptag, mtag, std::false_type{}, lm);
         if constexpr (SEAM && X == 0) {
             constexpr int sj = decltype(jtag)::value;
-            half_pass(xtag, jtag, ptag, mtag, std::true_type{});
+            half_pass(xtag, jtag, ptag, mtag, std::true_type{}, lm);
             sw[0][sj].y = xinv_bitsel64(seam_lanes, sw[0][sj].x, sw[0][sj].y);
         }
     };
@@ -315,6 +389,7 @@
             const int r = rb_ + U;
             request(r + PF, ITAG((U + PF) % R));
             request_rf(r + PFR, ITAG((U + PFR) % R));
+            request_lm(ITAG((U + 1) % R));
             if (PW > 0) {
 #pragma unroll
                 for (int q = 0; q < NP; q++) {
@@ -342,17 +417,18 @@
                         }
                     }
                 }
-                half_sweep(ITAG(X), ITAG(sj), ITAG(sjp), ITAG(sjm));
+                half_sweep(ITAG(X), ITAG(sj), ITAG(sjp), ITAG(sjm), mred[U]);
             }
             {
                 const int jb = r - 2;
                 constexpr int sj = SLOT(2), sjp = SLOT(1), sjm = SLOT(3);
-                half_sweep(ITAG(X), ITAG(sj), ITAG(sjp), ITAG(sjm));
+                half_sweep(ITAG(X), ITAG(sj), ITAG(sjp), ITAG(sjm), mblk[U]);
                 if ((unsigned)(jb - yu0) < (unsigned)(yu1 - yu0)) {
 #pragma unroll
                     for (int q = 0; q < NP; q++) {
                         const double2 t = sw[q][sj];
-                        xinv_norm_row(nsx[q], nsy[q], nnx[q], nny[q], t.x, t.y, u);
+                        if constexpr (LM) xinv_norm_row_owned(nsx[q], nsy[q], scnt, t.x, t.y, u, ownx64[q], owny64[q]);
+                        else xinv_norm_row(nsx[q], nsy[q], nnx[q], nny[q], t.x, t.y, u);
                     }
                 }
                 if (PW < P - 1) {
@@ -395,9 +471,10 @@
         acc += (lc[q].use_y ? nsy[q] : 0.0);
         cnt += (lc[q].use_x ? nnx[q] : 0) + (lc[q].use_y ? nny[q] : 0);
     }
-}
-
-template <class M, unsigned UM, bool FR, int NP, bool AL, bool EXT, bool SEAM = false>
+    if (LM) cnt += (lane == 0) ? scnt : 0;
+}
+
+template <class M, unsigned UM, bool FR, int NP, bool AL, bool EXT, bool SEAM = false, bool LM = false>
 __global__ __launch_bounds__(64 * XINV_PIPE_P) void k_pipe2d(FusedArgs a_)
 {
     xinv_fresh_scalar_cache();
@@ -469,12 +546,13 @@
         }
         gtot = ((gtot + B - 1) / B) * B;
         const bool wraps = rs.any;
+        const void *lmrow = LM ? (const void *)((const char *)a.lmask + ((m * a.nstrip + strip) * (yc + 2 * XINV_LM_PAD)) * 16) : nullptr;
 #define XINV_PIPE_MARCH(SM) \
         switch (pwi) { \
-        case 0: xinv_pipe_wave<M, UM, FR, NP, AL, EXT, 0, XINV_PIPE_PF0, SM>(a, m, yu0, yu1, lc, st0, lane, ring, gtot, acc, cnt, rs.lanes); break; \
-        case 1: xinv_pipe_wave<M, UM, FR, NP, AL, EXT, 1, XINV_PIPE_PF, SM>(a, m, yu0, yu1, lc, st0, lane, ring, gtot, acc, cnt, rs.lanes); break; \
-        case 2: xinv_pipe_wave<M, UM, FR, NP, AL, EXT, 2, XINV_PIPE_PF, SM>(a, m, yu0, yu1, lc, st0, lane, ring, gtot, acc, cnt, rs.lanes); break; \
-        default: xinv_pipe_wave<M, UM, FR, NP, AL, EXT, 3, XINV_PIPE_PF, SM>(a, m, yu0, yu1, lc, st0, lane, ring, gtot, acc, cnt, rs.lanes); break; \
+        case 0: xinv_pipe_wave<M, UM, FR, NP, AL, EXT, 0, XINV_PIPE_PF0, SM, LM>(a, m, yu0, yu1, lc, st0, lane, ring, gtot, acc, cnt, rs.lanes, lmrow); break; \
+        case 1: xinv_pipe_wave<M, UM, FR, NP, AL, EXT, 1, XINV_PIPE_PF, SM, LM>(a, m, yu0, yu1, lc, st0, lane, ring, gtot, acc, cnt, rs.lanes, lmrow); break; \
+        case 2: xinv_pipe_wave<M, UM, FR, NP, AL, EXT, 2, XINV_PIPE_PF, SM, LM>(a, m, yu0, yu1, lc, st0, lane, ring, gtot, acc, cnt, rs.lanes, lmrow); break; \
+        default: xinv_pipe_wave<M, UM, FR, NP, AL, EXT, 3, XINV_PIPE_PF, SM, LM>(a, m, yu0, yu1, lc, st0, lane, ring, gtot, acc, cnt, rs.lanes, lmrow); break; \
         }
         if (wraps) { XINV_PIPE_MARCH(SEAM) } else { XINV_PIPE_MARCH(false) }
 #undef XINV_PIPE_MARCH
diff --git a/xinvert_amd/csrc/xinv_plan.h b/xinvert_amd/csrc/xinv_plan.h
--- a/xinvert_amd/csrc/xinv_plan.h
+++ b/xinvert_amd/csrc/xinv_plan.h
@@ -257,6 +257,7 @@
     const int fr_env = opt.pipe_fr ? (opt.pipe_fr > 0 ? 1 : 0) : XINV_ENV_INT("XINV_PIPE_FR", -1);
     const bool fr_size = (double)p.nbatch * (double)p.yc * (double)p.xc * 24.0 > 2.0e8;
     pl.pipe_fr = pl.pipe && pipe_form && pl.npair == 1 && (fr_env < 0 ? fr_size : fr_env != 0);
+    pl.lmask = pl.pipe && pipe_form && !(opt.flags & XINV_FLAG_NO_LANE_MASKS);
     return XINV_OK;
 }
 
@@ -292,7 +293,14 @@
     const int nw = __builtin_popcount(pl.um & ((1u << sm.nuni) - 1u)) + (hoist ? 2 : 0);
     const int rw = nw == 0 ? 0 : (nw <= 4 ? 4 : 8);
     if (!rw) return XINV_OK;
-    const int rc = ensure_dev(&ws->d_rowf, &ws->d_rowf_cap, (size_t)p.nbatch * p.yc * rw * sizeof(double));
+    pl.lmask = pl.lmask && hoist;
+    const int UW = strip_uw(pl, pl.K, true), nstrip = (int)cdiv(p.xc, UW);
+    const size_t rec_bytes = (((size_t)p.nbatch * p.yc * rw * sizeof(double)) + 63u) & ~(size_t)63u;
+    pl.lmask = pl.lmask && pl.npair == 1;
+    const size_t lm_rows = (size_t)nstrip * (size_t)(p.yc + 2 * XINV_LM_PAD);
+    const size_t lm_bytes = pl.lmask ? (size_t)p.nbatch * lm_rows * 16u : 0u;
+    pl.lm_off = rec_bytes;
+    const int rc = ensure_dev(&ws->d_rowf, &ws->d_rowf_cap, rec_bytes + lm_bytes);
     if (rc) return rc;
     RowFactorArgs ra;
     memset(&ra, 0, sizeof ra);
@@ -300,6 +308,22 @@
     ra.gen = gen ? 1 : 0; ra.um = pl.um; ra.hoist = hoist ? 1 : 0; ra.rw = rw;
     ra.yc = p.yc; ra.xc = p.xc; ra.sc_ = p.sc_; ra.rowf = (double *)ws->d_rowf;
     hipLaunchKernelGGL(k_row_factor, dim3(cdiv(p.yc, 256), (unsigned)p.nbatch, 1), dim3(256), 0, st, ra);
+    if (pl.lmask) {
+        LaneMaskArgs la;
+        memset(&la, 0, sizeof la);
+        la.f = p.c[sm.c[sm.forcing]]; la.sf = p.sc[sm.c[sm.forcing]];
+        la.rowf = (const double *)ws->d_rowf; la.rw = rw; la.irok = nw - 1;
+        la.yc = p.yc; la.xc = p.xc; la.nstrip = nstrip; la.UW = UW; la.H = 2 * XINV_PIPE_P;
+        la.per = (p.BCx == XINV_BC_PERIODIC); la.seam = pl.seam; la.al = pl.aligned; la.np = pl.npair;
+        la.undef = p.sc_.undef; la.lm = (unsigned long long *)((char *)ws->d_rowf + pl.lm_off);
+        HIPCHK(hipMemsetAsync(la.lm, 0, lm_bytes, st));
+        for_member_chunks(0, p.nbatch, [&](int64_t m0, int64_t nm) {
+            LaneMaskArgs lb = la;
+            lb.f += m0 * la.sf; lb.rowf += m0 * p.yc * rw; lb.lm += (size_t)m0 * lm_rows * 2;
+            hipLaunchKernelGGL(k_lane_masks, dim3(cdiv(p.yc * nstrip, 4), (unsigned)nm, 1), dim3(256), 0, st, lb);
+            return XINV_OK;
+        });
+    }
     return XINV_OK;
 }
 
diff --git a/xinvert_amd/csrc/xinv_tiles.h b/xinvert_amd/csrc/xinv_tiles.h
--- a/xinvert_amd/csrc/xinv_tiles.h
+++ b/xinvert_amd/csrc/xinv_tiles.h
@@ -46,6 +46,67 @@
 __host__ __device__ inline int xinv_ring_hw(int64_t xc, int H, int strip)
 {
     return xinv_ring_asym(xc, H) ? (strip == 0 ? H + 2 : H) : H + 2;
+}
+
+#ifdef __HIPCC__
+#define XINV_HD_INLINE __host__ __device__ __forceinline__
+#else
+#define XINV_HD_INLINE inline
+#endif
+struct LaneCols {
+    int64_t l0, l1;
+    bool ok_x, ok_y;
+    bool use_x, use_y;
+    int cls_x, cls_y;
+};
+
+template <bool AL>
+XINV_HD_INLINE LaneCols make_lanecols(int64_t xu0, int H, int UW, int lane, int64_t xc, bool per, int np = 1, int q = 0)
+{
+    LaneCols lc;
+    const int64_t c0 = xu0 - H + 2 * np * lane + 2 * q, c1 = c0 + 1;
+    if (per) {
+        int64_t w0 = c0 % xc; if (w0 < 0) w0 += xc;
+        int64_t w1 = c1 % xc; if (w1 < 0) w1 += xc;
+        lc.l0 = w0; lc.l1 = w1;
+        lc.ok_x = lc.ok_y = true;
+        lc.cls_x = lc.cls_y = 1;
+    } else {
+        if (AL) {
+            int64_t p = c0 < 0 ? 0 : (c0 > xc - 2 ? xc - 2 : c0);
+            lc.l0 = p; lc.l1 = p + 1;
+        } else {
+            lc.l0 = c0 < 0 ? 0 : (c0 > xc - 1 ? xc - 1 : c0);
+            lc.l1 = c1 < 0 ? 0 : (c1 > xc - 1 ? xc - 1 : c1);
+        }
+        lc.ok_x = (c0 >= 1 && c0 <= xc - 2);
+        lc.ok_y = (c1 >= 1 && c1 <= xc - 2);
+        lc.cls_x = lc.ok_x ? 1 : (c0 == 0 ? 2 : (c0 == xc - 1 ? 3 : 0));
+        lc.cls_y = lc.ok_y ? 1 : (c1 == xc - 1 ? 3 : 0);
+    }
+    lc.use_x = (c0 >= xu0 && c0 < xu0 + UW && c0 < xc);
+    lc.use_y = (c1 >= xu0 && c1 < xu0 + UW && c1 < xc);
+    return lc;
+}
+
+XINV_HD_INLINE LaneCols make_lanecols_ring_lane(int64_t xu0, int HW, int UW, int lane, int64_t xc, bool &seam_lane)
+{
+    LaneCols lc;
+    const int64_t c0 = xu0 - HW + 2 * lane, c1 = c0 + 1, xv = xc + 1;
+    int64_t w0 = c0 % xv; if (w0 < 0) w0 += xv;
+    int64_t w1 = c1 % xv; if (w1 < 0) w1 += xv;
+    lc.l0 = w0; lc.l1 = (w1 == xc) ? xc - 1 : w1;
+    lc.ok_x = true; lc.ok_y = (w1 != xc);
+    lc.cls_x = lc.cls_y = 1;
+    lc.use_x = (c0 >= xu0 && c0 < xu0 + UW && c0 < xc);
+    lc.use_y = (c1 >= xu0 && c1 < xu0 + UW && c1 < xc);
+    seam_lane = (w0 == xc - 1);
+    return lc;
+}
+
+XINV_HD_INLINE bool xinv_lane_pred(const LaneCols &lc, int X, const double *frow, double undef)
+{
+    return X ? (lc.ok_y && frow[lc.l1] != undef) : (lc.ok_x && frow[lc.l0] != undef);
 }
 
 __host__ __device__ inline int xinv_p3_slot_tile(int L, int nfull, int nkc, int &kc)
diff --git a/xinvert_amd/csrc/xinv_tu_pipe2d.hip b/xinvert_amd/csrc/xinv_tu_pipe2d.hip
--- a/xinvert_amd/csrc/xinv_tu_pipe2d.hip
+++ b/xinvert_amd/csrc/xinv_tu_pipe2d.hip
@@ -5,31 +5,38 @@
 #endif
 constexpr bool SEAM = XINV_TU_SEAM != 0;
 
-template <class M, unsigned UM, bool FR, int NP, bool AL, bool EXT>
+template <class M, unsigned UM, bool FR, int NP, bool AL, bool EXT, bool LM>
 static int pipe_one(dim3 grid, hipStream_t st, const FusedArgs &a, int *occ, int lds_pad)
 {
     if (occ) {
         static int cached = 0;
         int n = cached;
         if (!n) {
-            if (hipOccupancyMaxActiveBlocksPerMultiprocessor(&n, k_pipe2d<M, UM, FR, NP, AL, EXT, SEAM>, 64 * XINV_PIPE_P, 0) != hipSuccess)
+            if (hipOccupancyMaxActiveBlocksPerMultiprocessor(&n, k_pipe2d<M, UM, FR, NP, AL, EXT, SEAM, LM>, 64 * XINV_PIPE_P, 0) != hipSuccess)
                 n = 1;
             cached = n = n < 1 ? 1 : n;
         }
         *occ = n;
         return 0;
     }
-    hipLaunchKernelGGL((k_pipe2d<M, UM, FR, NP, AL, EXT, SEAM>), grid, dim3(64 * XINV_PIPE_P, 1, 1), (size_t)lds_pad, st, a);
+    hipLaunchKernelGGL((k_pipe2d<M, UM, FR, NP, AL, EXT, SEAM, LM>), grid, dim3(64 * XINV_PIPE_P, 1, 1), (size_t)lds_pad, st, a);
     return 0;
 }
 
-template <class M, unsigned UM, bool FR, int NP>
-static int pipe_np(bool al, bool ext, dim3 grid, hipStream_t st, const FusedArgs &a, int *occ, int lds_pad)
+template <class M, unsigned UM, bool FR, int NP, bool LM>
+static int pipe_lm(bool al, bool ext, dim3 grid, hipStream_t st, const FusedArgs &a, int *occ, int lds_pad)
 {
     if constexpr (!SEAM) {
-        if (al) return ext ? pipe_one<M, UM, FR, NP, true, true>(grid, st, a, occ, lds_pad) : pipe_one<M, UM, FR, NP, true, false>(grid, st, a, occ, lds_pad);
+        if (al) return ext ? pipe_one<M, UM, FR, NP, true, true, LM>(grid, st, a, occ, lds_pad) : pipe_one<M, UM, FR, NP, true, false, LM>(grid, st, a, occ, lds_pad);
     } else if (al) return 1;
-    return ext ? pipe_one<M, UM, FR, NP, false, true>(grid, st, a, occ, lds_pad) : pipe_one<M, UM, FR, NP, false, false>(grid, st, a, occ, lds_pad);
+    return ext ? pipe_one<M, UM, FR, NP, false, true, LM>(grid, st, a, occ, lds_pad) : pipe_one<M, UM, FR, NP, false, false, LM>(grid, st, a, occ, lds_pad);
+}
+
+template <class M, unsigned UM, bool FR, int NP>
+static int pipe_np(bool lm, bool al, bool ext, dim3 grid, hipStream_t st, const FusedArgs &a, int *occ, int lds_pad)
+{
+    return lm ? pipe_lm<M, UM, FR, NP, true>(al, ext, grid, st, a, occ, lds_pad)
+              : pipe_lm<M, UM, FR, NP, false>(al, ext, grid, st, a, occ, lds_pad);
 }
 
 #if XINV_TU_SEAM
@@ -37,27 +44,27 @@
 #define xinv_launch_pipe2d_gen xinv_launch_pipe2d_gen_seam
 #endif
 #if XINV_TU_MODEL == 2
-int xinv_launch_pipe2d_fma(bool gen, unsigned um, bool fr, bool al, bool ext, dim3 grid, hipStream_t st, const FusedArgs &a, int *occ, int lds_pad)
+int xinv_launch_pipe2d_fma(bool gen, unsigned um, bool fr, bool al, bool ext, dim3 grid, hipStream_t st, const FusedArgs &a, int *occ, int lds_pad, bool lm)
 {
-    if (!gen && um == 3u) return fr ? pipe_np<FusedStd2DF, 3u, true, 1>(al, ext, grid, st, a, occ, lds_pad)
-                                    : pipe_np<FusedStd2DF, 3u, false, 1>(al, ext, grid, st, a, occ, lds_pad);
-    if (gen && um == 0x1fu) return fr ? pipe_np<FusedGen2DF, 0x1fu, true, 1>(al, ext, grid, st, a, occ, lds_pad)
-                                      : pipe_np<FusedGen2DF, 0x1fu, false, 1>(al, ext, grid, st, a, occ, lds_pad);
+    if (!gen && um == 3u) return fr ? pipe_np<FusedStd2DF, 3u, true, 1>(lm, al, ext, grid, st, a, occ, lds_pad)
+                                    : pipe_np<FusedStd2DF, 3u, false, 1>(lm, al, ext, grid, st, a, occ, lds_pad);
+    if (gen && um == 0x1fu) return fr ? pipe_np<FusedGen2DF, 0x1fu, true, 1>(lm, al, ext, grid, st, a, occ, lds_pad)
+                                      : pipe_np<FusedGen2DF, 0x1fu, false, 1>(lm, al, ext, grid, st, a, occ, lds_pad);
     return 1;
 }
 #elif XINV_TU_MODEL == 0
-int xinv_launch_pipe2d_std(unsigned um, int np, bool fr, bool al, bool ext, dim3 grid, hipStream_t st, const FusedArgs &a, int *occ, int lds_pad)
+int xinv_launch_pipe2d_std(unsigned um, int np, bool fr, bool al, bool ext, dim3 grid, hipStream_t st, const FusedArgs &a, int *occ, int lds_pad, bool lm)
 {
-    if (um == 3u && np == 1) return fr ? pipe_np<FusedStd2D, 3u, true, 1>(al, ext, grid, st, a, occ, lds_pad)
-                                       : pipe_np<FusedStd2D, 3u, false, 1>(al, ext, grid, st, a, occ, lds_pad);
+    if (um == 3u && np == 1) return fr ? pipe_np<FusedStd2D, 3u, true, 1>(lm, al, ext, grid, st, a, occ, lds_pad)
+                                       : pipe_np<FusedStd2D, 3u, false, 1>(lm, al, ext, grid, st, a, occ, lds_pad);
     return 1;
 }
 #else
-int xinv_launch_pipe2d_gen(unsigned um, int np, bool fr, bool al, bool ext, dim3 grid, hipStream_t st, const FusedArgs &a, int *occ, int lds_pad)
+int xinv_launch_pipe2d_gen(unsigned um, int np, bool fr, bool al, bool ext, dim3 grid, hipStream_t st, const FusedArgs &a, int *occ, int lds_pad, bool lm)
 {
     (void)np;
-    if (um == 0x1fu) return fr ? pipe_np<FusedGen2D, 0x1fu, true, 1>(al, ext, grid, st, a, occ, lds_pad)
-                               : pipe_np<FusedGen2D, 0x1fu, false, 1>(al, ext, grid, st, a, occ, lds_pad);
+    if (um == 0x1fu) return fr ? pipe_np<FusedGen2D, 0x1fu, true, 1>(lm, al, ext, grid, st, a, occ, lds_pad)
+                               : pipe_np<FusedGen2D, 0x1fu, false, 1>(lm, al, ext, grid, st, a, occ, lds_pad);
     return 1;
 }
 #endif
```

New measurement: 718.1 billion. 0.974x the previous value.
